# mountain/qingdai

Measured on AMD Instinct MI355X. Metric: simulated planet-days/sec at 721x1440 f64, higher is better.
Workload: dtype f64; 1 GPU; 721x1440 seed-42 planet, dt=300 s: forcing + time_step(Teq, dt, albedo) with QD_ENERGY_W=1 QD_CLOUD_COUPLE=1 + slab-ocean coupling + driver-side precipitation/cloud/albedo diagnostics (run_simulation.py:1766-1934,2063-2146) (BASELINE configs[2]; loop order of benchmark_jax.py:124-158); ocean_n_sub=13, parallelism=lat-bands x1

## Files before the change

### include/qingdai_hip.h

```cpp
#ifndef QINGDAI_HIP_H
#define QINGDAI_HIP_H

#include <stddef.h>
#include <stdint.h>

#ifdef __cplusplus
extern "C" {
#endif

#define QD_ABI_VERSION 1

typedef struct qd_ctx* qd_handle;

typedef struct qd_grid_desc {
    int32_t n_lat, n_lon;
    int32_t row0, n_rows, halo;
    int32_t device;
    int32_t rank, world;
} qd_grid_desc;

enum qd_field {
    QD_F_U = 0, QD_F_V, QD_F_H, QD_F_TS, QD_F_Q, QD_F_CLOUD, QD_F_HICE,
    QD_F_ISR, QD_F_ISR_A, QD_F_ISR_B, QD_F_TEQ, QD_F_ALBEDO,
    QD_F_OLR, QD_F_EFLUX, QD_F_PCOND, QD_F_LH, QD_F_LHREL, QD_F_CLOUD_EFF,
    QD_F_FRICTION, QD_F_CSMAP, QD_F_BASE_ALBEDO, QD_F_ELEVATION,
    QD_F_UO, QD_F_VO, QD_F_ETA, QD_F_SST, QD_F_QNET,
    QD_F_PRECIP, QD_F_CLOUD_FROM_P, QD_F_CLOUD_SRC,
    QD_F_W_LAND, QD_F_S_SNOW, QD_F_C_SNOW,
    QD_F_S_SNOW_NEXT, QD_F_MELT, QD_F_P_RAIN, QD_F_GLACIER, QD_F_RUNOFF,
    QD_F_ECO_LAI, QD_F_ECO_LAI_SNAP, QD_F_ECO_F, QD_F_ECO_EDAY, QD_F_ECO_ALPHA, QD_F_ECO_ALPHA_BANDED, QD_F_WATER_ALPHA,
    QD_F_ECO_AGE, QD_F_ECO_SEEDBANK, QD_F_ECO_GATE,
    QD_F_PHYTO_N, QD_F_KD490,
    QD_F_COUNT_F64,
    QD_F_LAND_MASK = 100, QD_F_ICE_MASK = 101,
    QD_F_ECO_DIV_LS = 110, QD_F_ECO_DIV_ALPHA = 111, QD_F_ECO_DIV_BC = 112, QD_F_ECO_DIV_SUMMARY = 113
};

typedef struct qd_params {
    double g, H, tau_rad, greenhouse_factor, a, omega;
    double t_freeze, rho_i, L_f, Cs_ocean, Cs_land, Cs_ice;
    double C_E, rho_a, h_mbl, L_v, p0, ocean_evap_scale, land_evap_scale, ice_evap_scale, tau_cond;
    double sw_a0, sw_kc, lw_eps0, lw_kc, t_floor, c_sfc;
    double energy_w, rh0, k_q, k_p, pcond_ref, hice_ref, eps_default, ch, cp_a;
    double atm_h, gh_factor_lw, eps_ocean, eps_land, eps_ice, lw_tau0, lw_ktau;
    double sigma4, k4_u, k4_v, k4_h, k4_q, k4_cloud, spec_cutoff, spec_damp, diff_factor;
    double H_ocean, rho_w, cp_w, g_ocean, CD, r_bot, rho_a_ocean, vcap, tau_scale;
    double polar_sponge_lat, polar_sponge_gain, K_h, sigma4_ocean, ocean_cfl, ocean_max_u;
    double ocean_k4_u, ocean_k4_v, ocean_k4_eta, ocean_adv_alpha, ocean_ice_qfac, eta_cap, ts_min, ts_max;
    double D_crit, k_precip, alpha_water, alpha_ice, alpha_cloud, p_betadiv, pq_min, p_blend;
    double pref, cmax, w_mem, w_p, w_src, cloud_from_p_floor, cloud_adv_alpha, cloud_smooth_sigma;
    double runoff_tau_days, wland_cap_mm, snow_thresh_K, snow_melt_rate_mm_day, snow_t_band_K;
    double snow_ddf_mm_per_k_day, snow_melt_tref_K, swe_ref_mm, swe_max_mm, snow_albedo_fresh;
    double lapse_k_kpm, land_elev_max_m, polar_ice_thick_max_m, polar_lat_thresh, rho_snow, glacier_frac, glacier_swe_mm;
    double orog_k;
    double qnet_lw_eps0, qnet_lw_kc;
    int32_t seaice_enabled, cloud_couple, lw_v2, gh_lock, polar_freeze_fix_s, polar_freeze_fix_n;
    int32_t mom_scheme;
    int32_t diff_enable, filter_type;
    int32_t diff_every, k4_nsub, diff_q, diff_cloud, shapiro_every, shapiro_n, spec_every;
    int32_t ocean_k4_nsub, ocean_diff_every, ocean_shapiro_n, ocean_shapiro_every;
    int32_t ocean_outlier;
    int32_t ocean_use_qnet, ocean_polar_fix;
    int32_t p_hybrid_fallback, cloud_advect, use_topo_albedo, has_csmap;
    int32_t snow_melt_mode;
    int32_t swe_enable, lapse_enable;
    int32_t orog_enable;
} qd_params;

int qd_abi_version(void);
int qd_device_count(void);
int qd_create(const qd_grid_desc* desc, const qd_params* params, double q_init_rh, qd_handle* out);
int qd_destroy(qd_handle h);
const char* qd_last_error(qd_handle h);

int qd_upload(qd_handle h, int field, const void* host_global, size_t bytes);
int qd_download(qd_handle h, int field, void* host_global, size_t bytes);
int qd_set_params(qd_handle h, const qd_params* params, size_t sizeof_params);
int qd_get_step_counter(qd_handle h, int64_t* atmos_counter, int64_t* ocean_counter);
int qd_set_step_counter(qd_handle h, int64_t atmos_counter, int64_t ocean_counter);

int qd_forcing(qd_handle h, const double star_a[3], const double star_b[3], double theta, int with_teq);
int qd_simple_albedo(qd_handle h, double ocean_albedo);
int qd_atmos_step(qd_handle h, double dt, int has_albedo);
int qd_ocean_step(qd_handle h, double dt, int compute_qnet, int use_ice_mask, int inject_sst);
int qd_driver_physics(qd_handle h, double dt);
int qd_hydrology_commit(qd_handle h, double dt);
int qd_step_n(qd_handle h, int n, double dt, int flags, const double* stars);
int qd_last_ocean_nsub(qd_handle h, int* n_sub);
int qd_sync(qd_handle h);

int qd_op_laplacian(qd_handle h, const double* F, int cos_kind, double* out);
int qd_op_hyperdiffuse(qd_handle h, const double* F, const double* k4_row, double k4_scalar, double dt,
                       int n_substeps, int cos_kind, double* out);
int qd_op_advect(qd_handle h, const double* field, const double* u, const double* v, double dt,
                 int cos_kind, double* out);
int qd_op_shapiro(qd_handle h, const double* F, int n, double* out);
int qd_op_zonal_filter(qd_handle h, const double* F, double cutoff, double damp, double* out);
int qd_op_divergence(qd_handle h, const double* u, const double* v, double* out);
int qd_op_vorticity(qd_handle h, const double* u, const double* v, double* out);
int qd_op_gaussian(qd_handle h, const double* F, double sigma, int mode_wrap, double* out);
int qd_op_median_positive(qd_handle h, const double* x, double dflt, double* out);
int qd_median_state(qd_handle h, double* out64);
int qd_step_scalars(qd_handle h, double* out8);
int qd_ocean_mean_next_count(qd_handle h, int64_t* out);

int qd_band_insolation(qd_handle h, int nb, const double* specA, const double* specB, const double* tray, double* out_host_or_null);

typedef struct qd_eco_params {
    double k_canopy;
    double leaf_scalar;
    double soil_ref;
    double w_lai;
    double light_update_hours;
    double recompute_lai_delta;
    int32_t substep_every_nphys;
    int32_t albedo_couple;
    int32_t bands_couple;
    int32_t water_couple;
    int32_t use_lai;
    int32_t map_f32;
} qd_eco_params;
int qd_eco_configure(qd_handle h, const qd_eco_params* p, size_t sizeof_params);
int qd_eco_set_lai_layers(qd_handle h, const double* layers, int n_planes, int init);
int qd_eco_substep(qd_handle h, double dt);
int qd_eco_banded_alpha(qd_handle h, int nb, const double* r_eff, const double* w_b);
int qd_eco_get_state(qd_handle h, double out[5]);
int qd_eco_set_state(qd_handle h, const double in[3]);

int qd_indiv_configure(qd_handle h, int n_cells, const int32_t* sample_j, const int32_t* sample_i, int n_indiv,
                       const int32_t* cell_index, const double* Ab, const double* tol, int nb, const double* specA,
                       const double* specB, const double* tray, int substeps_per_day, double day_seconds, double soil_cap,
                       int ab_f32);
int qd_indiv_substep(qd_handle h, double dt, int* fired_or_null);
int qd_indiv_download(qd_handle h, double* E_day, double* stress_days);
int qd_indiv_upload(qd_handle h, const double* E_day, const double* stress_days);

int qd_phyto_configure(qd_handle h, int n_species, double K_h, double adv_alpha);
int qd_phyto_upload(qd_handle h, int species, const double* host);
int qd_phyto_download(qd_handle h, int species, double* host);
int qd_phyto_advect_diffuse(qd_handle h, double dt_seconds);

#define QD_PHYTO_DAILY_LOG_W 4
typedef struct qd_phyto_daily_params {
    int32_t n_species, n_bands;
    int32_t idx_490;
    int32_t enable_N;
    int32_t couple;
    int32_t reserved;
    double H_mld;
    double alpha_P, Q10, T_ref, kd_exp_m;
    double sink;
    double R_remin;
    double alpha_clip_min, alpha_clip_max;
    double dt_days;
} qd_phyto_daily_params;
int qd_phyto_daily_configure(qd_handle h, const qd_phyto_daily_params* p, size_t sizeof_params, const double* band_tab,
                             const double* species_tab, const double* shape);
int qd_phyto_daily(qd_handle h, const double* star_row, int use_sst);
int qd_phyto_daily_schedule(qd_handle h, int n, const int32_t* fire);
int qd_phyto_daily_log(qd_handle h, double* out, int max, int* n);
int qd_phyto_daily_download_bands(qd_handle h, double* host, size_t n);
int qd_phyto_daily_state(qd_handle h, int64_t* n_steps);
int qd_phyto_daily_insolation(qd_handle h, const double* star_row, double* insA, double* insB);

#define QD_ECO_DAILY_LOG_W 4
#define QD_ECO_DAILY_MAX_K 8
typedef struct qd_eco_daily_params {
    int32_t n_species, n_layers;
    int32_t spread;
    int32_t moore;
    int32_t gate_soil;
    int32_t reserved;
    double lai_max, k_canopy, growth_per_j, senesce_per_day, stress_thresh, stress_strength;
    double soil_cap;
    double repro_frac;
    double spread_rate;
    double soil_exp, upfrac, dlai_max;
    double seed_energy, seed_scale;
    double seedling_lai, retain, bank_max, seed_dlai_max, germ_frac, bank_decay;
} qd_eco_daily_params;
int qd_eco_daily_configure(qd_handle h, const qd_eco_daily_params* p, size_t sizeof_params, const int32_t* species_mode,
                           const double* species_weights);
int qd_eco_daily_set_layers(qd_handle h, const double* layers, int n_planes);
int qd_eco_daily_get_layers(qd_handle h, double* layers, int n_planes);
int qd_eco_daily_step(qd_handle h, const double* soil_index);
int qd_eco_daily_schedule(qd_handle h, int n, const int32_t* fire);
int qd_eco_daily_log(qd_handle h, double* out, int max, int* n);
// ... 239 lines not shown
```

### qingdai_amd/_lib.py

```python
from __future__ import annotations

import ctypes
import os

from .params import qd_params

_HERE = os.path.dirname(os.path.abspath(__file__))
LIB_PATH = os.environ.get("QD_LIB_PATH") or os.path.join(_HERE, "libqingdai_hip.so")

FIELDS = ["U", "V", "H", "TS", "Q", "CLOUD", "HICE", "ISR", "ISR_A", "ISR_B", "TEQ", "ALBEDO",
          "OLR", "EFLUX", "PCOND", "LH", "LHREL", "CLOUD_EFF", "FRICTION", "CSMAP", "BASE_ALBEDO", "ELEVATION",
          "UO", "VO", "ETA", "SST", "QNET", "PRECIP", "CLOUD_FROM_P", "CLOUD_SRC", "W_LAND", "S_SNOW", "C_SNOW",
          "S_SNOW_NEXT", "MELT", "P_RAIN", "GLACIER", "RUNOFF",
          "ECO_LAI", "ECO_LAI_SNAP", "ECO_F", "ECO_EDAY", "ECO_ALPHA", "ECO_ALPHA_BANDED", "WATER_ALPHA",
          "ECO_AGE", "ECO_SEEDBANK", "ECO_GATE", "PHYTO_N", "KD490"]
F = {n: i for i, n in enumerate(FIELDS)}
F["LAND_MASK"] = 100
F["ICE_MASK"] = 101
F.update({"ECO_DIV_LS": 110, "ECO_DIV_ALPHA": 111, "ECO_DIV_BC": 112, "ECO_DIV_SUMMARY": 113})
R_SUM, R_COSMEAN, R_MAX, R_MIN, R_MAXABS = 0, 1, 2, 3, 4

SYMBOLS = [
    "qd_abi_version", "qd_device_count", "qd_create", "qd_destroy", "qd_last_error", "qd_upload", "qd_download", "qd_set_params",
    "qd_get_step_counter", "qd_set_step_counter", "qd_forcing", "qd_simple_albedo", "qd_atmos_step",
    "qd_ocean_step", "qd_driver_physics", "qd_hydrology_commit", "qd_step_n", "qd_last_ocean_nsub", "qd_sync",
    "qd_op_laplacian", "qd_op_hyperdiffuse", "qd_op_advect", "qd_op_shapiro", "qd_op_zonal_filter", "qd_op_divergence",
    "qd_op_vorticity", "qd_op_gaussian", "qd_op_median_positive", "qd_median_state", "qd_step_scalars", "qd_ocean_mean_next_count", "qd_reduce", "qd_energy_diagnostics", "qd_energy_diagnostics_last", "qd_band_insolation",
    "qd_comm_unique_id", "qd_comm_init", "qd_comm_init_local", "qd_comm_stats", "qd_comm_allreduce_count", "qd_comm_grouped_sum_count", "qd_comm_init_shm", "qd_comm_host_allreduce_count", "qd_hostring_open", "qd_hostring_allreduce",
    "qd_hostring_close", "qd_comm_barrier", "qd_comm_allreduce_max", "qd_peer_export", "qd_peer_connect", "qd_comm_peer_stats", "qd_comm_peer_carried", "qd_peer_selftest", "qd_peer_disable", "qd_tune_reload",
    "qd_plansim_create", "qd_plansim_destroy", "qd_plansim_plan", "qd_plansim_mark", "qd_plansim_margin", "qd_plansim_segments",
    "qd_plansim_pop_exchange", "qd_plansim_segments_rows",
    "qd_eco_configure", "qd_eco_set_lai_layers", "qd_eco_substep", "qd_eco_banded_alpha", "qd_eco_get_state", "qd_eco_set_state",
    "qd_indiv_configure", "qd_indiv_substep", "qd_indiv_download", "qd_indiv_upload",
    "qd_phyto_configure", "qd_phyto_upload", "qd_phyto_download", "qd_phyto_advect_diffuse",
    "qd_phyto_daily_configure", "qd_phyto_daily", "qd_phyto_daily_schedule", "qd_phyto_daily_log", "qd_phyto_daily_download_bands",
    "qd_phyto_daily_state", "qd_phyto_daily_insolation",
    "qd_eco_daily_configure", "qd_eco_daily_set_layers", "qd_eco_daily_get_layers", "qd_eco_daily_step", "qd_eco_daily_schedule",
    "qd_eco_daily_log", "qd_eco_daily_state", "qd_eco_daily_speciate",
    "qd_eco_state_restore",
    "qd_indiv_daily_configure", "qd_indiv_daily_step", "qd_indiv_daily_log", "qd_indiv_daily_weights", "qd_indiv_daily_state",
    "qd_eco_diversity", "qd_eco_diversity_on", "qd_eco_diversity_download",
    "qd_truecolor_configure", "qd_truecolor_render", "qd_truecolor_download",
    "qd_stateframe_configure", "qd_stateframe_scan", "qd_stateframe_render", "qd_stateframe_download",
    "qd_tiles_configure", "qd_tiles_set_plane", "qd_tiles_available", "qd_tiles_scan", "qd_tiles_order_stats", "qd_tiles_render", "qd_tiles_download",
    "qd_budget_diag_configure", "qd_budget_diag_schedule", "qd_budget_diag_log", "qd_budget_diag_reset",
    "qd_history_configure", "qd_history_schedule", "qd_history_sample", "qd_history_read", "qd_history_reset", "qd_history_restore",
    "qd_state_digest", "qd_state_scalars_get", "qd_state_scalars_set",
    "qd_route_configure", "qd_route_free", "qd_route_reset", "qd_route_accumulate", "qd_route_event", "qd_route_schedule",
    "qd_route_download", "qd_route_events", "qd_route_restore",
    "qd_hydronet_build", "qd_hydronet_sweeps",
    "qd_topogen_smooth", "qd_topogen_build", "qd_topogen_last_ms",
    "qd_copy_ceiling", "qd_timing_enable", "qd_timing_select", "qd_timing_get", "qd_timing_reset",
]


class qd_eco_params(ctypes.Structure):
    _fields_ = ([(n, ctypes.c_double) for n in ("k_canopy", "leaf_scalar", "soil_ref", "w_lai", "light_update_hours",
                                                 "recompute_lai_delta")] +
                [(n, ctypes.c_int32) for n in ("substep_every_nphys", "albedo_couple", "bands_couple", "water_couple", "use_lai", "map_f32")])


class qd_phyto_daily_params(ctypes.Structure):
    _fields_ = ([(n, ctypes.c_int32) for n in ("n_species", "n_bands", "idx_490", "enable_N", "couple", "reserved")] +
                [(n, ctypes.c_double) for n in ("H_mld", "alpha_P", "Q10", "T_ref", "kd_exp_m", "sink", "R_remin", "alpha_clip_min",
                                                 "alpha_clip_max", "dt_days")])


class qd_eco_daily_params(ctypes.Structure):
    _fields_ = ([(n, ctypes.c_int32) for n in ("n_species", "n_layers", "spread", "moore", "gate_soil", "reserved")] +
                [(n, ctypes.c_double) for n in ("lai_max", "k_canopy", "growth_per_j", "senesce_per_day", "stress_thresh", "stress_strength",
                                                 "soil_cap", "repro_frac", "spread_rate", "soil_exp", "upfrac", "dlai_max", "seed_energy",
                                                 "seed_scale", "seedling_lai", "retain", "bank_max", "seed_dlai_max", "germ_frac",
                                                 "bank_decay")])


class qd_indiv_daily_params(ctypes.Structure):
    _fields_ = ([(n, ctypes.c_int32) for n in ("n_species", "n_layers", "per_cell", "seed_couple")] +
                [(n, ctypes.c_double) for n in ("stress_penalty", "lai_grow", "lai_decay", "recruit_frac", "stress_decay", "repro_frac",
                                                 "seed_energy", "retain", "bank_max", "lai_max")])


class qd_truecolor_params(ctypes.Structure):
    _fields_ = ([(n, ctypes.c_int32) for n in ("snow_by_swe", "veg", "veg_f_one", "oceancolor", "snow_by_ts", "rivers", "lakes", "nb_eco",
                                                "nb_phyto", "reserved")] +
                [(n, ctypes.c_double) for n in ("h_ice_ref", "ice_frac_thr", "snow_cover_frac", "snow_vis_alpha", "veg_gamma", "veg_sat",
                                                 "soil_ref", "oc_gamma", "oc_blend", "snow_thresh", "cloud_alpha", "cloud_white",
                                                 "river_min", "river_alpha", "lake_alpha")])


TRUECOLOR_MAX_BANDS = 16

STATEFRAME_PANELS = 15
STATEFRAME_MAX_LEVELS = 32
STATEFRAME_GUTTER = 4
STATEFRAME_SCAN_N = 28


class qd_stateframe_params(ctypes.Structure):
    _fields_ = ([(n, ctypes.c_int32) for n in ("ps_abs", "ocean", "rivers", "lakes")] +
                [(n, ctypes.c_double) for n in ("p0", "rho_a", "H", "river_min", "river_alpha", "lake_alpha")])


class qd_stateframe_panel(ctypes.Structure):
    _fields_ = ([(n, ctypes.c_int32) for n in ("n_levels", "extend_max", "constant", "coast")] +
                [("levels", ctypes.c_double * STATEFRAME_MAX_LEVELS), ("rgb", (ctypes.c_double * 3) * STATEFRAME_MAX_LEVELS)])


class qd_stateframe_table(ctypes.Structure):
    _fields_ = [("panel", qd_stateframe_panel * STATEFRAME_PANELS), ("mark_cell", ctypes.c_int64 * 2)]

# ... 100 lines not shown
    lib.qd_op_shapiro.argtypes = [vp, vp, i32, vp]
    lib.qd_op_zonal_filter.argtypes = [vp, vp, dbl, dbl, vp]
    lib.qd_op_divergence.argtypes = [vp, vp, vp, vp]
    lib.qd_op_vorticity.argtypes = [vp, vp, vp, vp]
    lib.qd_op_gaussian.argtypes = [vp, vp, dbl, i32, vp]
    lib.qd_op_median_positive.argtypes = [vp, vp, dbl, dp]
    lib.qd_reduce.argtypes = [vp, i32, i32, dp]
    lib.qd_energy_diagnostics.argtypes = [vp, dp]
    lib.qd_energy_diagnostics_last.argtypes = [vp, dp]
    lib.qd_copy_ceiling.argtypes = [vp, sz, i32, dp]
    lib.qd_band_insolation.argtypes = [vp, i32, dp, dp, dp, vp]
    lib.qd_eco_configure.argtypes = [vp, ctypes.POINTER(qd_eco_params), sz]
    lib.qd_eco_set_lai_layers.argtypes = [vp, vp, i32, i32]
    lib.qd_eco_substep.argtypes = [vp, dbl]
    lib.qd_eco_banded_alpha.argtypes = [vp, i32, dp, dp]
    lib.qd_eco_get_state.argtypes = [vp, dp]
    lib.qd_eco_set_state.argtypes = [vp, dp]
    lib.qd_indiv_configure.argtypes = [vp, i32, ip, ip, i32, ip, vp, vp, i32, dp, dp, dp, i32, dbl, dbl, i32]
    lib.qd_indiv_substep.argtypes = [vp, dbl, ip]
    lib.qd_indiv_download.argtypes = [vp, vp, vp]
    lib.qd_indiv_upload.argtypes = [vp, vp, vp]
    lib.qd_phyto_configure.argtypes = [vp, i32, dbl, dbl]
    lib.qd_phyto_upload.argtypes = [vp, i32, vp]
    lib.qd_phyto_download.argtypes = [vp, i32, vp]
    lib.qd_phyto_advect_diffuse.argtypes = [vp, dbl]
    lib.qd_phyto_daily_configure.argtypes = [vp, ctypes.POINTER(qd_phyto_daily_params), sz, dp, dp, dp]
    lib.qd_phyto_daily.argtypes = [vp, dp, i32]
    lib.qd_phyto_daily_schedule.argtypes = [vp, i32, ip]
    lib.qd_phyto_daily_log.argtypes = [vp, dp, i32, ip]
    lib.qd_phyto_daily_download_bands.argtypes = [vp, dp, sz]
    lib.qd_phyto_daily_state.argtypes = [vp, ctypes.POINTER(i64)]
    lib.qd_phyto_daily_insolation.argtypes = [vp, dp, dp, dp]
    lib.qd_eco_daily_configure.argtypes = [vp, ctypes.POINTER(qd_eco_daily_params), sz, ip, dp]
    lib.qd_eco_daily_set_layers.argtypes = [vp, vp, i32]
    lib.qd_eco_daily_get_layers.argtypes = [vp, vp, i32]
    lib.qd_eco_state_restore.argtypes = [vp, vp, i32, dp, i32, i32, ctypes.c_double]
    lib.qd_eco_daily_step.argtypes = [vp, vp]
    lib.qd_eco_daily_schedule.argtypes = [vp, i32, ip]
    lib.qd_eco_daily_log.argtypes = [vp, dp, i32, ip]
    lib.qd_eco_daily_state.argtypes = [vp, ctypes.POINTER(i64)]
    lib.qd_eco_daily_speciate.argtypes = [vp, i32, ctypes.c_double, dp]
    lib.qd_indiv_daily_configure.argtypes = [vp, ctypes.POINTER(qd_indiv_daily_params), sz, ip, ip]
    lib.qd_indiv_daily_step.argtypes = [vp, vp]
    lib.qd_indiv_daily_log.argtypes = [vp, dp, i32, ip]
    lib.qd_indiv_daily_weights.argtypes = [vp, dp, i32]
    lib.qd_indiv_daily_state.argtypes = [vp, ctypes.POINTER(i64)]
    lib.qd_eco_diversity.argtypes = [vp, vp, i32, i32, dp, dp]
    lib.qd_eco_diversity_on.argtypes = [vp, i32, i32, u8p, vp, i32, i32, dp, dp]
    lib.qd_eco_diversity_download.argtypes = [vp, i32, dp, sz]
    lib.qd_truecolor_configure.argtypes = [vp, ctypes.POINTER(qd_truecolor_params), sz, dp, dp, dp, u8p]
    lib.qd_truecolor_render.argtypes = [vp, i32, dp, dp]
    lib.qd_truecolor_download.argtypes = [vp, i32, vp, sz]
    lib.qd_stateframe_configure.argtypes = [vp, ctypes.POINTER(qd_stateframe_params), sz, u8p]
    lib.qd_stateframe_scan.argtypes = [vp, dp, ctypes.POINTER(i64)]
    lib.qd_stateframe_render.argtypes = [vp, ctypes.POINTER(qd_stateframe_table), sz, dp, i32]
    lib.qd_stateframe_download.argtypes = [vp, i32, vp, sz]
    lib.qd_tiles_configure.argtypes = [vp, dbl, dp, i32, i32]
    lib.qd_tiles_set_plane.argtypes = [vp, dp]
    lib.qd_tiles_available.argtypes = [vp, ip]
    lib.qd_tiles_scan.argtypes = [vp, ctypes.POINTER(qd_tile_ref), i32, dp, ctypes.POINTER(i64)]
    lib.qd_tiles_order_stats.argtypes = [vp, i32, i32, ctypes.POINTER(i64), i32, dp, ctypes.POINTER(i64)]
    lib.qd_tiles_render.argtypes = [vp, ctypes.POINTER(qd_tile_desc), sz, i32, i32]
    lib.qd_tiles_download.argtypes = [vp, i32, vp, sz]
    lib.qd_budget_diag_configure.argtypes = [vp, i32, u8p]
    lib.qd_budget_diag_schedule.argtypes = [vp, i32, ip]
    lib.qd_budget_diag_log.argtypes = [vp, dp, i32, ip]
    lib.qd_budget_diag_reset.argtypes = [vp]
    lib.qd_history_configure.argtypes = [vp, i32, ip, ip, ip]
    lib.qd_history_schedule.argtypes = [vp, i32, ip]
    lib.qd_history_sample.argtypes = [vp]
    lib.qd_history_read.argtypes = [vp, dp, ctypes.POINTER(i64)]
    lib.qd_history_reset.argtypes = [vp]
    lib.qd_history_restore.argtypes = [vp, dp, i64]
    lib.qd_state_digest.argtypes = [vp, i32, ip, ctypes.POINTER(ctypes.c_uint64)]
    lib.qd_state_scalars_get.argtypes = [vp, dp, i32]
    lib.qd_state_scalars_set.argtypes = [vp, dp, i32]
    lib.qd_comm_unique_id.argtypes = [vp, sz]
    lib.qd_comm_init.argtypes = [vp, vp, sz]
    lib.qd_comm_barrier.argtypes = [vp]
    lib.qd_comm_init_local.argtypes = [ctypes.POINTER(vp), i32]
    lib.qd_median_state.argtypes = [vp, dp]
    lib.qd_step_scalars.argtypes = [vp, dp]
    lib.qd_ocean_mean_next_count.argtypes = [vp, ctypes.POINTER(i64)]
    lib.qd_comm_stats.argtypes = [vp, ctypes.POINTER(i32)]
    lib.qd_comm_allreduce_count.argtypes = [vp, ctypes.POINTER(i32)]
    lib.qd_comm_grouped_sum_count.argtypes = [vp, ctypes.POINTER(i32)]
    lib.qd_comm_init_shm.argtypes = [vp, ctypes.c_char_p]
    lib.qd_comm_host_allreduce_count.argtypes = [vp, ctypes.POINTER(i32)]
    lib.qd_hostring_open.argtypes = [ctypes.c_char_p, i32, i32, ctypes.POINTER(vp)]
    lib.qd_hostring_allreduce.argtypes = [vp, dp, i32, i32]
    lib.qd_hostring_close.argtypes = [vp]
    lib.qd_comm_allreduce_max.argtypes = [vp, dp, i32]
    lib.qd_tune_reload.argtypes = [vp]
    lib.qd_peer_export.argtypes = [vp, vp, sz]
    lib.qd_peer_connect.argtypes = [vp, vp, sz, i32]
    lib.qd_peer_selftest.argtypes = [vp, i32, ctypes.POINTER(ctypes.c_longlong)]
    lib.qd_peer_disable.argtypes = [vp]
    lib.qd_comm_peer_stats.argtypes = [vp, ctypes.POINTER(i32), ctypes.POINTER(i32)]
    lib.qd_comm_peer_carried.argtypes = [vp]
    lib.qd_plansim_create.argtypes = [ctypes.POINTER(qd_grid_desc), ctypes.POINTER(vp)]
    lib.qd_plansim_destroy.argtypes = [vp]
    lib.qd_plansim_plan.argtypes = [vp, ip, ip, i32, i32]
    lib.qd_plansim_mark.argtypes = [vp, ip, i32, i32]
    lib.qd_plansim_margin.argtypes = [vp, i32]
    lib.qd_plansim_segments.argtypes = [vp, i32, ip]
    lib.qd_plansim_pop_exchange.argtypes = [vp, ip, i32, ip]
    lib.qd_plansim_segments_rows.argtypes = [vp, i32, i32, ip]
    lib.qd_route_configure.argtypes = [vp, ctypes.POINTER(qd_route_plan), sz]
    lib.qd_route_free.argtypes = [vp]
    lib.qd_route_reset.argtypes = [vp]
    lib.qd_route_accumulate.argtypes = [vp, dbl]
    lib.qd_route_event.argtypes = [vp, dbl, i32]
    lib.qd_route_schedule.argtypes = [vp, i32, dp]
    lib.qd_route_download.argtypes = [vp, i32, dp, sz]
    lib.qd_route_events.argtypes = [vp, dp, i32, ip]
    lib.qd_route_restore.argtypes = [vp, dp, dp, dp, i64]
    lib.qd_hydronet_build.argtypes = [vp, i32, i32, u8p, dp, dbl, i32, dp, dp, dp, dbl, dp, ip, ip, u8p, ip, ip, i32,
                                      ip, ip]
    lib.qd_hydronet_sweeps.argtypes = [vp, ip]
    lib.qd_topogen_smooth.argtypes = [vp, i32, i32, dp, dp, i32, dp, i32, i32, dp]
    lib.qd_topogen_build.argtypes = [vp, i32, i32, dp, i32, dp, dp, i32, dp, dp, dp, dp, dp, ip, dp, dp, u8p, dp]
    lib.qd_topogen_last_ms.argtypes = [vp, dp]
    lib.qd_timing_enable.argtypes = [vp, i32]
    lib.qd_timing_select.argtypes = [vp, ctypes.c_char_p]
    lib.qd_timing_get.argtypes = [vp, ctypes.c_char_p, dp, ctypes.POINTER(i64)]
    lib.qd_timing_reset.argtypes = [vp]
    for s in SYMBOLS:
        getattr(lib, s).restype = i32
    lib.qd_last_error.restype = ctypes.c_char_p
    _lib = lib
    return lib
```

### qingdai_amd/csrc/qd_api.hip

```cpp
#include "qd_span.h"
#include <chrono>
#include <atomic>
#include <cstring>
#include <cstdio>
#include <cstdlib>
#include <algorithm>

thread_local std::string g_qd_create_err;

int qd_fail(qd_ctx* c, const char* what, hipError_t e) {
    std::string m = what ? what : "error";
    if (e != hipSuccess) { m += ": "; m += hipGetErrorString(e); }
    if (c) c->err = m; else g_qd_create_err = m;
    return -1;
}

static hipEvent_t qd_get_event(qd_ctx* c) {
    if (!c->ev_free.empty()) { hipEvent_t e = c->ev_free.back(); c->ev_free.pop_back(); return e; }
    hipEvent_t e = nullptr;
    hipEventCreate(&e);
    return e;
}
QdScope::QdScope(qd_ctx* c_, const char* n, bool attach_) : c(c_), name(n), attach(attach_) {
    on = c->timing == 1;
// ... 211 lines not shown
    std::atomic_thread_fence(std::memory_order_acquire);
    return 0;
}


int qd_wait_host_nonneg(qd_ctx* c, volatile double* slot, double* out, const char* what) {
    const auto t0 = std::chrono::steady_clock::now();
    unsigned spins = 0;
    double v;
    while (!((v = *slot) >= 0.0)) {
        __builtin_ia32_pause();
        if ((++spins & 0x3FFFu) == 0) {
            const hipError_t q = hipStreamQuery(c->stream);
            if (q != hipErrorNotReady && !(*slot >= 0.0)) return qd_fail(c, what, q);
            if (std::chrono::duration<double>(std::chrono::steady_clock::now() - t0).count() > 60.0) return qd_fail(c, what);
        }
    }
    *slot = -1.0;
    std::atomic_thread_fence(std::memory_order_seq_cst);
    *out = v;
    return 0;
}

__global__ void k_publish_host(const double* __restrict__ src, int n, double* dst, double* stamp, double seq) {
    if ((int)threadIdx.x < n)
        __hip_atomic_store((unsigned long long*)dst + threadIdx.x, (unsigned long long)__double_as_longlong(src[threadIdx.x]), __ATOMIC_RELAXED,
                           __HIP_MEMORY_SCOPE_SYSTEM);
    asm volatile("s_waitcnt vmcnt(0)" ::: "memory");
    if (threadIdx.x == 0)
        __hip_atomic_store((unsigned long long*)stamp, (unsigned long long)__double_as_longlong(seq), __ATOMIC_RELAXED, __HIP_MEMORY_SCOPE_SYSTEM);
}
int qd_fetch_scalars(qd_ctx* c, const double* dsrc, int n, double* hdst) {
    if (n < 1 || n > 32) return qd_fail(c, "qd_fetch_scalars: bad count");
    c->pub_seq += 1.0;
    hipLaunchKernelGGL(k_publish_host, dim3(1), dim3(64), 0, c->stream, dsrc, n, hdst, c->hpin + 61, c->pub_seq);
    if (qd_wait_host_flag(c, c->hpin + 61, c->pub_seq, "device scalars never reached the host")) return -1;
    if (c->hpin[60] != 0.0) return qd_fail(c, "peer exchange: a rank did not arrive within the deadline");
    return 0;
}

extern "C" int qd_abi_version(void) { return QD_ABI_VERSION; }
extern "C" int qd_device_count(void) { int n = 0; return hipGetDeviceCount(&n) == hipSuccess ? n : 0; }

static void qd_read_tuning(qd_ctx* c) {
    c->tune = QdTune();
    auto geti = [](const char* name, int dflt) { const char* e = std::getenv(name); return e ? std::atoi(e) : dflt; };
    QdTune& t = c->tune;
    c->stream_rows = std::max(0, geti("QD_STREAM_R", 0));
    { const int r = geti("QD_TAIL_R", 0); if (r > 0) t.tail_r = r; }
    { const int r = geti("QD_TAIL_RP", 0); if (r >= 3) t.tail_rp = r; }
    t.tail_v = geti("QD_TAIL_V", 0) == 1 ? 1 : 0;
    t.tail_general = geti("QD_TAIL_GENERAL", 0) == 1 ? 1 : 0;
    t.stream_r_dyn = std::max(0, geti("QD_STREAM_R_DYN", 0));
    t.stream_r_ocn = std::max(0, geti("QD_STREAM_R_OCN", 0));
    t.stream_vb = geti("QD_STREAM_VB", -1);
    { const int b = geti("QD_MED_BLOCKS", 0); if (b >= 16) t.med_blocks = b; }
    t.shapiro_r = std::max(0, geti("QD_SHAPIRO_R", 0));
    t.tile_tr = std::max(0, geti("QD_TILE_TR", 0));
    t.fused_r = std::max(0, geti("QD_FUSED_R", 0));
    t.fused_seq = geti("QD_FUSED_SEQ", 0) == 1 ? 1 : 0;
    t.fused_norot = geti("QD_FUSED_NOROT", 0) == 1 ? 1 : 0;
    t.stream_no_pair = geti("QD_STREAM_NO_PAIR", 0) == 1 ? 1 : 0;
}
extern "C" int qd_tune_reload(qd_handle c) { if (!c) return -1; qd_read_tuning(c); c->tile = QdTileShape{0, 0, 0, 0}; return 0; }

extern "C" int qd_create(const qd_grid_desc* d, const qd_params* params, double q_init_rh, qd_handle* out) {
    if (!d || !params || !out) return qd_fail(nullptr, "qd_create: null argument");
    if (d->n_lat < 5 || d->n_lon < 4) return qd_fail(nullptr, "qd_create: grid too small (need n_lat>=5, n_lon>=4)");
    if (d->row0 < 0 || d->n_rows < 1 || d->row0 + d->n_rows > d->n_lat || d->halo < 0)
        return qd_fail(nullptr, "qd_create: bad latitude band");
    const bool full = (d->row0 == 0 && d->n_rows == d->n_lat);
    if (full && d->halo != 0) return qd_fail(nullptr, "qd_create: a whole-globe handle takes halo = 0");
    if (!full && d->n_rows + 2 * d->halo > d->n_lat) return qd_fail(nullptr, "qd_create: band + 2 halos taller than the grid");
    if (!full && d->halo < 5) return qd_fail(nullptr, "qd_create: band handles need halo >= 5 rows");
    int ndev = 0;
    if (hipGetDeviceCount(&ndev) != hipSuccess || ndev == 0) return qd_fail(nullptr, "qd_create: no HIP device visible");
    if (d->device < 0 || d->device >= ndev) return qd_fail(nullptr, "qd_create: bad device ordinal");
    qd_ctx* c = new qd_ctx();
    c->desc = *d; c->p = *params;
    { const char* ef = std::getenv("QD_FUSED"); if (ef && ef[0] == '0') c->use_fused = 0; }
    { const char* ef = std::getenv("QD_FUSED_FAST"); if (ef) c->fused_fast = std::atoi(ef); }
    { const char* ef = std::getenv("QD_TAIL_ACC"); if (ef) c->tail_acc = std::atoi(ef); }
    { const char* ef = std::getenv("QD_MEAN_IN_MOMENTUM"); if (ef) c->mean_in_momentum = ef[0] == '0' ? 0 : 1; }
    { const char* ef = std::getenv("QD_SHAPIRO_STREAM"); if (ef) c->shapiro_stream = std::atoi(ef); }
    { const char* ef = std::getenv("QD_OCN_TAIL"); if (ef) c->ocn_tail = std::atoi(ef); }
    if (c->ocn_tail != 0) c->ocn_tail = 1;
    { const char* ef = std::getenv("QD_OCN_FUSED"); if (ef) c->ocn_fused = ef[0] == '1' ? 1 : 0; }
    { const char* ef = std::getenv("QD_BAND_TAIL"); if (ef) c->band_tail = ef[0] == '0' ? 0 : 1; }
    qd_read_tuning(c);
    { const char* ef = std::getenv("QD_GROUP_SUMS"); if (ef) c->group_sums = ef[0] == '0' ? 0 : 1; }
    c->geo = QdGeom{d->n_lat, d->n_lon, d->row0, d->n_rows, d->halo, full ? 1 : 0, d->row0 - d->halo, d->n_rows + 2 * d->halo};
    c->own_row0 = d->row0; c->own_nrows = d->n_rows;
    auto bail = [&](const char* w, hipError_t e) { qd_fail(nullptr, w, e); qd_destroy(c); return -1; };
    hipError_t e;
    if ((e = hipSetDevice(d->device)) != hipSuccess) return bail("hipSetDevice", e);
    if ((e = hipStreamCreate(&c->stream)) != hipSuccess) return bail("hipStreamCreate", e);
    { int ncu = 0; c->n_cu = (hipDeviceGetAttribute(&ncu, hipDeviceAttributeMultiprocessorCount, d->device) == hipSuccess && ncu > 0) ? ncu : 256; }
    const size_t cells = c->geo.cells() + (size_t)QD_PAD_ROWS * c->geo.nlon;
    for (int f = 0; f < QD_F_COUNT_F64; ++f) {
        if ((e = hipMalloc(&c->f[f], cells * sizeof(double))) != hipSuccess) return bail("hipMalloc field", e);
        hipMemsetAsync(c->f[f], 0, cells * sizeof(double), c->stream);
    }
    for (int s = 0; s < QD_NSCRATCH; ++s) {
        if ((e = hipMalloc(&c->scratch[s], cells * sizeof(double))) != hipSuccess) return bail("hipMalloc scratch", e);
        hipMemsetAsync(c->scratch[s], 0, cells * sizeof(double), c->stream);
    }
    if ((e = hipMalloc(&c->land, cells)) != hipSuccess) return bail("hipMalloc mask", e);
    if ((e = hipMalloc(&c->icemask, cells)) != hipSuccess) return bail("hipMalloc mask", e);
    hipMemsetAsync(c->land, 0, cells, c->stream); hipMemsetAsync(c->icemask, 0, cells, c->stream);
    if (build_tables(c)) return bail("table allocation", hipErrorOutOfMemory);
    if ((e = hipMalloc(&c->k4_atm, (size_t)5 * d->n_lat * sizeof(double))) != hipSuccess) return bail("hipMalloc", e);
    if ((e = hipMalloc(&c->k4_ocn, (size_t)3 * d->n_lat * sizeof(double))) != hipSuccess) return bail("hipMalloc", e);
    c->red_blocks = (12 + (d->n_lon + QD_BLOCK - 1) / QD_BLOCK) * c->geo.lrows() + 64;
    if ((e = hipMalloc(&c->red_partial, (size_t)c->red_blocks * sizeof(double))) != hipSuccess) return bail("hipMalloc", e);
    if ((e = hipMalloc(&c->dscal, QD_S_COUNT * sizeof(double))) != hipSuccess) return bail("hipMalloc", e);
    if ((e = hipMalloc(&c->dcount, 32 * sizeof(unsigned long long))) != hipSuccess) return bail("hipMalloc", e);
    if ((e = hipMalloc(&c->eta_acc, 1024 * sizeof(unsigned long long))) != hipSuccess) return bail("hipMalloc", e);
    hipMemsetAsync(c->eta_acc, 0, 1024 * sizeof(unsigned long long), c->stream);
    if ((e = hipMalloc(&c->hist, 2 * QD_HIST_BINS * sizeof(unsigned int))) != hipSuccess) return bail("hipMalloc", e);
    if ((e = hipMalloc(&c->sel_state, 8 * sizeof(unsigned long long))) != hipSuccess) return bail("hipMalloc", e);
    hipMemsetAsync(c->dscal, 0, QD_S_COUNT * sizeof(double), c->stream);
    hipMemsetAsync(c->dcount, 0, 32 * sizeof(unsigned long long), c->stream);
    hipMemsetAsync(c->hist, 0, 2 * QD_HIST_BINS * sizeof(unsigned int), c->stream);
    hipMemsetAsync(c->sel_state, 0, 8 * sizeof(unsigned long long), c->stream);
    { const char* ef = std::getenv("QD_TAIL_FIX"); if (ef) c->tail_fix = ef[0] == '0' ? 0 : 1; }
    c->fix_dense = 256.0 * (double)c->geo.cells() / (721.0 * 1440.0);
    { const char* ef = std::getenv("QD_TAIL_FIX_DENSE"); if (ef) c->fix_dense = std::atof(ef); }
    { const char* ef = std::getenv("QD_LAZY_DIAG"); if (ef) c->lazy_diag = ef[0] == '0' ? 0 : 1; }
    if (c->tail_fix) {
        if ((e = hipMalloc(&c->fix_count, 64)) != hipSuccess) return bail("hipMalloc", e);
        hipMemsetAsync(c->fix_count, 0, 64, c->stream);
        if ((e = hipMalloc(&c->fix_list, c->geo.cells() * 3 * sizeof(unsigned long long))) != hipSuccess) return bail("hipMalloc", e);
    }
    if (!full) {
        if ((e = hipMalloc(&c->med_pred, 64 * sizeof(double))) != hipSuccess) return bail("hipMalloc", e);
        hipMemsetAsync(c->med_pred, 0, 64 * sizeof(double), c->stream);
        if ((e = hipMalloc(&c->med_gather, (size_t)std::max(1, d->world) * 4096 * sizeof(double))) != hipSuccess) return bail("hipMalloc", e);
        if ((e = hipMalloc(&c->sel_ccount, 2 * sizeof(unsigned int))) != hipSuccess) return bail("hipMalloc", e);
        hipMemsetAsync(c->sel_ccount, 0, 2 * sizeof(unsigned int), c->stream);
        { const char* ef = std::getenv("QD_MEDIAN_PREDICT"); if (ef && ef[0] == '0') c->med_predict = 0; }
    }
    if (full) {
        if ((e = hipMalloc(&c->sel_cand, 2 * cells * sizeof(double))) != hipSuccess) return bail("hipMalloc", e);
        if ((e = hipMalloc(&c->sel_ccount, 2 * sizeof(unsigned int))) != hipSuccess) return bail("hipMalloc", e);
        hipMemsetAsync(c->sel_ccount, 0, 2 * sizeof(unsigned int), c->stream);
        if ((e = hipMalloc(&c->med_pred, 64 * sizeof(double))) != hipSuccess) return bail("hipMalloc", e);
        hipMemsetAsync(c->med_pred, 0, 64 * sizeof(double), c->stream);
        { const char* ef = std::getenv("QD_MEDIAN_PREDICT"); if (ef && ef[0] == '0') c->med_predict = 0; }
        { const char* ef = std::getenv("QD_MERGE_POINTWISE"); if (ef) c->merge_pointwise = ef[0] == '0' ? 0 : 1; }
        { const char* ef = std::getenv("QD_HOIST_PRECIP"); if (ef) c->hoist_precip = ef[0] == '0' ? 0 : 1; }
        { const char* ef = std::getenv("QD_SIDE_STREAM"); if (ef) c->side_stream_on = ef[0] == '0' ? 0 : 1; }
        { const char* ef = std::getenv("QD_MERGE_FINAL"); if (ef) c->merge_final = ef[0] == '0' ? 0 : 1; }
        { const char* ef = std::getenv("QD_MERGE_PCOND"); if (ef) c->merge_pcond = ef[0] == '0' ? 0 : 1; }


        c->n_wgmax = (int)(qd_grid2d(c->geo).x * (unsigned)c->geo.nrows);
        if ((e = hipMalloc(&c->wgmax, (size_t)2 * c->n_wgmax * sizeof(double))) != hipSuccess) return bail("hipMalloc", e);
        { const char* ef = std::getenv("QD_MED_SIDE"); if (ef) c->med_side = ef[0] == '0' ? 0 : 1; }
        { const char* ef = std::getenv("QD_MED_PAIR"); if (ef) c->med_pair = ef[0] == '0' ? 0 : 1; }
        { const char* ef = std::getenv("QD_MED_FOLD"); if (ef) c->med_fold = ef[0] == '0' ? 0 : 1; }
        { const char* ef = std::getenv("QD_MERGE_SAF"); if (ef) c->merge_saf = ef[0] == '0' ? 0 : 1; }
        if (c->med_side) {
            if ((e = hipEventCreateWithFlags(&c->med_fork, hipEventDisableTiming)) != hipSuccess) return bail("hipEventCreate", e);
            if ((e = hipEventCreateWithFlags(&c->med_done, hipEventDisableTiming)) != hipSuccess) return bail("hipEventCreate", e);
        }
        if (c->med_side || c->med_pair) {
            if ((e = hipMalloc(&c->hist_b, 2 * QD_HIST_BINS * sizeof(unsigned int))) != hipSuccess) return bail("hipMalloc", e);
            if ((e = hipMalloc(&c->sel_state_b, 8 * sizeof(unsigned long long))) != hipSuccess) return bail("hipMalloc", e);
            if ((e = hipMalloc(&c->sel_cand_b, 2 * cells * sizeof(double))) != hipSuccess) return bail("hipMalloc", e);
            if ((e = hipMalloc(&c->sel_ccount_b, 2 * sizeof(unsigned int))) != hipSuccess) return bail("hipMalloc", e);
            hipMemsetAsync(c->hist_b, 0, 2 * QD_HIST_BINS * sizeof(unsigned int), c->stream);
            hipMemsetAsync(c->sel_state_b, 0, 8 * sizeof(unsigned long long), c->stream);
            hipMemsetAsync(c->sel_ccount_b, 0, 2 * sizeof(unsigned int), c->stream);
        }
        if ((c->side_stream_on || c->med_side) && (e = hipStreamCreateWithFlags(&c->side_stream, hipStreamNonBlocking)) != hipSuccess) return bail("hipStreamCreate", e);
        if (c->side_stream_on) {
            if ((e = hipEventCreateWithFlags(&c->side_fork, hipEventDisableTiming)) != hipSuccess) return bail("hipEventCreate", e);
            if ((e = hipEventCreateWithFlags(&c->side_done, hipEventDisableTiming)) != hipSuccess) return bail("hipEventCreate", e);
            if ((e = hipMalloc(&c->red_partial_b, (size_t)c->red_blocks * sizeof(double))) != hipSuccess) return bail("hipMalloc", e);
        }
    }
    if ((e = hipHostMalloc((void**)&c->hpin, 64 * sizeof(double), hipHostMallocMapped | hipHostMallocCoherent)) != hipSuccess) return bail("hipHostMalloc", e);
    if ((e = hipHostMalloc((void**)&c->hpin_rows, (size_t)3 * c->geo.lrows() * sizeof(double), hipHostMallocMapped | hipHostMallocCoherent)) != hipSuccess) return bail("hipHostMalloc", e);
    std::memset(c->hpin, 0, 64 * sizeof(double));
    c->hpin[57] = -1.0; c->hpin[58] = -1.0; c->hpin[59] = -1.0;
    std::memset(c->hpin_rows, 0, (size_t)3 * c->geo.lrows() * sizeof(double));
    const double q0 = std::min(std::max(q_init_rh, 0.0), 1.0) * host_qsat(288.0, params->p0);
    hipLaunchKernelGGL(k_init_state, dim3((d->n_lon + QD_BLOCK - 1) / QD_BLOCK, c->geo.lrows()), dim3(QD_BLOCK), 0,
                       c->stream, c->geo, c->tabs, params->H, q0, c->f[QD_F_H], c->f[QD_F_TS], c->f[QD_F_Q], c->f[QD_F_SST]);
    if ((e = hipStreamSynchronize(c->stream)) != hipSuccess) return bail("init", e);
    if (!full) {
        for (int f = 0; f < QD_F_COUNT_F64; ++f) c->vm[c->f[f]] = d->halo;
        c->vm[c->land] = d->halo; c->vm[c->icemask] = d->halo;
    }
    *out = c;
    return 0;
}

extern "C" int qd_destroy(qd_handle c) {
    if (!c) return 0;
    hipSetDevice(c->desc.device);
    if (c->stream) hipStreamSynchronize(c->stream);
    if (c->med_pred && std::getenv("QD_MEDIAN_DEBUG")) {
        double h[64];
        if (hipMemcpy(h, c->med_pred, sizeof(h), hipMemcpyDeviceToHost) == hipSuccess)
            for (int s = 0; s < 4; ++s)
                fprintf(stderr, "[median site %d] last median %.6g bracket [%.6g, %.6g] hits %.0f misses %.0f last list %.0f of %.0f; "
                        "last miss at call %.0f: centre %.6g -> median %.6g\n", s, h[16 * s], h[16 * s + 8], h[16 * s + 9], h[16 * s + 4],
                        h[16 * s + 5], h[16 * s + 6], h[16 * s + 7], h[16 * s + 13], h[16 * s + 14], h[16 * s + 15]);
    }
    qd_phyto_release(c);
    qd_route_release(c);
    qd_phyto_daily_release(c);
    qd_indiv_daily_release(c);
    qd_eco_daily_release(c);
    qd_eco_div_release(c);
    qd_truecolor_release(c);
    qd_stateframe_release(c);
    qd_tiles_release(c);
    qd_budget_release(c);
    qd_history_release(c);
    for (int f = 0; f < QD_F_COUNT_F64; ++f) if (c->f[f]) hipFree(c->f[f]);
    for (int s = 0; s < QD_NSCRATCH; ++s) if (c->scratch[s]) hipFree(c->scratch[s]);
    for (double* t : c->tab_alloc) hipFree(t);
    if (c->land) hipFree(c->land); if (c->icemask) hipFree(c->icemask);
    if (c->k4_atm) hipFree(c->k4_atm); if (c->k4_ocn) hipFree(c->k4_ocn); for (int k = 0; k < 2; ++k) if (c->qs_tab[k]) hipFree(c->qs_tab[k]);
    if (c->red_partial) hipFree(c->red_partial); if (c->dscal) hipFree(c->dscal);
    if (c->red_partial_b) hipFree(c->red_partial_b);
    if (c->wgmax) hipFree(c->wgmax);
    qd_saf_drop(c);
    if (c->fix_count && std::getenv("QD_TAIL_FIX_DEBUG")) {
        unsigned int h[8] = {0};
        if (hipMemcpy(h, c->fix_count, sizeof(h), hipMemcpyDeviceToHost) == hipSuccess)
            fprintf(stderr, "[tail fix list] %u entries in %u launches (%.1f per launch), longest list %u of %zu cells\n", h[4], h[5],
                    h[5] ? (double)h[4] / h[5] : 0.0, h[6], c->geo.cells());
    }
    if (c->fix_count) hipFree(c->fix_count); if (c->fix_list) hipFree(c->fix_list);
    if (c->side_stream) { hipStreamSynchronize(c->side_stream); hipStreamDestroy(c->side_stream); }
    if (c->side_fork) hipEventDestroy(c->side_fork); if (c->side_done) hipEventDestroy(c->side_done);
    if (c->med_fork) hipEventDestroy(c->med_fork); if (c->med_done) hipEventDestroy(c->med_done);
    if (c->hist_b) hipFree(c->hist_b); if (c->sel_state_b) hipFree(c->sel_state_b); if (c->sel_cand_b) hipFree(c->sel_cand_b); if (c->sel_ccount_b) hipFree(c->sel_ccount_b);
    if (c->eta_acc) hipFree(c->eta_acc);
    if (c->dcount) hipFree(c->dcount); if (c->hist) hipFree(c->hist); if (c->sel_state) hipFree(c->sel_state);
    if (c->zonal_tw) hipFree(c->zonal_tw);
    if (c->bands) hipFree(c->bands);
    if (c->digest_out) hipFree(c->digest_out);
    qd_eco_free(c);
    if (c->sel_cand) hipFree(c->sel_cand); if (c->sel_ccount) hipFree(c->sel_ccount);
    if (c->med_pred) hipFree(c->med_pred);
    if (c->med_gather) hipFree(c->med_gather);
    qd_comm_release(c);
    if (c->hpin) hipHostFree(c->hpin);
    if (c->hpin_rows) hipHostFree(c->hpin_rows);
    if (c->stage) hipHostFree(c->stage);
    qd_resolve_timers(c);
    for (hipEvent_t e : c->ev_free) hipEventDestroy(e);
    if (c->stream) hipStreamDestroy(c->stream);
    delete c;
    return 0;
}

extern "C" const char* qd_last_error(qd_handle c) { return c ? c->err.c_str() : g_qd_create_err.c_str(); }

int qd_band_copy_in(qd_ctx* c, void* dst, const void* host, size_t esz) {
    const QdGeom& G = c->geo;
    const size_t rowb = (size_t)G.nlon * esz;
    if (G.full) return hipMemcpyAsync(dst, host, rowb * G.nlat, hipMemcpyHostToDevice, c->stream) == hipSuccess ? 0 : -1;
    for (int l = 0; l < G.lrows(); ++l) {
        int g = l + G.row0 - G.halo;
        if (g < 0) g += G.nlat; if (g >= G.nlat) g -= G.nlat;
        if (hipMemcpyAsync((char*)dst + (size_t)l * rowb, (const char*)host + (size_t)g * rowb, rowb,
                           hipMemcpyHostToDevice, c->stream) != hipSuccess) return -1;
    }
    return 0;
}

extern "C" int qd_upload(qd_handle c, int field, const void* host, size_t bytes) {
    if (!c || !host) return -1;
    hipSetDevice(c->desc.device);
    const size_t n = (size_t)c->geo.nlat * c->geo.nlon;
    if (field == QD_F_LAND_MASK || field == QD_F_ICE_MASK) {
        if (bytes != n) return qd_fail(c, "qd_upload: mask size mismatch");
        uint8_t* dst = field == QD_F_LAND_MASK ? c->land : c->icemask;
        if (qd_band_copy_in(c, dst, host, 1)) return qd_fail(c, "qd_upload: copy failed");
        qd_mark(c, {dst}, c->geo.halo);
    } else {
        if (field < 0 || field >= QD_F_COUNT_F64) return qd_fail(c, "qd_upload: unknown field");
        if (bytes != n * sizeof(double)) return qd_fail(c, "qd_upload: size mismatch (expect n_lat*n_lon float64)");
        if (qd_eco_is_f32(c, field)) {
            if (qd_band_copy_in(c, c->scratch[10], host, sizeof(double))) return qd_fail(c, "qd_upload: copy failed");
            qd_eco_convert_slab(c, c->scratch[10], 0, c->f[field], 1);
        } else if (qd_band_copy_in(c, c->f[field], host, sizeof(double))) return qd_fail(c, "qd_upload: copy failed");
        qd_mark(c, {c->f[field]}, c->geo.halo);
        if (field == QD_F_CLOUD_EFF) c->cloud_eff_valid = 1;
        if (field == QD_F_ELEVATION) c->has_elevation = 1;
        if (field == QD_F_ECO_ALPHA) c->eco.alpha_valid = 1;
        if (field == QD_F_ECO_ALPHA_BANDED) c->eco.banded_valid = 1;
        if (field == QD_F_WATER_ALPHA) c->eco.water_valid = 1;
    }
    QD_HIP(c, hipStreamSynchronize(c->stream));
    if (field == QD_F_LAND_MASK) {
        const uint8_t* m = (const uint8_t*)host;
        const int nlat = c->geo.nlat, nlon = c->geo.nlon;
        double ws = 0.0;
        for (int i = 0; i < nlat; ++i) {
            const double w = std::max(std::cos((-90.0 + 180.0 * i / (double)(nlat - 1)) * (M_PI / 180.0)), 0.0);
            int cnt = 0;
            for (int j = 0; j < nlon; ++j) cnt += (m[(size_t)i * nlon + j] == 0);
            ws += w * cnt;
        }
        c->wsum_ocean = ws;
    }
    return 0;
}

extern "C" int qd_download(qd_handle c, int field, void* host, size_t bytes) {
    if (!c || !host) return -1;
    hipSetDevice(c->desc.device);
    const QdGeom& G = c->geo;
    const size_t n = (size_t)G.nlat * G.nlon;
    const void* src; size_t esz;
    if (field == QD_F_LAND_MASK || field == QD_F_ICE_MASK) { src = field == QD_F_LAND_MASK ? c->land : c->icemask; esz = 1; }
    else {
        if (field < 0 || field >= QD_F_COUNT_F64) return qd_fail(c, "qd_download: unknown field");
        src = c->f[field]; esz = sizeof(double);
        if (qd_eco_is_f32(c, field)) { qd_eco_convert_slab(c, c->f[field], 1, c->scratch[10], 0); src = c->scratch[10]; }
    }
    if (bytes != n * esz) return qd_fail(c, "qd_download: size mismatch");
    const size_t rowb = (size_t)G.nlon * esz;
    QD_HIP(c, hipMemcpyAsync((char*)host + (size_t)G.row0 * rowb, (const char*)src + (size_t)G.halo * rowb,
                             rowb * G.nrows, hipMemcpyDeviceToHost, c->stream));
    QD_HIP(c, hipStreamSynchronize(c->stream));
    return 0;
}

extern "C" int qd_set_params(qd_handle c, const qd_params* p, size_t sz) {
    if (!c || !p) return -1;
    if (sz != sizeof(qd_params)) return qd_fail(c, "qd_set_params: struct size mismatch (ABI drift)");
    const bool tabs_stale = (p->omega != c->p.omega) || (p->g != c->p.g) || (p->a != c->p.a) || (p->polar_sponge_lat != c->p.polar_sponge_lat) ||
                            (p->polar_sponge_gain != c->p.polar_sponge_gain);
    c->p = *p;
    c->k4_atm_dt = -1; c->k4_ocn_dt = -1;
    if (tabs_stale) {
        hipSetDevice(c->desc.device);
        hipStreamSynchronize(c->stream);
        for (double* t : c->tab_alloc) hipFree(t);
        c->tab_alloc.clear();
        if (build_tables(c)) return qd_fail(c, "qd_set_params: table rebuild failed");
    }
    return 0;
}

extern "C" int qd_get_step_counter(qd_handle c, int64_t* a, int64_t* o) {
    if (!c) return -1; if (a) *a = c->atm_counter; if (o) *o = c->ocn_counter; return 0;
}
extern "C" int qd_set_step_counter(qd_handle c, int64_t a, int64_t o) {
    if (!c) return -1; c->atm_counter = a; c->ocn_counter = o; return 0;
}
extern "C" int qd_sync(qd_handle c) {
    if (!c) return -1;
    hipSetDevice(c->desc.device);
    QD_HIP(c, hipStreamSynchronize(c->stream));
    return 0;
}
extern "C" int qd_last_ocean_nsub(qd_handle c, int* n) { if (!c || !n) return -1; *n = c->last_nsub; return 0; }

extern "C" int qd_forcing(qd_handle c, const double sa[3], const double sb[3], double theta, int with_teq) {
    if (!c || !sa || !sb) return -1;
    hipSetDevice(c->desc.device);
    return qd_forcing_impl(c, sa, sb, theta, with_teq);
}
extern "C" int qd_simple_albedo(qd_handle c, double ocean_albedo) {
    if (!c) return -1;
    hipSetDevice(c->desc.device);
    return qd_simple_albedo_impl(c, ocean_albedo);
}
extern "C" int qd_atmos_step(qd_handle c, double dt, int has_albedo) {
    if (!c) return -1;
    hipSetDevice(c->desc.device);
    if (int rc = qd_atmos_step_impl(c, dt, has_albedo)) return rc;
    return qd_launch_check(c, "qd_atmos_step");
}
extern "C" int qd_ocean_step(qd_handle c, double dt, int compute_qnet, int use_ice_mask, int inject_sst) {
    if (!c) return -1;
    hipSetDevice(c->desc.device);
    if (int rc = qd_ocean_step_impl(c, dt, compute_qnet, use_ice_mask, inject_sst)) return rc;
    return qd_launch_check(c, "qd_ocean_step");
}
extern "C" int qd_driver_physics(qd_handle c, double dt) {
    if (!c) return -1;
    hipSetDevice(c->desc.device);
    if (int rc = qd_driver_physics_impl(c, dt)) return rc;
    return qd_launch_check(c, "qd_driver_physics");
}
// ... 148 lines not shown
    qd_hyperdiffuse_fields(c, fl, 1, tab, &skip, &ov, dt, n_substeps, cos_kind ? c->tabs.cos05 : c->tabs.cos02, 0);
    int rc = seam_out(c, fl[0], out);
    if (fl[0] != save10) { for (int s = 0; s < QD_NSCRATCH; ++s) if (c->scratch[s] == save10 && s != 10) { c->scratch[s] = fl[0]; break; } c->scratch[10] = save10; }
    return rc;
}

extern "C" int qd_op_advect(qd_handle c, const double* field, const double* u, const double* v, double dt,
                            int cos_kind, double* out) {
    if (!c || !field || !u || !v || !out) return -1;
    hipSetDevice(c->desc.device);
    if (seam_in(c, c->scratch[10], field) || seam_in(c, c->scratch[11], u) || seam_in(c, c->scratch[12], v)) return -1;
    qd_launch_advect(c, c->scratch[11], c->scratch[12], cos_kind ? c->tabs.cos05 : c->tabs.cos6, dt,
                     c->scratch[10], c->scratch[13], nullptr, nullptr, 1.0, 0, 0);
    return seam_out(c, c->scratch[13], out);
}

extern "C" int qd_op_shapiro(qd_handle c, const double* F, int n, double* out) {
    if (!c || !F || !out) return -1;
    hipSetDevice(c->desc.device);
    if (seam_in(c, c->scratch[10], F)) return -1;
    double* fl[1] = {c->scratch[10]};
    double* save10 = c->scratch[10];
    qd_shapiro_fields(c, fl, 1, n, 0);
    int rc = seam_out(c, fl[0], out);
    if (fl[0] != save10) { for (int s = 0; s < QD_NSCRATCH; ++s) if (c->scratch[s] == save10 && s != 10) { c->scratch[s] = fl[0]; break; } c->scratch[10] = save10; }
    return rc;
}

static int seam_divvort(qd_ctx* c, const double* u, const double* v, double* out, int vort) {
    if (!c || !u || !v || !out) return -1;
    hipSetDevice(c->desc.device);
    if (seam_in(c, c->scratch[10], u) || seam_in(c, c->scratch[11], v)) return -1;
    qd_launch_divvort(c, c->scratch[10], c->scratch[11], c->scratch[12], vort, 0);
    return seam_out(c, c->scratch[12], out);
}
extern "C" int qd_op_zonal_filter(qd_handle c, const double* F, double cutoff, double damp, double* out) {
    if (!c || !F || !out) return -1;
    hipSetDevice(c->desc.device);
    if (seam_in(c, c->scratch[10], F)) return -1;
    double* fl[1] = {c->scratch[10]};
    if (qd_zonal_filter_fields(c, fl, 1, cutoff, damp, 0)) return -1;
    return seam_out(c, c->scratch[10], out);
}
extern "C" int qd_op_divergence(qd_handle c, const double* u, const double* v, double* out) { return seam_divvort(c, u, v, out, 0); }
extern "C" int qd_op_vorticity(qd_handle c, const double* u, const double* v, double* out) { return seam_divvort(c, u, v, out, 1); }

extern "C" int qd_op_gaussian(qd_handle c, const double* F, double sigma, int mode_wrap, double* out) {
    if (!c || !F || !out) return -1;
    hipSetDevice(c->desc.device);
    if (seam_in(c, c->scratch[10], F)) return -1;
    if (qd_gaussian(c, c->scratch[10], c->scratch[11], c->scratch[12], sigma, mode_wrap, 0)) return -1;
    return seam_out(c, c->scratch[11], out);
}

extern "C" int qd_op_median_positive(qd_handle c, const double* x, double dflt, double* out) {
    if (!c || !x || !out) return -1;
    hipSetDevice(c->desc.device);
    if (seam_in(c, c->scratch[10], x)) return -1;
    qd_median_positive_dev(c, c->scratch[10], dflt, QD_S_MED_OUT, 0, 0.0, 0);
    QD_HIP(c, hipMemcpyAsync(c->hpin, c->dscal + QD_S_MED_OUT, sizeof(double), hipMemcpyDeviceToHost, c->stream));
    QD_HIP(c, hipStreamSynchronize(c->stream));
    *out = c->hpin[0];
    return 0;
}

extern "C" int qd_median_state(qd_handle c, double* out64) {
    if (!c || !out64) return -1;
    hipSetDevice(c->desc.device);
    for (int k = 0; k < 16 * 4; ++k) out64[k] = 0.0;
    if (!c->med_pred) return 0;
    QD_HIP(c, hipStreamSynchronize(c->stream));
    QD_HIP(c, hipMemcpy(out64, c->med_pred, sizeof(double) * 16 * 4, hipMemcpyDeviceToHost));
    return 0;
}

extern "C" int qd_step_scalars(qd_handle c, double* out8) {
    if (!c || !out8) return -1;
    hipSetDevice(c->desc.device);
    QD_HIP(c, hipStreamSynchronize(c->stream));
    QD_HIP(c, hipMemcpy(out8, c->dscal, sizeof(double) * 8, hipMemcpyDeviceToHost));
    return 0;
}

extern "C" int qd_ocean_mean_next_count(qd_handle c, int64_t* out) {
    if (!c || !out) return -1;
    *out = c->mean_next_count;
    return 0;
}

extern "C" int qd_reduce(qd_handle c, int field, int op, double* out) {
    if (!c || !out) return -1;
    if (field < 0 || field >= QD_F_COUNT_F64) return qd_fail(c, "qd_reduce: unknown field");
    hipSetDevice(c->desc.device);
    double v = 0;
    const int op1 = (op == QD_R_COSWEIGHTED_MEAN) ? 1 : (op == QD_R_SUM ? 0 : (op == QD_R_MAX ? 2 : (op == QD_R_MIN ? 3 : 4)));
    if (qd_reduce_field(c, c->f[field], op1, &v)) return -1;
    if (op == QD_R_COSWEIGHTED_MEAN) v = v / (c->wsum_all + 1e-15);
    *out = v;
    return 0;
}

extern "C" int qd_band_insolation(qd_handle c, int nb, const double* specA, const double* specB, const double* tray, double* out_host) {
    if (!c || !specA || !specB || !tray) return -1;
    hipSetDevice(c->desc.device);
    return qd_band_insolation_impl(c, nb, specA, specB, tray, out_host);
}
extern "C" int qd_energy_diagnostics_last(qd_handle c, double* out) {
    if (!c || !out) return -1;
    for (int k = 0; k < 10; ++k) out[k] = c->last_diag[k];
    return 0;
}
extern "C" int qd_energy_diagnostics(qd_handle c, double* out) {
    if (!c || !out) return -1;
    hipSetDevice(c->desc.device);
    return qd_energy_diag_impl(c, out);
}

extern "C" int qd_copy_ceiling(qd_handle c, size_t bytes, int reps, double* gbs) {
    if (!c || !gbs || bytes == 0 || reps < 1) return -1;
    hipSetDevice(c->desc.device);
    void *a = nullptr, *b = nullptr;
    if (hipMalloc(&a, bytes) != hipSuccess || hipMalloc(&b, bytes) != hipSuccess) { if (a) hipFree(a); return qd_fail(c, "qd_copy_ceiling: hipMalloc"); }
    hipMemsetAsync(a, 1, bytes, c->stream); hipMemsetAsync(b, 2, bytes, c->stream);
    hipEvent_t e0, e1;
    hipEventCreate(&e0); hipEventCreate(&e1);
    hipMemcpyAsync(b, a, bytes, hipMemcpyDeviceToDevice, c->stream);
    hipEventRecord(e0, c->stream);
    for (int r = 0; r < reps; ++r) hipMemcpyAsync((r & 1) ? a : b, (r & 1) ? b : a, bytes, hipMemcpyDeviceToDevice, c->stream);
    hipEventRecord(e1, c->stream);
    hipStreamSynchronize(c->stream);
    float ms = 0.f;
    hipEventElapsedTime(&ms, e0, e1);
    hipEventDestroy(e0); hipEventDestroy(e1);
    hipFree(a); hipFree(b);
    *gbs = ms > 0.f ? (2.0 * (double)bytes * reps / 1e9) / ((double)ms / 1e3) : 0.0;
    return 0;
}

extern "C" int qd_timing_enable(qd_handle c, int on) { if (!c) return -1; c->timing = on ? 1 : 0; return 0; }
extern "C" int qd_timing_select(qd_handle c, const char* name) {
    if (!c || !name) return -1; c->timing = 2; c->timing_sel = name; return 0;
}
extern "C" int qd_timing_reset(qd_handle c) { if (!c) return -1; qd_resolve_timers(c); c->timers.clear(); c->timing_seen.clear(); return 0; }
extern "C" int qd_timing_get(qd_handle c, const char* name, double* mean_ms, int64_t* launches) {
    if (!c || !name) return -1;
    hipSetDevice(c->desc.device);
    qd_resolve_timers(c);
    auto it = c->timers.find(name);
    if (it == c->timers.end() || it->second.n == 0) { if (mean_ms) *mean_ms = 0; if (launches) *launches = 0; return 0; }
    if (mean_ms) *mean_ms = it->second.total_ms / (double)it->second.n;
    if (launches) *launches = it->second.n;
    return 0;
}
```

### qingdai_amd/csrc/qd_fused.h

```cpp
#pragma once
#include "qd_internal.h"

struct QdDynArgs {
    const double *u, *v, *h, *fric, *q, *cloud;
    double *uo, *vo, *ho, *qo, *co;
    const double* k4row[5];
    double k4s[5];
    int skip[5];
    double g, a, dt, dlat, dlon, f_min;
    double inv_dlon, inv_2dlon, inv_dlat, inv_2dlat, pgf_y;
    int primitive;
    int fast;
    QdTileShape ts;
};


struct QdOcnArgs {
    const double *uo, *vo, *eta, *taux, *tauy;
    const uint8_t* land;
    double *uo_out, *vo_out, *eta_out;
    const double* k4row[3];
    double k4s[3];
    int skip[3];
    double a, g, dlat, dlon, sub_dt, rhoH, r_bot;
    double inv_2dlon, inv_2dlat, inv_a, inv_rhoH;
    const double* eta_mean;
    double eta_cap;
    int fast;
    QdTileShape ts;
    const unsigned long long* acc_read = nullptr;
    const double* acc_partial = nullptr;
    int acc_n = 0;
    double acc_wsum = 0.0;
};


QdTileShape qd_pick_tile(const QdGeom& G);
int qd_launch_dyn_hyper(qd_ctx* c, QdDynArgs& P, int margin);
int qd_launch_ocn_hyper(qd_ctx* c, QdOcnArgs& P, int margin);

bool qd_stream_ok(const qd_ctx* c, int margin);
bool qd_ocn_stream_ok(const qd_ctx* c, int margin);
int qd_launch_dyn_stream(qd_ctx* c, const QdDynArgs& P, int margin);
int qd_launch_ocn_stream(qd_ctx* c, const QdOcnArgs& P, int margin);
bool qd_ocn_stream_ok_list(const qd_ctx* c, const QdSegList& S);
int qd_launch_ocn_stream_list(qd_ctx* c, const QdOcnArgs& P, const QdSegList& S);
```

### qingdai_amd/csrc/qd_internal.h

```cpp
#pragma once

#include <hip/hip_runtime.h>
#include <hip/hip_ext.h>
#include <stdint.h>
#include <string>
#include <vector>
#include <functional>
#include <map>
#include <unordered_map>
#include <initializer_list>
#include <climits>
#include <cfloat>
#include <cmath>

#include "../../include/qingdai_hip.h"

#define QD_NSCRATCH 16
#define QD_MAX_DEVICES 64
#define QD_PAD_ROWS 8
#define QD_BLOCK 256
#define QD_MAXF 5
#define QD_HIST_BINS 2048

struct QdGeom {
// ... 138 lines not shown
    double k4_atm_dt = -1, k4_ocn_dt = -1;
    int k4_atm_skip[5] = {0}, k4_ocn_skip[3] = {0};
    double* red_partial = nullptr;
    int red_blocks = 0;
    double* dscal = nullptr;
    unsigned long long* dcount = nullptr;
    unsigned int* hist = nullptr;
    unsigned long long* sel_state = nullptr;
    double* bands = nullptr;
    int bands_nb = 0;
    double last_diag[10] = {0};
    int has_elevation = 0;
    QdPhyto phyto;
    QdEco eco;
    struct QdRoute* route = nullptr;
    struct QdPhytoDaily* pdaily = nullptr;
    struct QdEcoDaily* edaily = nullptr;
    struct QdIndivDaily* idaily = nullptr;
    struct QdEcoDiv* ediv = nullptr;
    struct QdTrueColor* tcol = nullptr;
    struct QdTiles* tiles = nullptr;
    struct QdStateFrame* sframe = nullptr;
    struct QdBudget* budget = nullptr;
    struct QdHistory* history = nullptr;
    unsigned long long* digest_out = nullptr;
    double budget_fire = 0.0;
    int hydronet_sweeps = -1;
    double topogen_ms = -1.0;
    double* zonal_tw = nullptr;
    double* sel_cand = nullptr;
    unsigned int* sel_ccount = nullptr;
    double* med_pred = nullptr;
    int med_predict = 1;
    int med_seen[4] = {0, 0, 0, 0};
    double* pending_sum = nullptr;
    int group_sums = 1;
    long grouped_sums = 0;
    int band_tail = 1;
    double* qt_tab = nullptr;
    double qt_tab_a = 0.0;
    int hoist_precip = 1;
    int precip_done = 0;
    int lazy_diag = 1, diag_write = 1;
    int merge_pcond = 1;
    int med_pair = 1;
    int med_fold = 0;
    int med_side = 0;
    bool med_side_active = false;
    hipEvent_t med_fork = nullptr, med_done = nullptr;
    unsigned int* hist_b = nullptr; unsigned long long* sel_state_b = nullptr; double* sel_cand_b = nullptr; unsigned int* sel_ccount_b = nullptr;
    int want_pcond_ahead = 0;
    int pcond_ahead = 0;
    int tail_fix = 1;
    unsigned int* fix_count = nullptr;
    unsigned long long* fix_list = nullptr;
    double fix_avg = 0.0;
    double fix_dense = 256.0;
    int64_t fix_probe_at = 0;
    int fix_probe_every = 32;
    int merge_saf = 1;
    void* saf_pending = nullptr;
    int defer_final = 0;
    int merge_final = 1;
    struct { int on = 0; double dt = 0, decay = 0, dfac = 0; } final_pending;
    double* wgmax = nullptr;
    int n_wgmax = 0;
    int side_stream_on = 0;
    hipStream_t side_stream = nullptr;
    hipEvent_t side_fork = nullptr, side_done = nullptr;
    bool side_pending = false;
    double* red_partial_b = nullptr;
    std::function<int()> before_cfl_wait;
    int merge_pointwise = 1;
    double* med_gather = nullptr;
    double* hpin = nullptr;
    double* hpin_rows = nullptr;
    double wsum_ocean = 0, wsum_all = 0;
    int64_t atm_counter = 0, ocn_counter = 0;
    QdTileShape tile{0, 0, 0, 0};
    int use_fused = 1;
    int fused_fast = 1;
    long long mean_next_count = 0;
    int mean_in_momentum = 1;
    int tail_acc = 1;
    unsigned long long* eta_acc = nullptr;
    int shapiro_stream = 1;
    int ocn_fused = 0;
    int ocn_tail = 1;
    int stream_rows = 0;
    double* qs_tab[2] = {nullptr, nullptr};
    double qs_key[2][8] = {{NAN, 0, 0, 0, 0, 0, 0, 0}, {NAN, 0, 0, 0, 0, 0, 0, 0}};
    std::vector<double> h_lapK[2];
    std::vector<double> h_k4[2];
    QdTune tune;
    int n_cu = 0;
    int qs_wgs_per_cu[3] = {0, 0, 0};
    int cloud_eff_valid = 0;
    int last_nsub = 0;
    void* stage = nullptr; size_t stage_bytes = 0;
    std::unordered_map<const void*, int> vm;
    int own_row0 = 0, own_nrows = 0;
    void* comm = nullptr;
    struct QdLocalGroup* lgroup = nullptr;
    struct QdPeer* peer = nullptr;
    std::vector<struct QdUse> split_pending;
    std::vector<struct QdUse> corefresh;
    int exchanges = 0;
    int allreduces = 0;
    double pub_seq = 0.0;
    double eta_seq = 0.0;
    void* hring = nullptr;
    void* plansim = nullptr;
    int host_allreduces = 0;
    const char* lap_tag = "k_laplacian";
    const char* hyp_tag = "k_hyper_apply";
    int timing = 0;
    std::string timing_sel;
    std::map<std::string, long> timing_seen;
    std::map<std::string, QdTimer> timers;
    struct Pending { hipEvent_t e0, e1; std::string name; };
    std::vector<Pending> pending;
    std::vector<hipEvent_t> ev_free;
    std::string err;
};

enum { QD_S_PREF = 0, QD_S_ETA_MEAN, QD_S_MED_OUT, QD_S_PSCALE, QD_S_RENORM, QD_S_PQMEAN, QD_S_TMP0, QD_S_TMP1,
       QD_S_DIAG0 = 16,
       QD_S_COUNT = 32 };

extern thread_local std::string g_qd_create_err;

int qd_fail(qd_ctx* c, const char* what, hipError_t e = hipSuccess);
#define QD_HIP(c, call) do { hipError_t _e = (call); if (_e != hipSuccess) return qd_fail((c), #call, _e); } while (0)
inline int qd_launch_check(qd_ctx* c, const char* who) {
    const hipError_t e = hipGetLastError();
    return e == hipSuccess ? 0 : qd_fail(c, (std::string(who) + ": launch").c_str(), e);
}
inline bool qd_whole_globe(const qd_ctx* c) { return c->geo.full && c->desc.world <= 1; }
struct QdPartials {
    double* p = nullptr; int nblk = 0, planes = 0; size_t cap = 0;
    int ensure(qd_ctx* c, int planes_, int nblk_) {
        const size_t n = (size_t)planes_ * (size_t)nblk_;
        if (!p || cap < n) {
            free();
            QD_HIP(c, hipMalloc(&p, n * sizeof(double)));
            cap = n;
        }
        planes = planes_; nblk = nblk_;
        return 0;
    }
    void free() { if (p) hipFree(p); p = nullptr; cap = 0; }
};

struct QdScope {
    qd_ctx* c; const char* name; hipEvent_t e0 = nullptr, e1 = nullptr; bool on = false, attach = false;
    bool used = false;
    QdScope(qd_ctx* c_, const char* n, bool attach_ = false);
    ~QdScope();
};
#define QD_LAUNCH_TIMED(sc, kernel, grid, block, stream, ...) do { \
    if ((sc).on && (sc).attach) { (sc).used = true; hipExtLaunchKernelGGL(kernel, grid, block, 0, stream, (sc).e0, (sc).e1, 0, __VA_ARGS__); } \
    else hipLaunchKernelGGL(kernel, grid, block, 0, stream, __VA_ARGS__); } while (0)

#define QD_IN(ptr, r) QdUse{(void**)&(ptr), (r), 0}
#define QD_IN8(ptr, r) QdUse{(void**)&(ptr), (r), 1}
int qd_allreduce_sum_deferred(qd_ctx* c, double* dptr);
// ... 152 lines not shown
```

### qingdai_amd/csrc/qd_ocean.hip

```cpp
#include <cstdlib>
#include <atomic>
#include <chrono>
#include "qd_internal.h"
#include "qd_device.h"
#include "qd_wave.h"

#include "qd_fluxes.h"
#include "qd_fused.h"
#include "qd_ocntail.h"
#include "qd_band.h"
#include "qd_blockred.h"

QdColP qd_make_colp(const qd_ctx* c, double dt);

__global__ void __launch_bounds__(QD_BLOCK)
k_qnet(QdGeom G, QdColP P, const double* __restrict__ isr, const double* __restrict__ albedo,
       const double* __restrict__ cloud, const double* __restrict__ Ts, const double* __restrict__ h,
       const double* __restrict__ u, const double* __restrict__ v, const uint8_t* __restrict__ land,
       const double* __restrict__ hice, const double* __restrict__ LH, double* __restrict__ qnet,
       uint8_t* __restrict__ icemask) {
    const QdTile tl = qd_tile();
    const int j = tl.seg * QD_BLOCK + threadIdx.x;
    if (j >= G.nlon) return;
    const size_t o = (size_t)qd_lrow(G, G.row0 + tl.row) * G.nlon + j;
// ... 716 lines not shown
            } else {
            for (int k = 0; k < G.nrows; ++k)
                if (qd_wait_host_flag(c, c->hpin_rows + (size_t)2 * G0.lrows() + k, c->eta_seq, "ocean step: the CFL maxima never arrived")) return -1;
            for (int k = 0; k < G.nrows; ++k) { maxVa = std::max(maxVa, c->hpin_rows[k]); maxUo = std::max(maxUo, c->hpin_rows[G.nrows + k]); }
            }
        } else {
        const bool hooked = qd_peer_hooks(c) && !qd_has_host_ring(c) && S.n <= 3;
        for (int k = 0; k < S.n; ++k) {
            const QdGeom& G = S.g[k];
            hipLaunchKernelGGL(k_stress_max, dim3(1, G.nrows), blk, 0, c->stream, G, F[QD_F_U], F[QD_F_V], F[QD_F_UO],
                               F[QD_F_VO], p.vcap, p.rho_a_ocean * p.CD, p.tau_scale, taux, tauy,
                               c->red_partial + (size_t)k * 2 * G0.lrows(), (double*)nullptr, 0.0);
            if (!hooked)
            hipLaunchKernelGGL(k_max2_finish, dim3(1), blk, 0, c->stream, c->red_partial + (size_t)k * 2 * G0.lrows(), G.nrows,
                               c->dscal + QD_S_TMP0 + 2 * k, k == S.n - 1 ? 2 * (3 - S.n) : 0);
        }
        qd_mark(c, {taux, tauy}, m);
        if (hooked) {
            QdPeerHook H; H.pre = 3; H.partial = c->red_partial; H.pstride = (size_t)2 * G0.lrows(); H.nseg = S.n;
            for (int k = 0; k < S.n; ++k) H.nsegrows[k] = S.g[k].nrows;
            c->allreduces++;
            c->pub_seq += 1.0;
            H.fixstat = (c->tail_fix && c->fix_count) ? c->fix_count : nullptr;
            if (qd_peer_allreduce_hooked(c, c->dscal + QD_S_TMP0, H.fixstat ? 7 : 6, 1, H, c->hpin, c->pub_seq)) return -1;
            if (qd_wait_host_flag(c, c->hpin + 61, c->pub_seq, "reduced scalars never reached the host")) return -1;
            if (c->hpin[60] != 0.0) return qd_fail(c, "peer exchange: a rank did not arrive within the deadline");
            if (H.fixstat && c->hpin[6] >= 0.0) c->fix_avg = c->hpin[6];
            band_fix_stats = H.fixstat != nullptr;
        } else if (qd_has_host_ring(c)) {
            QD_HIP(c, hipMemcpyAsync(c->hpin, c->dscal + QD_S_TMP0, 6 * sizeof(double), hipMemcpyDeviceToHost, c->stream));
            QD_HIP(c, hipStreamSynchronize(c->stream));
            if (qd_host_allreduce(c, c->hpin, 6, 1)) return -1;
        } else {
        if (qd_allreduce_fetch(c, c->dscal + QD_S_TMP0, 6, 1, c->hpin)) return -1;
        }
        for (int k = 0; k < 3; ++k) { maxVa = std::max(maxVa, c->hpin[2 * k]); maxUo = std::max(maxUo, c->hpin[2 * k + 1]); }
        }
        const double dx_lat = p.a * c->dlat;
        const double min_cos = 0.5;
        const double dx_lon_min = p.a * c->dlon * std::max(1e-3, min_cos);
        const double dx_min = std::min(dx_lat, dx_lon_min);
        const double cg = std::sqrt(p.g_ocean * H);
        double uadv = std::max(maxUo, maxVa);
        const double target = std::max(1e-3, p.ocean_cfl);
        const double v = std::ceil(std::max(cg, uadv) * (dt / std::max(1e-12, dx_min)) / target);
        n_sub = (v != v) ? 1 : (v > 500.0 ? 500 : (v < 1.0 ? 1 : (int)v));
        c->last_nsub = n_sub;
    }
    bool fix_now = c->tail_fix && c->fix_count && (!band || band_fix_stats);
    if (fix_now) {
        if (c->fix_avg <= c->fix_dense) c->fix_probe_every = 32;
        else if (step >= c->fix_probe_at) {
            c->fix_probe_at = step + c->fix_probe_every;
            c->fix_probe_every = std::min(256, c->fix_probe_every * 2);
        } else fix_now = false;
    }
    const double sub_dt = dt / n_sub;
    QdOcnP OP{p.a, p.g_ocean, c->dlat, c->dlon, sub_dt, p.rho_w * H, p.r_bot};
    QdHeatP HP{sub_dt, p.K_h, p.rho_w * p.cp_w * H, p.ocean_ice_qfac, p.ocean_use_qnet ? 1 : 0, use_ice_mask ? 1 : 0};
    const bool do_diff = (p.ocean_diff_every > 0) && (step % p.ocean_diff_every == 0);
    const bool do_shap = (p.ocean_shapiro_n > 0) && (p.ocean_shapiro_every > 0) && (step % p.ocean_shapiro_every == 0);
    if (do_diff) { int rc = qd_build_k4_tables(c, dt, true, sub_dt); if (rc) return rc; }
    const double ov[3] = {p.ocean_k4_u, p.ocean_k4_v, p.ocean_k4_eta};
    const int Ro = qd_adv_reach(c, sub_dt, 4.0);

    const bool can_defer = do_diff && c->use_fused && p.ocean_k4_nsub == 1 && !do_shap && c->wsum_ocean > 0.0;
    const bool band_defer = band && can_defer && qd_has_host_ring(c);
    const bool band_tail = band && can_defer && !band_defer && c->ocn_tail == 1 && c->tail_acc && c->band_tail && G0.nlon >= 64 &&
                           G0.halo >= std::max(7, Ro + 2);
    const bool defer_eta = (!band && can_defer) || band_defer || band_tail;
    double* const mean_ptr = band_defer ? c->hpin + 42 : c->dscal + QD_S_ETA_MEAN;
    struct CoRefresh { qd_ctx* c; ~CoRefresh() { c->corefresh.clear(); } } corefresh_guard{c};
    if (band) c->corefresh = {QD_IN(F[QD_F_UO], 0), QD_IN(F[QD_F_VO], 0), QD_IN(F[QD_F_ETA], 0), QD_IN(F[QD_F_SST], 0), QD_IN(taux, 0),
                              QD_IN(tauy, 0), QD_IN(F[QD_F_QNET], 0), QD_IN8(c->icemask, 0)};
    const bool use_tail = c->use_fused && (!band || band_tail) && defer_eta && G0.nlon >= 64 && c->ocn_tail;
    const bool tail_acc = use_tail && c->tail_acc;
    const bool use_fused1 = use_tail && !band && c->ocn_fused && c->ocn_tail == 1 && tail_acc && c->fused_fast == 1 && do_diff &&
                            p.ocean_k4_nsub == 1 && !do_shap && HP.use_q && HP.K_h > 0.0 && qd_ocn_fused_ok(c) &&
                            !c->k4_ocn_skip[0] && !c->k4_ocn_skip[1] && !c->k4_ocn_skip[2];
    const bool mean_form_ok = c->mean_in_momentum && !band && G0.full && tail_acc && !use_fused1 && do_diff && c->use_fused && n_sub > 1 &&
                              p.ocean_k4_nsub == 1 && !do_shap && qd_ocn_tail_is_fast(c) && qd_ocn_stream_ok(c, 0);
    if (mean_form_ok) fix_now = false;
    const bool mean_next_ok = mean_form_ok;
    unsigned long long* acc_pending = nullptr;
    for (int s = 0; s < n_sub; ++s) {
        if (use_fused1) {
            QdOcnArgs O;
            O.uo = F[QD_F_UO]; O.vo = F[QD_F_VO]; O.eta = F[QD_F_ETA]; O.taux = taux; O.tauy = tauy; O.land = c->land;
            O.uo_out = qd_scratch(c, 0); O.vo_out = qd_scratch(c, 1); O.eta_out = qd_scratch(c, 6);
            for (int f = 0; f < 3; ++f) {
                const bool sc1 = !(ov[f] != ov[f]);
                O.k4row[f] = sc1 ? nullptr : c->k4_ocn + (size_t)f * G0.nlat;
                O.k4s[f] = sc1 ? ov[f] : 0.0;
                O.skip[f] = c->k4_ocn_skip[f];
            }
            O.a = p.a; O.g = p.g_ocean; O.dlat = c->dlat; O.dlon = c->dlon; O.sub_dt = sub_dt; O.rhoH = p.rho_w * H; O.r_bot = p.r_bot;
            O.inv_2dlon = 1.0 / (2.0 * c->dlon); O.inv_2dlat = 1.0 / (2.0 * c->dlat); O.inv_a = 1.0 / p.a; O.inv_rhoH = 1.0 / (p.rho_w * H);
            O.eta_mean = s > 0 ? mean_ptr : nullptr;
            O.eta_cap = p.eta_cap;
            QdTailArgs A;
            A.uo = O.uo_out; A.vo = O.vo_out; A.eta_in = O.eta_out; A.Ts = F[QD_F_SST]; A.qnet = F[QD_F_QNET]; A.land = c->land; A.ice = c->icemask;
            A.eta = qd_scratch(c, 2); A.Ts_out = qd_scratch(c, 3); A.uo_out = qd_scratch(c, 12); A.vo_out = qd_scratch(c, 13); A.partial = c->red_partial;
            A.a = p.a; A.dlat = c->dlat; A.dlon = c->dlon; A.sub_dt = sub_dt; A.msdtH = -sub_dt * H; A.alpha = p.ocean_adv_alpha;
            A.K_h = HP.K_h; A.rcH = HP.rcH; A.ice_qfac = HP.ice_qfac; A.cap = p.ocean_max_u;
            A.use_q = HP.use_q; A.has_ice = HP.has_ice; A.mean4 = p.ocean_outlier == 0 ? 1 : 0;
            A.r_a = 1.0 / p.a; A.r_dlon = 1.0 / c->dlon; A.r_dlat = 1.0 / c->dlat; A.r_2dlon = 1.0 / (2 * c->dlon); A.r_2dlat = 1.0 / (2 * c->dlat);
            A.r_rcH = 1.0 / HP.rcH;
            A.acc = c->eta_acc; A.mean_out = c->dscal + QD_S_ETA_MEAN; A.wsum = c->wsum_ocean;
            if (qd_launch_ocn_fused(c, O, A)) return -1;
            qd_swap(c, QD_F_UO, 12); qd_swap(c, QD_F_VO, 13); qd_swap(c, QD_F_ETA, 2); qd_swap(c, QD_F_SST, 3);
            continue;
        }
        if (do_diff && c->use_fused && p.ocean_k4_nsub == 1) {
            const QdUse narrow[5] = {QD_IN(F[QD_F_ETA], 5), QD_IN(F[QD_F_UO], 4), QD_IN(F[QD_F_VO], 4), QD_IN(taux, 4), QD_IN(tauy, 4)};
            bool pending = false;
            int m_old = 0;
            if (band_tail) {
                const QdUse wide[8] = {QD_IN(F[QD_F_ETA], 7), QD_IN(F[QD_F_UO], 6), QD_IN(F[QD_F_VO], 6), QD_IN(taux, 6), QD_IN(tauy, 6),
                                       QD_IN(F[QD_F_SST], Ro + 2), QD_IN(F[QD_F_QNET], 0), QD_IN8(c->icemask, 0)};
                if (qd_plan_begin(c, wide, 8, &pending) < 0) return -1;
                if (pending) m_old = qd_plan_peek(c, narrow, 5);
            }
            QdOcnArgs O;
            O.uo = F[QD_F_UO]; O.vo = F[QD_F_VO]; O.eta = F[QD_F_ETA]; O.taux = taux; O.tauy = tauy; O.land = c->land;
            O.uo_out = qd_scratch(c, 0); O.vo_out = qd_scratch(c, 1); O.eta_out = qd_scratch(c, 2);
            for (int f = 0; f < 3; ++f) {
                const bool sc1 = !(ov[f] != ov[f]);
                O.k4row[f] = sc1 ? nullptr : c->k4_ocn + (size_t)f * G0.nlat;
                O.k4s[f] = sc1 ? ov[f] : 0.0;
                O.skip[f] = c->k4_ocn_skip[f];
            }
            O.a = p.a; O.g = p.g_ocean; O.dlat = c->dlat; O.dlon = c->dlon; O.sub_dt = sub_dt; O.rhoH = p.rho_w * H; O.r_bot = p.r_bot;
            O.inv_2dlon = 1.0 / (2.0 * c->dlon); O.inv_2dlat = 1.0 / (2.0 * c->dlat); O.inv_a = 1.0 / p.a; O.inv_rhoH = 1.0 / (p.rho_w * H);
            O.eta_mean = (defer_eta && s > 0) ? mean_ptr : nullptr;
            O.eta_cap = p.eta_cap;
            if (acc_pending) { O.acc_read = acc_pending; O.acc_partial = c->red_partial; O.acc_n = qd_ocn_tail_tiles(c, Gown); O.acc_wsum = c->wsum_ocean; }
            int m_int = 0;
            bool split = false;
            if (pending) {
                m_int = m_old >= 0 ? m_old : -12;
                const QdSegList Si = qd_segments_rows(c, c->own_row0 - m_int, c->own_nrows + 2 * m_int);
                if (c->own_nrows + 2 * m_int >= 12 && qd_ocn_stream_ok_list(c, Si)) {
                    if (qd_launch_ocn_stream_list(c, O, Si)) return -1;
                    split = true;
                }
                if (qd_plan_end(c)) return -1;
            }
            const int m = qd_plan(c, narrow, 5);
            if (m < 0) return -1;
            if (qd_allreduce_flush(c)) return -1;
            if (split && m > m_int) {
                QdSegList Sb = qd_segments_rows(c, c->own_row0 - m, m - m_int);
                Sb = qd_segments_rows(c, c->own_row0 + c->own_nrows + m_int, m - m_int, Sb);
                if (!qd_ocn_stream_ok_list(c, Sb)) {
                    if (qd_launch_ocn_hyper(c, O, m)) return -1;
                } else if (qd_launch_ocn_stream_list(c, O, Sb)) return -1;
            } else if (!split) {
                if (qd_launch_ocn_hyper(c, O, m)) return -1;
            }
            qd_mark(c, {O.uo_out, O.vo_out, O.eta_out}, m);
            qd_swap(c, QD_F_UO, 0); qd_swap(c, QD_F_VO, 1); qd_swap(c, QD_F_ETA, 2);
        } else {
            {
                QdScope sc(c, "ocean_momentum");
                const int m = qd_plan(c, {QD_IN(F[QD_F_ETA], 1), QD_IN(F[QD_F_UO], 0), QD_IN(F[QD_F_VO], 0), QD_IN(taux, 0),
                                          QD_IN(tauy, 0)});
                if (m < 0) return -1;
                QD_ROWS(c, m, G, hipLaunchKernelGGL(k_ocean_momentum, qd_grid2d(G), blk, 0, c->stream, G, c->tabs, OP,
                                                    F[QD_F_ETA], taux, tauy, c->land, F[QD_F_UO], F[QD_F_VO]));
                qd_mark(c, {F[QD_F_UO], F[QD_F_VO]}, m);
            }
            if (do_diff) {
                QdScope sc(c, "ocean_hyperdiffusion");
                const int ns = std::max(1, p.ocean_k4_nsub);
                const int m = qd_plan(c, {QD_IN(F[QD_F_UO], 4 * ns), QD_IN(F[QD_F_VO], 4 * ns), QD_IN(F[QD_F_ETA], 4 * ns)});
                if (m < 0) return -1;
                double* fl[3] = {F[QD_F_UO], F[QD_F_VO], F[QD_F_ETA]};
                c->lap_tag = "ocean_k_laplacian"; c->hyp_tag = "ocean_k_hyper_apply";
                qd_hyperdiffuse_fields(c, fl, 3, c->k4_ocn, c->k4_ocn_skip, ov, sub_dt, ns, c->tabs.cos05, m);
                c->lap_tag = "k_laplacian"; c->hyp_tag = "k_hyper_apply";
                F[QD_F_UO] = fl[0]; F[QD_F_VO] = fl[1]; F[QD_F_ETA] = fl[2];
            }
        }
        if (do_shap) {
            const int np_ = p.ocean_shapiro_n;
            const int m = qd_plan(c, {QD_IN(F[QD_F_UO], np_), QD_IN(F[QD_F_VO], np_), QD_IN(F[QD_F_ETA], np_)});
            if (m < 0) return -1;
            double* fl[3] = {F[QD_F_UO], F[QD_F_VO], F[QD_F_ETA]};
            qd_shapiro_fields(c, fl, 3, np_, m);
            F[QD_F_UO] = fl[0]; F[QD_F_VO] = fl[1]; F[QD_F_ETA] = fl[2];
        }
        if (use_tail) {
            QdTailArgs A;
            A.uo = F[QD_F_UO]; A.vo = F[QD_F_VO]; A.Ts = F[QD_F_SST]; A.qnet = F[QD_F_QNET]; A.land = c->land; A.ice = c->icemask;
            A.eta = F[QD_F_ETA]; A.Ts_out = qd_scratch(c, 1); A.uo_out = qd_scratch(c, 2); A.vo_out = qd_scratch(c, 3); A.partial = c->red_partial;
            A.a = p.a; A.dlat = c->dlat; A.dlon = c->dlon; A.sub_dt = sub_dt; A.msdtH = -sub_dt * H; A.alpha = p.ocean_adv_alpha;
            A.K_h = HP.K_h; A.rcH = HP.rcH; A.ice_qfac = HP.ice_qfac; A.cap = p.ocean_max_u;
            A.use_q = HP.use_q; A.has_ice = HP.has_ice; A.mean4 = p.ocean_outlier == 0 ? 1 : 0;
            A.r_a = 1.0 / p.a; A.r_dlon = 1.0 / c->dlon; A.r_dlat = 1.0 / c->dlat; A.r_2dlon = 1.0 / (2 * c->dlon); A.r_2dlat = 1.0 / (2 * c->dlat);
            A.r_rcH = 1.0 / HP.rcH;
            A.acc = tail_acc ? c->eta_acc : nullptr; A.mean_out = c->dscal + QD_S_ETA_MEAN; A.wsum = c->wsum_ocean;
            if (band) {
                const int m = qd_plan(c, {QD_IN(F[QD_F_UO], 2), QD_IN(F[QD_F_VO], 2), QD_IN(F[QD_F_ETA], 0), QD_IN(F[QD_F_SST], Ro + 2),
                                          QD_IN(F[QD_F_QNET], 0), QD_IN8(c->icemask, 0)});
                if (m < 0) return -1;
                A.own0 = c->own_row0; A.own1 = c->own_row0 + c->own_nrows;
                QdSegs S = qd_segments(c, m);
                size_t off = 0;
                QdPeerFold pf;
                const bool folded = qd_peer_fold_begin(c, &pf);
                if (fix_now && S.n == 1) { A.fix_count = c->fix_count; A.fix_list = c->fix_list; }
                for (int k = 0; k < S.n; ++k) {
                    const QdGeom& Gs = S.g[k];
                    const bool owned = Gs.row0 <= c->own_row0 && c->own_row0 < Gs.row0 + Gs.nrows;
                    A.acc = owned ? c->eta_acc : nullptr;
                    A.pf = owned ? pf : QdPeerFold();
                    A.partial = c->red_partial + off;
                    if (qd_launch_ocn_tail(c, Gs, A)) return -1;
                    off += (size_t)qd_ocn_tail_tiles(c, Gs);
                }
                if (!folded && qd_allreduce_sum_deferred(c, c->dscal + QD_S_ETA_MEAN)) return -1;
                if (A.fix_count) qd_mark(c, {F[QD_F_ETA], A.Ts_out, F[QD_F_UO], F[QD_F_VO]}, m);
                else qd_mark(c, {F[QD_F_ETA], A.Ts_out, A.uo_out, A.vo_out}, m);
            } else {
            if (fix_now) { A.fix_count = c->fix_count; A.fix_list = c->fix_list; }
            A.acc_clear = acc_pending;
            acc_pending = (mean_next_ok && s + 1 < n_sub) ? QD_ACC_NEXT_SET(c->eta_acc, s & 1) : nullptr;
            A.acc_next = acc_pending;
            if (acc_pending) c->mean_next_count++;
            if (qd_launch_ocn_tail(c, Gown, A)) return -1;
            if (!tail_acc)
                hipLaunchKernelGGL(k_eta_mean_tail, dim3(1), dim3(256), 0, c->stream, c->red_partial, qd_ocn_tail_tiles(c, Gown), c->wsum_ocean,
                                   c->dscal + QD_S_ETA_MEAN);
            }
            qd_swap(c, QD_F_SST, 1);
            if (!A.fix_count) { qd_swap(c, QD_F_UO, 2); qd_swap(c, QD_F_VO, 3); }
        } else if (c->use_fused) {
            QdScope sc(c, "ocean_cont_sst");
            bool band_raw_mean = false;
            const int m = qd_plan(c, {QD_IN(F[QD_F_UO], 1), QD_IN(F[QD_F_VO], 1), QD_IN(F[QD_F_ETA], 0), QD_IN(F[QD_F_SST], Ro)});
            if (m < 0) return -1;
            double* T1 = qd_scratch(c, 0);
            const int own0 = c->own_row0, own1 = c->own_row0 + c->own_nrows;
            const int has_ocean = c->wsum_ocean > 0.0 ? 1 : 0;
            if (!band) {
                const dim3 g2 = qd_grid2d(Gown);
                hipLaunchKernelGGL(k_cont_sstadv, g2, blk, 0, c->stream, Gown, c->tabs, p.a, c->dlat, c->dlon, -sub_dt * H, sub_dt,
                                   p.ocean_adv_alpha, F[QD_F_UO], F[QD_F_VO], c->land, F[QD_F_ETA], F[QD_F_SST], T1, own0, own1,
                                   c->red_partial, (unsigned long long*)nullptr, 0.0, (double*)nullptr);
                if (!defer_eta)
                    hipLaunchKernelGGL(k_eta_mean, dim3(1), blk, 0, c->stream, c->red_partial, (int)(g2.x * g2.y), c->wsum_ocean,
                                       c->dscal + QD_S_ETA_MEAN);
            } else {
                QdSegs S = qd_segments(c, m);
                size_t off = 0;
                for (int k = 0; k < S.n; ++k) {
                    hipLaunchKernelGGL(k_cont_sstadv, qd_grid2d(S.g[k]), blk, 0, c->stream, S.g[k], c->tabs, p.a, c->dlat, c->dlon,
                                       -sub_dt * H, sub_dt, p.ocean_adv_alpha, F[QD_F_UO], F[QD_F_VO], c->land, F[QD_F_ETA],
                                       F[QD_F_SST], T1, own0, own1, c->red_partial + off, (unsigned long long*)nullptr, 0.0,
                                       (double*)nullptr);
                    off += (size_t)S.g[k].nrows * qd_grid2d(S.g[k]).x;
                }
                if (band_defer) {
                    c->eta_seq += 1.0;
                    hipLaunchKernelGGL(k_eta_mean, dim3(1), blk, 0, c->stream, c->red_partial, (int)off, -1.0, c->hpin + 40, c->eta_seq);
                } else {
                hipLaunchKernelGGL(k_eta_mean, dim3(1), blk, 0, c->stream, c->red_partial, (int)off, -1.0, c->dscal + QD_S_ETA_MEAN);
                if (qd_allreduce_f64(c, c->dscal + QD_S_ETA_MEAN, 1, 0)) return -1;
                band_raw_mean = !defer_eta;
                if (!band_raw_mean)
                    hipLaunchKernelGGL(k_eta_mean_post, dim3(1), dim3(64), 0, c->stream, c->dscal + QD_S_ETA_MEAN, c->wsum_ocean);
                }
            }
            qd_mark(c, {T1, F[QD_F_ETA]}, m);
            double*& T1s = c->scratch[0];
            double* T2 = qd_scratch(c, 1);
            const int m2 = qd_plan(c, {QD_IN(T1s, 2), QD_IN(F[QD_F_QNET], 0), QD_IN8(c->icemask, 0), QD_IN(F[QD_F_UO], 1),
                                       QD_IN(F[QD_F_VO], 1), QD_IN(F[QD_F_ETA], 0)});
            if (m2 < 0) return -1;
            double* u2 = qd_scratch(c, 2); double* v2 = qd_scratch(c, 3);
            QD_ROWS(c, m2, G, hipLaunchKernelGGL(k_sst_outlier_fused, qd_grid2d(G), blk, 0, c->stream, G, c->tabs, c->dlat,
                                                 c->dlon, p.a, HP, c->scratch[0], T2, F[QD_F_QNET], c->land, c->icemask,
                                                 F[QD_F_UO], F[QD_F_VO], u2, v2, F[QD_F_ETA], p.ocean_max_u, p.eta_cap,
                                                 p.ocean_outlier == 0 ? 1 : 0,
                                                 has_ocean ? c->dscal + QD_S_ETA_MEAN : (const double*)nullptr,
                                                 c->red_partial, band_defer ? 0 : (band_raw_mean ? -1 : (int)(qd_grid2d(Gown).x * qd_grid2d(Gown).y)), c->wsum_ocean,
                                                 band_defer ? c->dscal + QD_S_TMP1 : (defer_eta ? c->dscal + QD_S_ETA_MEAN : (double*)nullptr)));
            qd_mark(c, {T2, u2, v2, F[QD_F_ETA]}, m2);
            if (band_defer) {
                if (qd_wait_host_flag(c, c->hpin + 41, c->eta_seq, "ocean sub-step: the eta sum never arrived")) return -1;
                double sum = c->hpin[40];
                if (qd_host_allreduce(c, &sum, 1, 0)) return -1;
                c->hpin[42] = sum / (c->wsum_ocean + 1e-15);
            }
            qd_swap(c, QD_F_SST, 1); qd_swap(c, QD_F_UO, 2); qd_swap(c, QD_F_VO, 3);
        } else {
        {
            QdScope sc(c, "ocean_continuity");
            const int m = qd_plan(c, {QD_IN(F[QD_F_UO], 1), QD_IN(F[QD_F_VO], 1), QD_IN(F[QD_F_ETA], 0)});
            if (m < 0) return -1;
            if (band && m > 0) {
                QdSegs S = qd_segments(c, m);
                for (int k = 0; k < S.n; ++k) {
                    QdGeom G = S.g[k];
                    const int own0 = c->own_row0, own1 = c->own_row0 + c->own_nrows;
                    int a0 = G.row0, a1 = G.row0 + G.nrows;
                    auto run = [&](int r0, int r1) {
                        if (r1 <= r0) return;
                        QdGeom g2 = G; g2.row0 = r0; g2.nrows = r1 - r0;
                        hipLaunchKernelGGL(k_continuity, dim3(1, g2.nrows), blk, 0, c->stream, g2, c->tabs, p.a, c->dlat, c->dlon,
                                           -sub_dt * H, F[QD_F_UO], F[QD_F_VO], c->land, F[QD_F_ETA],
                                           c->red_partial + (size_t)G0.lrows());
// ... 76 lines not shown
```

### qingdai_amd/csrc/qd_ocntail.h

```cpp
#pragma once
#include "qd_internal.h"
#include "qd_peer_dev.h"

struct QdTailArgs {
    const double *uo, *vo, *Ts, *qnet;
    const uint8_t *land, *ice;
    double *eta, *Ts_out, *uo_out, *vo_out, *partial;
    const double* tab;
    unsigned long long* acc;
    double* mean_out;
    double wsum;
    double a, dlat, dlon, sub_dt, msdtH, alpha, K_h, rcH, ice_qfac, cap;
    double r_a, r_dlon, r_dlat, r_2dlon, r_2dlat, r_rcH;
    int use_q, has_ice, mean4, ntc, R, Rp;
    int nmid, flags;
    int own0, own1;
    const double* eta_in = nullptr;
    unsigned int* fix_count = nullptr;
    unsigned long long* fix_list = nullptr;
    unsigned long long* acc_next = nullptr;
    unsigned long long* acc_clear = nullptr;
    QdPeerFold pf;
};

int qd_ocn_tail_tiles(const qd_ctx* c, const QdGeom& G);
int qd_launch_ocn_tail(qd_ctx* c, const QdGeom& G, QdTailArgs& P);
bool qd_ocn_tail_is_fast(const qd_ctx* c);

struct QdOcnArgs;
bool qd_ocn_fused_ok(const qd_ctx* c);
int qd_ocn_fused_tiles(const qd_ctx* c);
int qd_launch_ocn_fused(qd_ctx* c, const QdOcnArgs& O, QdTailArgs& P);
```

### qingdai_amd/csrc/qd_ocntail.hip

```cpp
#include "qd_internal.h"
#include "qd_device.h"
#include "qd_wave.h"
#include "qd_ocntail.h"
#include "qd_stream.h"
#include "qd_blockred.h"
#include <cstdlib>
#include <cstdio>
#include <vector>
#include <cstring>
#include <algorithm>


__device__ __forceinline__ double qt_div(double x, double c, double rc) {
    const double q0 = x * rc;
    const double e = __builtin_fma(-c, q0, x);
    const double q1 = __builtin_fma(e, rc, q0);
    return (q0 - q0 == 0.0) ? q1 : q0;
}

__device__ __forceinline__ double qt_div_fin(double x, double c, double rc) {
    const double q0 = x * rc;
    const double e = __builtin_fma(-c, q0, x);
    return __builtin_fma(e, rc, q0);
}
// ... 342 lines not shown
}
__device__ __forceinline__ double qfu_ring_ld(const double* plane, int row, int lane) { return plane[(row & (QFU_NR - 1)) * 64 + lane]; }

struct QtCurSlot { double u, v, e; int l; qt_f64x2 k0, k1; };
struct QtCurK { double dlon2, r_2dlon, dlat2, r_2dlat, msdtH, cap, cap81; int mean4; QtFixW fx = QtFixW{nullptr, nullptr, nullptr, nullptr}; };

template <bool RING = false, bool FIX = false>
__device__ __forceinline__ void qt_cur_fast_step(const QtCurK& P, const QtW& W, qt_rsrc U, qt_rsrc V, qt_rsrc E, qt_rsrc L,
                                                 qt_rsrc UO, qt_rsrc VO, qt_rsrc KT, double& us, double& uc, double& vs, double& vc, double& acc,
                                                 QtCurSlot& sl, int g, unsigned ro, const QfuRing* R = nullptr) {
    double un, vn, e0;
    if (RING) {
        qfu_wait_gt(R->prog + 0, g + 1); qfu_wait_gt(R->prog + 1, g + 1); qfu_wait_gt(R->prog + 2, g);
        un = qfu_ring_ld(R->u, g + 1, W.lane); vn = qfu_ring_ld(R->v, g + 1, W.lane); e0 = qfu_ring_ld(R->e, g, W.lane);
    } else { un = qs_own(sl.u); vn = qs_own(sl.v); e0 = sl.e; }
    const bool island = sl.l == 1;
    const double ue = qd_east(uc), uw = qd_west(uc), ve = qd_east(vc), vw = qd_west(vc);
    const double dp = qt_div(ue - uw, P.dlon2, P.r_2dlon);
    const double qn = vn * sl.k0.x;
    const double qs = vs * sl.k0.y;
    const double dq = qt_div(qn - qs, P.dlat2, P.r_2dlat);
    const double div = sl.k1.x * (dp + dq);
    double e = e0 + P.msdtH * div;
    if (island) e = 0.0;
    qt_st(E, ro, W.vs, e);
    acc += (W.own && g >= W.own0 && g < W.own1) ? e * (island ? 0.0 : sl.k1.y) : 0.0;
    double u = qd_nn(uc), v = qd_nn(vc);
    const double cap = P.cap, s2 = u * u + v * v;
    if (!(s2 < P.cap81)) {
        const double speed = sqrt(s2);
        if (P.mean4) {
            if (speed > cap) {
                u = 0.25 * (qd_nn(un) + qd_nn(us) + qd_nn(ue) + qd_nn(uw));
                v = 0.25 * (qd_nn(vn) + qd_nn(vs) + qd_nn(ve) + qd_nn(vw));
            }
            const double sp2 = sqrt(u * u + v * v);
            const double sc2 = (sp2 > cap) ? cap / (sp2 + 1e-12) : 1.0;
            u = u * sc2; v = v * sc2;
        } else {
            const double sc = (speed > cap) ? cap / (speed + 1e-12) : 1.0;
            u = u * sc; v = v * sc;
        }
    }
    qt_put_uv<FIX>(P.fx, UO, VO, ro, W.vs, u, v, uc, vc);
    us = uc; uc = un; vs = vc; vc = vn;
    if (RING) { if (W.lane == 0) __hip_atomic_store(R->prog + 3, g + 1, __ATOMIC_RELAXED, __HIP_MEMORY_SCOPE_WORKGROUP); }
    __builtin_amdgcn_sched_barrier(0);
    const unsigned r2 = ro + 2u * (unsigned)W.m;
    if (!RING) { sl.u = qt_ld(U, r2 + (unsigned)W.m, W.vo); sl.v = qt_ld(V, r2 + (unsigned)W.m, W.vo); sl.e = qt_ld(E, r2, W.vo); }
    sl.l = qt_ld8(L, r2, W.vo8);
    sl.k0 = qt_ldk(KT, 16u * (unsigned)(g + 2), 4u); sl.k1 = qt_ldk(KT, 16u * (unsigned)(g + 2), 5u);
    __builtin_amdgcn_sched_barrier(0);
}

template <bool FIX = false>
__device__ __forceinline__ double qt_currents_fast(const QdTailArgs& P, const QtW& W, const QtFixW& FX = QtFixW{nullptr, nullptr, nullptr, nullptr}) {
    const unsigned sb = W.slab, m = (unsigned)W.m;
    const qt_rsrc U = qt_make_rsrc(P.uo, sb), V = qt_make_rsrc(P.vo, sb), E = qt_make_rsrc(P.eta, sb), L = qt_make_rsrc(P.land, sb / 8u);
    const qt_rsrc UO = qt_make_rsrc(P.uo_out, sb), VO = qt_make_rsrc(P.vo_out, sb), KT = qt_make_rsrc(P.tab, (unsigned)W.n * 128u);
    unsigned ro = (unsigned)(W.o0 - W.lbase) * m;
    double us = qt_ld(U, ro - m, W.vo), vs = qt_ld(V, ro - m, W.vo);
    double uc = qt_ld(U, ro, W.vo), vc = qt_ld(V, ro, W.vo);
    double acc = 0.0;
    QtCurK K;
    K.dlon2 = qt_vreg(2 * P.dlon); K.r_2dlon = qt_vreg(P.r_2dlon); K.dlat2 = qt_vreg(2 * P.dlat); K.r_2dlat = qt_vreg(P.r_2dlat);
    K.msdtH = qt_vreg(P.msdtH); K.cap = qt_vreg(P.cap); K.cap81 = qt_vreg(0.81 * (P.cap * P.cap)); K.mean4 = P.mean4;
    if (FIX) K.fx = FX;
    QtCurSlot a, b;
    a.u = qt_ld(U, ro + m, W.vo); a.v = qt_ld(V, ro + m, W.vo); a.e = qt_ld(E, ro, W.vo); a.l = qt_ld8(L, ro, W.vo8);
    a.k0 = qt_ldk(KT, 16u * (unsigned)W.o0, 4u); a.k1 = qt_ldk(KT, 16u * (unsigned)W.o0, 5u);
    b.u = qt_ld(U, ro + 2u * m, W.vo); b.v = qt_ld(V, ro + 2u * m, W.vo); b.e = qt_ld(E, ro + m, W.vo); b.l = qt_ld8(L, ro + m, W.vo8);
    b.k0 = qt_ldk(KT, 16u * (unsigned)(W.o0 + 1), 4u); b.k1 = qt_ldk(KT, 16u * (unsigned)(W.o0 + 1), 5u);
    __builtin_amdgcn_s_waitcnt(0x0F70);
    int g = W.o0;
    for (; g + 1 < W.o1; g += 2) {
        qt_cur_fast_step<false, FIX>(K, W, U, V, E, L, UO, VO, KT, us, uc, vs, vc, acc, a, g, ro);
        qt_cur_fast_step<false, FIX>(K, W, U, V, E, L, UO, VO, KT, us, uc, vs, vc, acc, b, g + 1, ro + m);
        ro += 2u * m;
    }
    if (g < W.o1) qt_cur_fast_step<false, FIX>(K, W, U, V, E, L, UO, VO, KT, us, uc, vs, vc, acc, a, g, ro);
    return acc;
}

struct QtSstSlot { double u, v, s, q; int l, ic; qt_f64x2 k0, k1, k2; };
struct QtSstK { double a, r_a, dt, dlon, r_dlon, dlat, r_dlat, alpha, om_alpha, dtK, rcH, r_rcH, dtq; int has_ice, qfac_on; };

__device__ __forceinline__ double qt_shfl(double x, int src_lane) {
    const int lo = __builtin_amdgcn_ds_bpermute(src_lane << 2, __double2loint(x));
    const int hi = __builtin_amdgcn_ds_bpermute(src_lane << 2, __double2hiint(x));
    return __hiloint2double(hi, lo);
}

template <bool EDGE, bool OUT, bool RING = false>
__device__ __forceinline__ void qt_sst_fast_step(const QtSstK& K, const QtW& W, qt_rsrc U, qt_rsrc V, qt_rsrc S, qt_rsrc Q,
                                                 qt_rsrc L, qt_rsrc I, qt_rsrc SO, qt_rsrc KT, double& Tm, double& T0, double& Wm, double& W0, double& Em,
                                                 double& E0, double& w0, double& w1, double& w2, double& w3, double& w4, bool& bad,
                                                 QtSstSlot& sl, int g, unsigned ro, const QfuRing* R = nullptr) {
    const double Tp = qs_own(sl.s);
    double Wp = 0.0, Ep = 0.0;
    if (!EDGE) { Wp = qd_west(Tp); Ep = qd_east(Tp); }
    double u, v;
    if (RING) {
        qfu_wait_gt(R->prog + 0, g); qfu_wait_gt(R->prog + 1, g);
        u = qfu_ring_ld(R->u, g, W.lane); v = qfu_ring_ld(R->v, g, W.lane);
        if (W.lane == 0) __hip_atomic_store(R->prog + 4, g + 1, __ATOMIC_RELAXED, __HIP_MEMORY_SCOPE_WORKGROUP);
    } else { u = sl.u; v = sl.v; }
    const double acos = sl.k0.x, r_acos = sl.k0.y;
    const double dl = qt_div_fin(u * K.dt, acos, r_acos);
    const double dph = qt_div_fin(v * K.dt, K.a, K.r_a);
    const double dx = qt_div_fin(dl, K.dlon, K.r_dlon);
    const double dy = qt_div_fin(dph, K.dlat, K.r_dlat);
    const bool near = fabs(dx) < 1.0 && fabs(dy) < 1.0;
    bad = bad || (W.lane >= 1 && W.lane <= 62 && !near);
    const double r = (double)g - dy;
    double cc = (double)W.j - dx;
    if (EDGE) {
        const double sz = (double)(W.m - 1);
        cc = cc < 0.0 ? cc + sz * 1.0 : (cc > sz ? cc - sz * 1.0 : cc);
    }
    const double r0f = floor(r), c0f = floor(cc);
    const double tr = r - r0f, tc = cc - c0f;
    const bool pr = r0f < (double)g;
    double X_m, X_0, X_p, Y_m, Y_0, Y_p;
    if (EDGE) {
        const int c0 = (int)c0f;
        const int c1 = c0 + 1 < W.m ? c0 + 1 : W.m - 1;
        int l0 = c0 - W.jbase, l1 = c1 - W.jbase;
        l0 = l0 < 0 ? l0 + W.m : (l0 >= W.m ? l0 - W.m : l0);
        l1 = l1 < 0 ? l1 + W.m : (l1 >= W.m ? l1 - W.m : l1);
        l0 &= 63; l1 &= 63;
        X_m = qt_shfl(Tm, l0); X_0 = qt_shfl(T0, l0); X_p = qt_shfl(Tp, l0);
        Y_m = qt_shfl(Tm, l1); Y_0 = qt_shfl(T0, l1); Y_p = qt_shfl(Tp, l1);
    } else {
        const bool pc = c0f < (double)W.j;
        X_m = pc ? Wm : Tm; X_0 = pc ? W0 : T0; X_p = pc ? Wp : Tp;
        Y_m = pc ? Tm : Em; Y_0 = pc ? T0 : E0; Y_p = pc ? Tp : Ep;
    }
    QtGather q;
    q.f00 = pr ? X_m : X_0; q.f10 = pr ? X_0 : X_p; q.f01 = pr ? Y_m : Y_0; q.f11 = pr ? Y_0 : Y_p;
    q.wr0 = 1.0 - tr; q.wr1 = tr; q.wc0 = 1.0 - tc; q.wc1 = tc; q.nan_coord = false;
    const double t1v = qd_nn(K.om_alpha * T0 + K.alpha * qt_gather_use(q));
    Tm = T0; T0 = Tp;
    if (!EDGE) { Wm = W0; W0 = Wp; Em = E0; E0 = Ep; }
    w0 = w1; w1 = w2; w2 = w3; w3 = w4; w4 = t1v;
    if (OUT) {
        const double e = qd_east(w2), wst = qd_west(w2);
        const double Gb = sl.k1.x * (w4 - w2);
        const double Ga = sl.k1.y * (w2 - w0);
        const double d2 = (e - 2.0 * w2) + wst;
        const double lap = sl.k2.x * (Gb - Ga) + sl.k2.y * d2;
        double Tv = w2 + K.dtK * lap;
        const double heat = qt_div(sl.q, K.rcH, K.r_rcH);
        const bool ocean = sl.l == 0;
        const bool ic = K.has_ice && sl.ic != 0;
        if (ocean && !ic) Tv = Tv + K.dt * heat;
        if (K.qfac_on && ocean && ic) Tv = Tv + K.dtq * heat;
        qt_st(SO, ro - 2u * (unsigned)W.m, W.vs, qd_nn(Tv));
    }
    __builtin_amdgcn_sched_barrier(0);
    const unsigned r2 = ro + 2u * (unsigned)W.m;
    if (!RING) { sl.u = qt_ld(U, r2, W.vo); sl.v = qt_ld(V, r2, W.vo); }
    sl.s = qt_ld(S, r2 + (unsigned)W.m, W.vo);
    sl.q = qt_ld(Q, ro, W.vo); sl.l = qt_ld8(L, ro, W.vo8); sl.ic = qt_ld8(I, ro, W.vo8);
    sl.k0 = qt_ldk(KT, 16u * (unsigned)(g + 2), 0u); sl.k1 = qt_ldk(KT, 16u * (unsigned)(g + 2), 1u); sl.k2 = qt_ldk(KT, 16u * (unsigned)(g + 2), 2u);
    __builtin_amdgcn_sched_barrier(0);
}

template <bool EDGE>
__device__ __forceinline__ bool qt_sst_fast(const QdTailArgs& P, const QtW& W) {
    const unsigned sb = W.slab, m = (unsigned)W.m;
    const qt_rsrc U = qt_make_rsrc(P.uo, sb), V = qt_make_rsrc(P.vo, sb), S = qt_make_rsrc(P.Ts, sb), Q = qt_make_rsrc(P.qnet, sb);
    const qt_rsrc L = qt_make_rsrc(P.land, sb / 8u), I = qt_make_rsrc(P.ice, sb / 8u), SO = qt_make_rsrc(P.Ts_out, sb);
    const qt_rsrc KT = qt_make_rsrc(P.tab, (unsigned)W.n * 128u);
    QtSstK K;
    K.a = qt_vreg(P.a); K.r_a = qt_vreg(P.r_a); K.dt = qt_vreg(P.sub_dt); K.dlon = qt_vreg(P.dlon); K.r_dlon = qt_vreg(P.r_dlon);
    K.dlat = qt_vreg(P.dlat); K.r_dlat = qt_vreg(P.r_dlat); K.alpha = qt_vreg(P.alpha); K.om_alpha = qt_vreg(1.0 - P.alpha);
    K.dtK = qt_vreg(P.sub_dt * P.K_h); K.rcH = qt_vreg(P.rcH); K.r_rcH = qt_vreg(P.r_rcH); K.dtq = qt_vreg(P.sub_dt * P.ice_qfac);
    K.has_ice = P.has_ice; K.qfac_on = P.ice_qfac > 0.0 ? 1 : 0;
    const int t0 = W.o0 - 2;
    unsigned ro = (unsigned)(t0 - W.lbase) * m;
    double Tm = qt_ld(S, ro - m, W.vo), T0 = qt_ld(S, ro, W.vo);
    QtSstSlot a, b;
    a.u = qt_ld(U, ro, W.vo); a.v = qt_ld(V, ro, W.vo); a.s = qt_ld(S, ro + m, W.vo);
    a.k0 = qt_ldk(KT, 16u * (unsigned)t0, 0u); a.k1 = qt_ldk(KT, 16u * (unsigned)t0, 1u); a.k2 = qt_ldk(KT, 16u * (unsigned)t0, 2u);
    b.u = qt_ld(U, ro + m, W.vo); b.v = qt_ld(V, ro + m, W.vo); b.s = qt_ld(S, ro + 2u * m, W.vo);
    b.k0 = qt_ldk(KT, 16u * (unsigned)(t0 + 1), 0u); b.k1 = qt_ldk(KT, 16u * (unsigned)(t0 + 1), 1u); b.k2 = qt_ldk(KT, 16u * (unsigned)(t0 + 1), 2u);
    a.q = b.q = 0.0; a.l = b.l = 0; a.ic = b.ic = 0;
    __builtin_amdgcn_s_waitcnt(0x0F70);
    double Wm = 0.0, W0 = 0.0, Em = 0.0, E0 = 0.0;
    if (!EDGE) { Wm = qd_west(Tm); W0 = qd_west(T0); Em = qd_east(Tm); E0 = qd_east(T0); }
    double w0 = 0.0, w1 = 0.0, w2 = 0.0, w3 = 0.0, w4 = 0.0;
    bool bad = false;
#define QT_FS(OUTF, SL, GG, RO) qt_sst_fast_step<EDGE, OUTF>(K, W, U, V, S, Q, L, I, SO, KT, Tm, T0, Wm, W0, Em, E0, w0, w1, w2, w3, w4, bad, SL, GG, RO)
    int g = t0;
    QT_FS(false, a, g, ro); QT_FS(false, b, g + 1, ro + m); QT_FS(false, a, g + 2, ro + 2u * m); QT_FS(false, b, g + 3, ro + 3u * m);
    g += 4; ro += 4u * m;
    const int gend = W.o1 + 2;
    for (; g + 1 < gend; g += 2) { QT_FS(true, a, g, ro); QT_FS(true, b, g + 1, ro + m); ro += 2u * m; }
    if (g < gend) QT_FS(true, a, g, ro);
#undef QT_FS
    return __builtin_amdgcn_ballot_w64(bad) != 0ull;
}

template <bool FIX>
__global__ void __launch_bounds__(128)
k_ocn_tail_fast(QdGeom G, QdTabs T, QdTailArgs P) {
    const unsigned w = qd_xcd_chunk(blockIdx.x, gridDim.x);
    const int rs = (int)(w / (unsigned)P.ntc), cs = (int)(w % (unsigned)P.ntc);
    QtW W;
    W.n = G.nlat; W.m = G.nlon; W.lane = threadIdx.x & 63;
    W.jbase = cs * QS_TCF - 2;
    const int jraw = W.jbase + W.lane;
    W.j = jraw < 0 ? jraw + W.m : (jraw >= W.m ? jraw - W.m : jraw);
    W.own = W.lane >= 2 && W.lane <= QS_TCF + 1 && jraw < W.m;
    W.vo = (unsigned)W.j * 8u; W.vo8 = (unsigned)W.j; W.vs = W.own ? (unsigned)jraw * 8u : 0x80000000u;
    W.slab = (unsigned)(G.lrows_ + QD_PAD_ROWS) * (unsigned)G.nlon * 8u;
    W.lbase = G.lbase; W.lrows = G.lrows_; W.own0 = P.own0; W.own1 = P.own1;
    const int lo = G.row0, hi = G.row0 + G.nrows;
    const QtPart q = qt_partition(lo, hi, G.nlat, P.R, P.Rp);
    const int k = rs - (q.ps > 0 ? 1 : 0);
    if (q.ps > 0 && rs == 0) { W.o0 = lo; W.o1 = lo + q.ps; }
    else if (k < q.nmid) {
        const int M = q.mid1 - q.mid0;
        W.o0 = q.mid0 + (int)(((long long)k * M) / q.nmid);
        W.o1 = q.mid0 + (int)(((long long)(k + 1) * M) / q.nmid);
    } else { W.o0 = q.mid1; W.o1 = hi; }
    const int wv = __builtin_amdgcn_readfirstlane(threadIdx.x >> 6);
    const bool plain = (P.flags & 1) == 0 && W.o0 - 3 - W.lbase >= 0 && W.o1 + 2 - W.lbase <= W.lrows - 1;
    QT_STAMP(0);
    if (wv >= 1) {
        __builtin_amdgcn_s_setprio(2);
        bool general = !(plain && W.o0 >= 3 && W.o1 <= W.n - 3 && P.use_q && P.K_h > 0.0);
        if (!general) {
            const bool edge_lane = W.lane >= 1 && W.lane <= 62 && (W.j == 0 || W.j == W.m - 1);
            general = __builtin_amdgcn_ballot_w64(edge_lane) != 0ull ? qt_sst_fast<true>(P, W) : qt_sst_fast<false>(P, W);
        }
        if (general) qt_sst_wave(G, T, P, W);
        QT_STAMP(2);
        if (!FIX) return;
        __syncthreads();
        return;
    }
    __shared__ unsigned long long s_fix[FIX ? 3 * QT_FIX_STAGE : 1];
    __shared__ unsigned int s_nfix;
    const QtFixW FX{P.fix_count, P.fix_list, s_fix, &s_nfix};
    if (FIX && W.lane == 0) __hip_atomic_store(&s_nfix, 0u, __ATOMIC_RELAXED, __HIP_MEMORY_SCOPE_WAVEFRONT);
    double acc = (plain && W.o0 >= 1 && W.o1 <= W.n - 1) ? qt_currents_fast<FIX>(P, W, FX) : qt_currents_wave<FIX>(T, P, W, FX);
    if (FIX) qt_fix_flush(FX);
    QT_STAMP(2);
    if (FIX) __syncthreads();
    acc = qd_wave_sum(acc);
    if (W.lane == 0) __hip_atomic_store(P.partial + w, acc, __ATOMIC_RELAXED, __HIP_MEMORY_SCOPE_AGENT);
    if (!FIX && P.acc_clear && w == 0u) qd_acc_clear_set(P.acc_clear);
    if (!FIX && P.acc_next) {
        if (W.lane == 0) qd_acc_add(P.acc_next, w, acc);
        return;
    }
    if (P.acc) {
        const bool last = W.lane == 0 && qd_acc_arrive(P.acc, w, gridDim.x, acc);
        if (__builtin_amdgcn_ballot_w64(last) != 0ull) {
            double mm = qd_acc_finish(P.acc, P.partial, (int)gridDim.x, P.wsum);
            if (P.pf.pbox) mm = qp_fold_sum(P.pf, mm);
            if (W.lane == 0) *P.mean_out = mm;
            if (FIX) {
                const unsigned nfix = __hip_atomic_load(P.fix_count, __ATOMIC_RELAXED, __HIP_MEMORY_SCOPE_AGENT);
                for (unsigned k0 = 0; k0 < nfix; k0 += 512u) {
                    unsigned long long off[8], ub[8], vb[8];
#pragma unroll
                    for (int q = 0; q < 8; ++q) {
                        const unsigned k = k0 + (unsigned)q * 64u + (unsigned)W.lane;
                        const unsigned long long* e = P.fix_list + (size_t)3 * (k < nfix ? k : nfix - 1u);
                        off[q] = __hip_atomic_load(e, __ATOMIC_RELAXED, __HIP_MEMORY_SCOPE_AGENT);
                        ub[q] = __hip_atomic_load(e + 1, __ATOMIC_RELAXED, __HIP_MEMORY_SCOPE_AGENT);
                        vb[q] = __hip_atomic_load(e + 2, __ATOMIC_RELAXED, __HIP_MEMORY_SCOPE_AGENT);
                    }
#pragma unroll
                    for (int q = 0; q < 8; ++q) {
                        if (k0 + (unsigned)q * 64u + (unsigned)W.lane >= nfix) continue;
                        *(unsigned long long*)((char*)const_cast<double*>(P.uo) + off[q]) = ub[q];
                        *(unsigned long long*)((char*)const_cast<double*>(P.vo) + off[q]) = vb[q];
                    }
                }
                if (W.lane == 0) {
                    __hip_atomic_store(P.fix_count, 0u, __ATOMIC_RELAXED, __HIP_MEMORY_SCOPE_AGENT);
                    P.fix_count[4] += nfix; P.fix_count[5] += 1u; if (nfix > P.fix_count[6]) P.fix_count[6] = nfix;
                }
            }
        }
    }
}

#define QFU_TC 56
#define QFU_PH 7
typedef double __attribute__((address_space(3)))* qfu_ldp;
typedef int __attribute__((address_space(3)))* qfu_lip;
struct QfuArgs { int ntc, nmid, R, mode; };

struct QsOutRing {
    double* plane; int* prod; const int* c3; const int* c4; int row, chk, lane;
    __device__ __forceinline__ void put(double v) {
        if (row >= chk) {
            for (;;) {
                const int a = __hip_atomic_load(c3, __ATOMIC_RELAXED, __HIP_MEMORY_SCOPE_WORKGROUP);
                const int b = __hip_atomic_load(c4, __ATOMIC_RELAXED, __HIP_MEMORY_SCOPE_WORKGROUP);
                if (row + 3 - (a < b ? a : b) < QFU_NR) break;
                __builtin_amdgcn_s_sleep(1);
            }
            chk = row + 4;
        }
        plane[(row & (QFU_NR - 1)) * 64 + lane] = v;
        asm volatile("s_waitcnt lgkmcnt(0)" ::: "memory");
        if (lane == 0) __hip_atomic_store(prod, row + 1, __ATOMIC_RELAXED, __HIP_MEMORY_SCOPE_WORKGROUP);
        ++row;
    }
};

__device__ __forceinline__ void qfu_k1w(const QdGeom& G, int cs, int k0, int k1, QsW& W) {
    W.n = G.nlat; W.nlon = G.nlon; W.lane = threadIdx.x & 63;
    const int jraw = cs * QFU_TC - 4 + W.lane;
    W.j = jraw < 0 ? jraw + G.nlon : (jraw >= G.nlon ? jraw - G.nlon : jraw);
    W.vo = (unsigned)W.j * 8u; W.vo8 = (unsigned)W.j;
    W.vs = (W.lane >= 3 && W.lane <= 60) ? (unsigned)W.j * 8u : QS_OOB;
    W.slab_bytes = (unsigned)(G.lrows_ + QD_PAD_ROWS) * (unsigned)G.nlon * 8u;
    W.west_edge = W.j == 0; W.east_edge = W.j == G.nlon - 1;
    W.o0 = k0; W.o1 = k1;
}
__device__ __forceinline__ void qfu_tailw(const QdGeom& G, const QdTailArgs& P, int cs, int o0, int o1, QtW& W) {
    W.n = G.nlat; W.m = G.nlon; W.lane = threadIdx.x & 63;
    W.jbase = cs * QFU_TC - 4;
    const int jraw = W.jbase + W.lane;
// ... 185 lines not shown
    QsOcnArgs A;
    if (!qd_stream_ocn_args(c, O, A)) return qd_fail(c, "k_ocn_fused: coefficient row tables");
    A.G = c->geo;
    if (F.ntc * (1 + F.nmid) > c->red_blocks) return qd_fail(c, "k_ocn_fused: partial buffer too small");
    if (!c->qt_tab || c->qt_tab_a != P.a) {
        if (!c->qt_tab) {
            if (hipMalloc(&c->qt_tab, (size_t)c->geo.nlat * 16 * sizeof(double)) != hipSuccess) return qd_fail(c, "k_ocn_fused: row table");
            c->tab_alloc.push_back(c->qt_tab);
        }
        hipLaunchKernelGGL(k_tail_tab, dim3((c->geo.nlat + 255) / 256), dim3(256), 0, c->stream, c->tabs, c->geo.nlat, P.a, c->qt_tab);
        c->qt_tab_a = P.a;
    }
    P.tab = c->qt_tab; P.own0 = 0; P.own1 = c->geo.nlat; P.flags = 0; P.R = F.R; P.Rp = QFU_PH; P.ntc = F.ntc; P.nmid = F.nmid;
    QdScope sc(c, "ocean_step", true);
#ifdef QT_STAMPS
    static unsigned long long* stamps = nullptr;
    const size_t stamp_words = (size_t)8 * 5 * 8192;
    if (!stamps) { hipMalloc(&stamps, stamp_words * 8); hipMemcpyToSymbol(HIP_SYMBOL(qt_stamp_buf), &stamps, sizeof(stamps)); }
    hipMemsetAsync(stamps, 0, stamp_words * 8, c->stream);
#endif
    QD_LAUNCH_TIMED(sc, k_ocn_fused, dim3(F.ntc * (1 + F.nmid)), dim3(320), c->stream, A, c->tabs, P, F);
#ifdef QT_STAMPS
    if (const char* f = std::getenv("QD_STAMPS_FILE")) {
        std::vector<unsigned long long> h(stamp_words);
        hipStreamSynchronize(c->stream);
        hipMemcpy(h.data(), stamps, stamp_words * 8, hipMemcpyDeviceToHost);
        if (FILE* fp = std::fopen(f, "wb")) { std::fwrite(h.data(), 8, stamp_words, fp); std::fclose(fp); }
    }
#endif
    return 0;
}

static int qt_rows(const qd_ctx* c) { return c->tune.tail_r > 0 ? c->tune.tail_r : 7; }

static bool qt_use_fast(const qd_ctx* c) { return !c->tune.tail_v && c->ocn_tail == 1; }
bool qd_ocn_tail_is_fast(const qd_ctx* c) { return qt_use_fast(c); }
static int qt_fast_rows(const qd_ctx* c, const QdGeom& G) {
    if (c->tune.tail_r > 0) return c->tune.tail_r;
    const int ntc = (G.nlon + QS_TCF - 1) / QS_TCF;
    const double target = 13.7 * 256;
    const int r = (int)std::lround((double)G.nrows * ntc * 2.0 / target);
    return r < 7 ? 7 : r;
}
static int qt_fast_pole_rows(const qd_ctx* c) { return c->tune.tail_rp; }

int qd_ocn_tail_tiles(const qd_ctx* c, const QdGeom& G) {
    if (qt_use_fast(c))
        return qt_part_strips(qt_partition(G.row0, G.row0 + G.nrows, G.nlat, qt_fast_rows(c, G), qt_fast_pole_rows(c))) * ((G.nlon + QS_TCF - 1) / QS_TCF);
    const int R = qt_rows(c);
    return ((G.nrows + R - 1) / R) * ((G.nlon + QS_TC2 - 1) / QS_TC2);
}

int qd_launch_ocn_tail(qd_ctx* c, const QdGeom& G, QdTailArgs& P) {
    if (G.nlon < 64) return qd_fail(c, "k_ocn_tail: >= 64 columns");
    if (G.full) { P.own0 = 0; P.own1 = G.nlat; }
    QdScope sc(c, "ocean_tail", true);
    const bool fast = qt_use_fast(c);
    if (fast && (!c->qt_tab || c->qt_tab_a != P.a)) {
        if (!c->qt_tab) {
            if (hipMalloc(&c->qt_tab, (size_t)G.nlat * 16 * sizeof(double)) != hipSuccess) return qd_fail(c, "k_ocn_tail_fast: row table");
            c->tab_alloc.push_back(c->qt_tab);
        }
        hipLaunchKernelGGL(k_tail_tab, dim3((G.nlat + 255) / 256), dim3(256), 0, c->stream, c->tabs, G.nlat, P.a, c->qt_tab);
        c->qt_tab_a = P.a;
    }
    P.tab = c->qt_tab;
    P.flags = c->tune.tail_general ? 1 : 0;
    P.R = fast ? qt_fast_rows(c, G) : qt_rows(c);
    P.Rp = qt_fast_pole_rows(c);
    P.ntc = fast ? (G.nlon + QS_TCF - 1) / QS_TCF : (G.nlon + QS_TC2 - 1) / QS_TC2;
    const QtPart part = qt_partition(G.row0, G.row0 + G.nrows, G.nlat, P.R, P.Rp);
    P.nmid = part.nmid;
    const int nrs = fast ? qt_part_strips(part) : (G.nrows + P.R - 1) / P.R;
    if (nrs * P.ntc > c->red_blocks) return qd_fail(c, "k_ocn_tail_stream: partial buffer too small");
#ifdef QT_STAMPS
    static unsigned long long* stamps = nullptr;
    const size_t stamp_words = (size_t)8 * 2 * 8192;
    if (!stamps) { hipMalloc(&stamps, stamp_words * 8); hipMemcpyToSymbol(HIP_SYMBOL(qt_stamp_buf), &stamps, sizeof(stamps)); }
    hipMemsetAsync(stamps, 0, stamp_words * 8, c->stream);
#endif
    if ((P.acc_next || P.acc_clear) && (!fast || P.fix_count || !G.full))
        return qd_fail(c, "k_ocn_tail: the mean of a sub-step can only be left to the next launch by the storing fast form");
    if (!fast || !P.acc) { P.fix_count = nullptr; P.fix_list = nullptr; }
    if (fast && P.fix_count) QD_LAUNCH_TIMED(sc, k_ocn_tail_fast<true>, dim3(nrs * P.ntc), dim3(128), c->stream, G, c->tabs, P);
    else if (fast) QD_LAUNCH_TIMED(sc, k_ocn_tail_fast<false>, dim3(nrs * P.ntc), dim3(128), c->stream, G, c->tabs, P);
    else QD_LAUNCH_TIMED(sc, k_ocn_tail_stream<1>, dim3(nrs * P.ntc), dim3(128), c->stream, G, c->tabs, P);
#ifdef QT_STAMPS
    if (const char* f = std::getenv("QD_STAMPS_FILE")) {
        std::vector<unsigned long long> h(stamp_words);
        hipStreamSynchronize(c->stream);
        hipMemcpy(h.data(), stamps, stamp_words * 8, hipMemcpyDeviceToHost);
        if (FILE* fp = std::fopen(f, "wb")) { std::fwrite(h.data(), 8, stamp_words, fp); std::fclose(fp); }
    }
#endif
    return 0;
}
```

### qingdai_amd/csrc/qd_stream.h

```cpp
#pragma once
#include "qd_internal.h"
#include "qd_device.h"
#include "qd_fused.h"
#include "qd_wave.h"

#ifndef QS_STAMP
#define QS_STAMP(k) ((void)0)
#endif

#define QS_TC 58

struct QsRec { const double* in; const double* aux; double* out; const double* tab; int skip; int pad_; };

struct QsDynArgs {
    QdGeom G;
    const double *poleA, *c8, *c9;
    const double *h, *fric;
    double dt, inv_dlon, inv_2dlon, inv_dlat, inv_2dlat, pgf_y;
    int vb, ntc, nrs, exact;
    QsRec rec[5];
};

struct QsOcnArgs {
    QdGeom G;
    const double *poleA, *fcor, *igx, *rx;
    const double *uo, *vo, *eta;
    const uint8_t* land;
    const double* eta_mean;
    double eta_cap, sub_dt, g, r_bot, inv_2dlon, inv_2dlat, inv_a, inv_rhoH;
    int vb, ntc, nrs, exact;
    QsRec rec[3];
    const unsigned long long* acc_read = nullptr;
    const double* acc_partial = nullptr;
    int acc_n = 0;
    double acc_wsum = 0.0;
};

typedef unsigned int qs_u32x2 __attribute__((ext_vector_type(2)));
typedef __amdgpu_buffer_rsrc_t qs_rsrc;
#define QS_RSRC_FLAGS 0x00020000
#define QS_OOB 0x80000000u

__device__ __forceinline__ qs_rsrc qs_make_rsrc(const void* p, unsigned bytes) {
    return __builtin_amdgcn_make_buffer_rsrc(const_cast<void*>(p), 0, (int)bytes, QS_RSRC_FLAGS);
}
__device__ __forceinline__ double qs_ld(qs_rsrc r, unsigned row, unsigned vo) {
    return __builtin_bit_cast(double, __builtin_amdgcn_raw_buffer_load_b64(r, vo, row * 8u, 0));
}
__device__ __forceinline__ void qs_st(qs_rsrc r, unsigned row, unsigned vo, double v) {
    __builtin_amdgcn_raw_buffer_store_b64(__builtin_bit_cast(qs_u32x2, v), r, vo, row * 8u, 0);
}
__device__ __forceinline__ int qs_ld8(qs_rsrc r, unsigned row, unsigned vo8) {
    return (int)__builtin_amdgcn_raw_buffer_load_b8(r, vo8, row, 0);
}

__device__ __forceinline__ unsigned qs_off(const QdGeom& G, int g) {
    g = qd_clampi(g, 0, G.nlat - 1);
    int l = qd_lrow(G, g);
    l = l < G.lrows_ ? l : G.lrows_ - 1;
    return (unsigned)l * (unsigned)G.nlon;
}
__device__ __forceinline__ unsigned qs_off_roll(const QdGeom& G, int g) {
    if (g < 0) g += G.nlat; else if (g >= G.nlat) g -= G.nlat;
    return qs_off(G, g);
}

#ifndef QS_PD_DYN
#define QS_PD_DYN 4
#endif
#ifndef QS_PD_OCN
#define QS_PD_OCN 2
#endif

struct QsW {
    int n, nlon, lane, j, o0, o1;
    unsigned vo, vs, vo8;
    unsigned slab_bytes;
    bool west_edge, east_edge;
};

enum { QS_FAST = 0, QS_EXACT = 2 };

template <int V> __device__ __forceinline__ double qs_clip200(double x, bool& bad) {
    if (V == QS_EXACT) return qd_clip(x, -200.0, 200.0);
    bad |= qd_nonfinite(x);
    return fmin(fmax(x, -200.0), 200.0);
}


__device__ __forceinline__ double qs_own(double x) {
#if QS_OWN_ASM
    double y;
    asm("v_mov_b64 %0, %1" : "=v"(y) : "v"(x));
    return y;
#else
    const int lo = __builtin_amdgcn_update_dpp(0, __double2loint(x), 0xE4, 0xf, 0xf, true);
    const int hi = __builtin_amdgcn_update_dpp(0, __double2hiint(x), 0xE4, 0xf, 0xf, true);
    return __hiloint2double(hi, lo);
#endif
}

template <int V, int PD> struct QsSrcPlain {
    qs_rsrc p; const QdGeom& G; const QsW& W; double q[PD]; unsigned ro;
    __device__ __forceinline__ void start(int g0, bool&) {
        ro = qs_off(G, g0);
#pragma unroll
        for (int k = 0; k < PD; ++k) { q[k] = qs_ld(p, ro, W.vo); ro += W.nlon; }
    }
    __device__ __forceinline__ void settle(bool&) {}
    template <int K> __device__ __forceinline__ double get(int, bool&) { return qs_own(q[K % PD]); }
    template <int K> __device__ __forceinline__ double get_edge(int g, bool& bad) { return get<K>(g, bad); }
    template <int K> __device__ __forceinline__ void refill() { q[K % PD] = qs_ld(p, ro, W.vo); ro += W.nlon; }
};

template <bool PRIM, int V, int PD> struct QsSrcLat {
    const QsDynArgs& A; const QsW& W;
    qs_rsrc H, FR, X, Y;
    double hm, hc, hq[PD], x[PD], y[PD], fr[PD];
    unsigned ro;
// ... 339 lines not shown
        }
    }
    return bad;
}

__host__ __device__ __forceinline__ int qs_cut(int nrows, int nrs, int vb, int rs) {
    return rs >= nrs ? nrows : (int)(((long long)rs * (nrows + vb)) / nrs);
}
__device__ __forceinline__ void qs_strip(const QdGeom& G, int vb, int ntc, int nrs, QsW& W, unsigned bid, unsigned nb) {
    const unsigned w = qd_xcd_chunk(bid, nb);
    const int rs = (int)(w / (unsigned)ntc), cs = (int)(w % (unsigned)ntc);
    W.n = G.nlat; W.nlon = G.nlon;
    W.lane = threadIdx.x & 63;
    const int jraw = cs * QS_TC - 3 + W.lane;
    W.j = jraw < 0 ? jraw + G.nlon : (jraw >= G.nlon ? jraw - G.nlon : jraw);
    const bool col_ok = W.lane >= 3 && W.lane <= 60 && jraw < G.nlon;
    W.vo = (unsigned)W.j * 8u; W.vo8 = (unsigned)W.j; W.vs = col_ok ? (unsigned)jraw * 8u : QS_OOB;
#ifdef QS_NOSTORE
    W.vs = QS_OOB;
#endif
    W.slab_bytes = (unsigned)(G.lrows_ + QD_PAD_ROWS) * (unsigned)G.nlon * 8u;
    W.west_edge = W.j == 0; W.east_edge = W.j == G.nlon - 1;
    W.o0 = G.row0 + qs_cut(G.nrows, nrs, vb, rs);
    W.o1 = G.row0 + qs_cut(G.nrows, nrs, vb, rs + 1);
}
__device__ __forceinline__ void qs_strip(const QdGeom& G, int vb, int ntc, int nrs, QsW& W) { qs_strip(G, vb, ntc, nrs, W, blockIdx.x, gridDim.x); }

template <bool PRIM, int V>
__device__ __forceinline__ bool qs_dyn_wave(const QsDynArgs& A, const QsW& W, int wv) {
    const QsDynArgs QD_CONST* Ak = (const QsDynArgs QD_CONST*)__builtin_amdgcn_kernarg_segment_ptr();
    const QsRec QD_CONST* fp = &Ak->rec[wv];
    const unsigned sb = W.slab_bytes;
    QsOutGlobal out{qs_make_rsrc(fp->out, sb), qs_off(A.G, W.o0), W.vs, (unsigned)W.nlon};
    if (wv <= 1) {
        const qs_rsrc H = qs_make_rsrc(A.h, sb), FR = qs_make_rsrc(A.fric, sb), X = qs_make_rsrc(fp->in, sb), Y = qs_make_rsrc(fp->aux, sb);
        if ((wv == 0) == PRIM) {
            if (__builtin_amdgcn_ballot_w64(W.west_edge || W.east_edge) != 0ull) {
                QsSrcLon<PRIM, V, QS_PD_DYN, true> S{A, W, H, FR, X, Y};
                return qs_del4_stream<V>(S, A.G, W, A.poleA, fp, A.dt, out);
            }
            QsSrcLon<PRIM, V, QS_PD_DYN, false> S{A, W, H, FR, X, Y};
            return qs_del4_stream<V>(S, A.G, W, A.poleA, fp, A.dt, out);
        }
        QsSrcLat<PRIM, V, QS_PD_DYN> S{A, W, H, FR, X, Y};
        return qs_del4_stream<V>(S, A.G, W, A.poleA, fp, A.dt, out);
    }
    QsSrcPlain<V, QS_PD_DYN> S{qs_make_rsrc(fp->in, sb), A.G, W};
    return qs_del4_stream<V>(S, A.G, W, A.poleA, fp, A.dt, out);
}

template <int V, class OUT>
__device__ __forceinline__ bool qs_ocn_wave(const QsOcnArgs& A, const QsW& W, int wv, const QsRec QD_CONST* fp, OUT& out,
                                            double* sy = nullptr, double* em_io = nullptr) {
    const bool handover = em_io != nullptr && A.acc_read != nullptr;
    const bool defer = handover || A.eta_mean != nullptr;
    const double em = handover ? *em_io : (defer ? *A.eta_mean : 0.0);
    if (!handover) sy = nullptr;
    const double cap = (V == QS_EXACT || defer) ? A.eta_cap : __builtin_inf();
    const unsigned sb = W.slab_bytes;
    const qs_rsrc E = qs_make_rsrc(A.eta, sb);
    bool bad;
    if (wv <= 1) {
        const qs_rsrc U = qs_make_rsrc(A.uo, sb), Vv = qs_make_rsrc(A.vo, sb), T = qs_make_rsrc(fp->aux, sb), L = qs_make_rsrc(A.land, sb / 8u);
        if (wv == 0) {
            QsSrcOcnU<V, QS_PD_OCN> S{A, W, E, U, Vv, T, L, defer, em, cap};
            S.sy = sy;
            bad = qs_del4_stream<V>(S, A.G, W, A.poleA, fp, A.sub_dt, out);
            if (handover) *em_io = S.em;
            return bad;
        }
        QsSrcOcnV<V, QS_PD_OCN> S{A, W, E, U, Vv, T, L, defer, em, cap};
        S.sy = sy;
        bad = qs_del4_stream<V>(S, A.G, W, A.poleA, fp, A.sub_dt, out);
        if (handover) *em_io = S.em;
        return bad;
    }
    QsSrcEta<V, QS_PD_OCN> S{A, W, E, defer, em, cap};
    S.sy = sy;
    bad = qs_del4_stream<V>(S, A.G, W, A.poleA, fp, A.sub_dt, out);
    if (handover) *em_io = S.em;
    return bad;
}


const double* qd_stream_tables(qd_ctx* c, int kind, int nf, const double* const* k4row, const double* k4s, const int* skip);
bool qd_stream_ocn_args(qd_ctx* c, const QdOcnArgs& P, QsOcnArgs& A);
```

### qingdai_amd/csrc/qd_stream.hip

```cpp
#include "qd_internal.h"
#include <cstdlib>
#include <cstdio>
#include <vector>
#include <algorithm>

#ifdef QS_STAMPS
__device__ unsigned long long* qs_stamp_buf;
__device__ __forceinline__ void qs_stamp(int slot) {
    if ((threadIdx.x & 63) == 0) {
        const unsigned wid = blockIdx.x * (blockDim.x >> 6) + (threadIdx.x >> 6);
        qs_stamp_buf[(size_t)wid * 8 + slot] = __builtin_amdgcn_s_memrealtime();
        if (slot == 0) {
            unsigned hw, xcc;
            asm volatile("s_getreg_b32 %0, hwreg(HW_REG_HW_ID)" : "=s"(hw));
            asm volatile("s_getreg_b32 %0, hwreg(HW_REG_XCC_ID)" : "=s"(xcc));
            qs_stamp_buf[(size_t)wid * 8 + 4] = hw; qs_stamp_buf[(size_t)wid * 8 + 5] = xcc;
        }
    }
}
#define QS_STAMP(k) qs_stamp(k)
#endif

#include "qd_stream.h"
#include "qd_band.h"

template <bool PRIM>
__global__ void __launch_bounds__(320)
k_dyn_stream(QsDynArgs A) {
    QsW W;
    qs_strip(A.G, A.vb, A.ntc, A.nrs, W);
    const int wv = __builtin_amdgcn_readfirstlane(threadIdx.x >> 6);
    if (wv <= 1) __builtin_amdgcn_s_setprio(2);
    QS_STAMP(0);
    if (!A.exact) {
        const bool bad = qs_dyn_wave<PRIM, QS_FAST>(A, W, wv);
        QS_STAMP(2);
        if (__builtin_amdgcn_ballot_w64(bad) == 0ull) return;
    }
    qs_dyn_wave<PRIM, QS_EXACT>(A, W, wv);
}

__global__ void __launch_bounds__(192)
k_ocn_stream(QsOcnArgs A) {
    QsW W;
    qs_strip(A.G, A.vb, A.ntc, A.nrs, W);
    const int wv = __builtin_amdgcn_readfirstlane(threadIdx.x >> 6);
    if (wv <= 1) __builtin_amdgcn_s_setprio(2);
    const QsOcnArgs QD_CONST* Ak = (const QsOcnArgs QD_CONST*)__builtin_amdgcn_kernarg_segment_ptr();
    const QsRec QD_CONST* fp = &Ak->rec[wv];
    __shared__ double s_em;
    double em = 0.0;
    if (!A.exact) {
        QsOutGlobal out{qs_make_rsrc(fp->out, W.slab_bytes), qs_off(A.G, W.o0), W.vs, (unsigned)W.nlon};
        const bool bad = qs_ocn_wave<QS_FAST>(A, W, wv, fp, out, &s_em, &em);
        if (__builtin_amdgcn_ballot_w64(bad) == 0ull) return;
    }
    QsOutGlobal out{qs_make_rsrc(fp->out, W.slab_bytes), qs_off(A.G, W.o0), W.vs, (unsigned)W.nlon};
    qs_ocn_wave<QS_EXACT>(A, W, wv, fp, out, A.exact ? &s_em : (double*)nullptr, &em);
}

static int qs_wgs_per_cu(qd_ctx* c, int which) {
    if (c->qs_wgs_per_cu[which] > 0) return c->qs_wgs_per_cu[which];
    int nb = 0;
    hipError_t e = hipSuccess;
    if (which == 0) e = hipOccupancyMaxActiveBlocksPerMultiprocessor(&nb, k_dyn_stream<false>, 320, 0);
    else if (which == 1) e = hipOccupancyMaxActiveBlocksPerMultiprocessor(&nb, k_dyn_stream<true>, 320, 0);
    else e = hipOccupancyMaxActiveBlocksPerMultiprocessor(&nb, k_ocn_stream, 192, 0);
    if (e != hipSuccess || nb < 1) nb = which == 2 ? 6 : 4;
    c->qs_wgs_per_cu[which] = nb;
    return nb;
}

struct QsShape { int R, nrs, vb; };
static QsShape qs_shape(qd_ctx* c, int nrows, int nlon, int which, bool north_pole) {
    const int ntc = (nlon + QS_TC - 1) / QS_TC;
    int R = 0;
    R = which == 2 ? c->tune.stream_r_ocn : c->tune.stream_r_dyn;
    if (R <= 0) R = c->stream_rows;
    int nrs;
    if (R > 0) nrs = std::max(1, nrows / std::max(R, 5));
    else {
        const long target = which == 2 ? 1000 : 760;
        nrs = (int)std::max(1L, (target + ntc / 2) / ntc);
    }
    nrs = std::max(1, std::min(nrs, nrows / 12));
    int vb = 0;
    if (north_pole && nrs > 1) {
        vb = 6;
        if (c->tune.stream_vb >= 0) vb = c->tune.stream_vb;
        while (vb > 0 && nrows - qs_cut(nrows, nrs, vb, nrs - 1) < 12) --vb;
    }
    return QsShape{(nrows + nrs - 1) / nrs, nrs, vb};
}

static int host_lrow(const QdGeom& G, int g) {
    int l = g - G.lbase;
    if (l < 0) l += G.nlat; else if (l >= G.nlat) l -= G.nlat;
    return l;
}

static bool qs_segments_ok(const qd_ctx* c, int margin) {
    QdSegs S = qd_segments(const_cast<qd_ctx*>(c), margin);
    for (int k = 0; k < S.n; ++k) {
        const QdGeom& G = S.g[k];
        const int s0 = G.row0, s1 = G.row0 + G.nrows;
        if ((s0 > 0 && s0 < 5) || (s1 < G.nlat && s1 > G.nlat - 5) || G.nrows < 10) return false;
    }
    return true;
}

bool qd_stream_ok(const qd_ctx* c, int margin) {
    return c->fused_fast >= 1 && c->fused_fast <= 2 && c->geo.nlon >= 64 && c->geo.nlat >= 12 &&
           (size_t)(c->geo.lrows_ + QD_PAD_ROWS) * (size_t)c->geo.nlon * 8u < 0x7fffffffull &&
           qs_segments_ok(c, margin);
}

const double* qd_stream_tables(qd_ctx* c, int kind, int nf, const double* const* k4row, const double* k4s, const int* skip) {
    const int nlat = c->geo.nlat;
    double key[8] = {1.0, 0, 0, 0, 0, 0, 0, 0};
    for (int f = 0; f < nf; ++f) key[1 + f] = (k4row[f] || skip[f]) ? 0.0 : k4s[f];
    bool same = c->qs_tab[kind] != nullptr && c->qs_key[kind][0] == 1.0;
    for (int f = 0; same && f < nf; ++f) same = c->qs_key[kind][1 + f] == key[1 + f] || (key[1 + f] != key[1 + f] && c->qs_key[kind][1 + f] != c->qs_key[kind][1 + f]);
    if (same) return c->qs_tab[kind];
    if (c->h_lapK[kind].size() != (size_t)nlat * 4) return nullptr;
    std::vector<double> t((size_t)nf * nlat * 4);
    for (int f = 0; f < nf; ++f)
        for (int r = 0; r < nlat; ++r) {
            double* o = &t[((size_t)f * nlat + r) * 4];
            o[0] = c->h_lapK[kind][4 * r + 1]; o[1] = c->h_lapK[kind][4 * r + 2]; o[2] = c->h_lapK[kind][4 * r + 3];
            o[3] = k4row[f] ? (c->h_k4[kind].size() == (size_t)nf * nlat ? c->h_k4[kind][(size_t)f * nlat + r] : 0.0) : k4s[f];
        }
    if (!c->qs_tab[kind] && hipMalloc(&c->qs_tab[kind], (size_t)5 * nlat * 4 * sizeof(double)) != hipSuccess) return nullptr;
    if (hipMemcpyAsync(c->qs_tab[kind], t.data(), t.size() * sizeof(double), hipMemcpyHostToDevice, c->stream) != hipSuccess) return nullptr;
    hipStreamSynchronize(c->stream);
    for (int k = 0; k < 8; ++k) c->qs_key[kind][k] = key[k];
    return c->qs_tab[kind];
}

int qd_launch_dyn_stream(qd_ctx* c, const QdDynArgs& P, int margin) {
    QsDynArgs A;
    A.poleA = c->tabs.lapPoleA[0];
    A.c8 = P.primitive ? c->tabs.mom_px : c->tabs.mom_cu;
    A.c9 = P.primitive ? c->tabs.fcor : c->tabs.mom_cv;
    A.h = P.h; A.fric = P.fric;
    const double* tab = qd_stream_tables(c, 0, 5, P.k4row, P.k4s, P.skip);
    if (!tab) return qd_fail(c, "fused kernel: coefficient row tables");
    const double* in[5] = {P.u, P.v, P.h, P.q, P.cloud};
    const double* aux[5] = {P.v, P.u, nullptr, nullptr, nullptr};
    double* out[5] = {P.uo, P.vo, P.ho, P.qo, P.co};
    for (int f = 0; f < 5; ++f) A.rec[f] = QsRec{in[f], aux[f], out[f], tab + (size_t)f * c->geo.nlat * 4, P.skip[f], 0};
    A.dt = P.dt; A.inv_dlon = P.inv_dlon; A.inv_2dlon = P.inv_2dlon; A.inv_dlat = P.inv_dlat; A.inv_2dlat = P.inv_2dlat; A.pgf_y = P.pgf_y;
    A.exact = c->fused_fast == 2;
    QdScope sc(c, "k_dyn_hyper", c->geo.full != 0);
#ifdef QS_STAMPS
    static unsigned long long* stamps = nullptr;
    const size_t stamp_words = (size_t)8 * 5 * 4096;
    if (!stamps) { hipMalloc(&stamps, stamp_words * 8); hipMemcpyToSymbol(HIP_SYMBOL(qs_stamp_buf), &stamps, sizeof(stamps)); }
    hipMemsetAsync(stamps, 0, stamp_words * 8, c->stream);
#endif
    QD_ROWS(c, margin, G,
            const QsShape sh = qs_shape(c, G.nrows, G.nlon, P.primitive ? 1 : 0, G.row0 + G.nrows == G.nlat);
            A.G = G; A.vb = sh.vb; A.nrs = sh.nrs; A.ntc = (G.nlon + QS_TC - 1) / QS_TC;
            if (P.primitive) QD_LAUNCH_TIMED(sc, k_dyn_stream<true>, dim3(A.nrs * A.ntc), dim3(320), c->stream, A);
            else QD_LAUNCH_TIMED(sc, k_dyn_stream<false>, dim3(A.nrs * A.ntc), dim3(320), c->stream, A));
#ifdef QS_STAMPS
    if (const char* f = std::getenv("QD_STAMPS_FILE")) {
        std::vector<unsigned long long> h(stamp_words);
        hipStreamSynchronize(c->stream);
        hipMemcpy(h.data(), stamps, stamp_words * 8, hipMemcpyDeviceToHost);
        if (FILE* fp = std::fopen(f, "wb")) { std::fwrite(h.data(), 8, stamp_words, fp); std::fclose(fp); }
    }
#endif
    return 0;
}

bool qd_ocn_stream_ok(const qd_ctx* c, int margin) {
    if (!qd_stream_ok(c, margin)) return false;
    if (c->geo.full) return true;
    QdSegs S = qd_segments(const_cast<qd_ctx*>(c), margin);
    for (int k = 0; k < S.n; ++k) {
        const QdGeom& G = S.g[k];
        const bool pole = G.row0 == 0 || G.row0 + G.nrows == G.nlat;
        if (pole && !(host_lrow(G, 0) < G.lrows_ && host_lrow(G, G.nlat - 1) < G.lrows_)) return false;
    }
    return true;
}

bool qd_stream_ocn_args(qd_ctx* c, const QdOcnArgs& P, QsOcnArgs& A) {
    A.poleA = c->tabs.lapPoleA[1];
    A.fcor = c->tabs.fcor; A.igx = c->tabs.ocn_igx; A.rx = c->tabs.r_extra;
    A.uo = P.uo; A.vo = P.vo; A.eta = P.eta; A.land = P.land;
    const double* tab = qd_stream_tables(c, 1, 3, P.k4row, P.k4s, P.skip);
    if (!tab) return false;
    const double* in[3] = {P.uo, P.vo, P.eta};
    const double* aux[3] = {P.taux, P.tauy, nullptr};
    double* out[3] = {P.uo_out, P.vo_out, P.eta_out};
    for (int f = 0; f < 3; ++f) A.rec[f] = QsRec{in[f], aux[f], out[f], tab + (size_t)f * c->geo.nlat * 4, P.skip[f], 0};
    A.eta_mean = P.eta_mean; A.eta_cap = P.eta_cap; A.sub_dt = P.sub_dt; A.g = P.g; A.r_bot = P.r_bot;
    A.inv_2dlon = P.inv_2dlon; A.inv_2dlat = P.inv_2dlat; A.inv_a = P.inv_a; A.inv_rhoH = P.inv_rhoH;
    A.exact = c->fused_fast == 2;
    A.vb = 0; A.ntc = 0; A.nrs = 0;
    return true;
}

static bool qs_seg_ok(const QdGeom& G) {
    const int s0 = G.row0, s1 = G.row0 + G.nrows;
    return !((s0 > 0 && s0 < 5) || (s1 < G.nlat && s1 > G.nlat - 5) || G.nrows < 10);
}
bool qd_ocn_stream_ok_list(const qd_ctx* c, const QdSegList& S) {
    if (!(c->fused_fast >= 1 && c->fused_fast <= 2 && c->geo.nlon >= 64 && c->geo.nlat >= 12 &&
          (size_t)(c->geo.lrows_ + QD_PAD_ROWS) * (size_t)c->geo.nlon * 8u < 0x7fffffffull)) return false;
    for (int k = 0; k < S.n; ++k) {
        const QdGeom& G = S.g[k];
        if (!qs_seg_ok(G)) return false;
        const bool pole = G.row0 == 0 || G.row0 + G.nrows == G.nlat;
        if (!c->geo.full && pole && !(host_lrow(G, 0) < G.lrows_ && host_lrow(G, G.nlat - 1) < G.lrows_)) return false;
    }
    return S.n > 0;
}

int qd_launch_ocn_stream_list(qd_ctx* c, const QdOcnArgs& P, const QdSegList& S) {
    QsOcnArgs A;
    if (!qd_stream_ocn_args(c, P, A)) return qd_fail(c, "fused kernel: coefficient row tables");
    if (S.n == 2 && !c->tune.stream_no_pair && !qd_peer_job_waiting(c)) {
        const QsShape s0 = qs_shape(c, S.g[0].nrows, S.g[0].nlon, 2, S.g[0].row0 + S.g[0].nrows == S.g[0].nlat);
        const QsShape s1 = qs_shape(c, S.g[1].nrows, S.g[1].nlon, 2, S.g[1].row0 + S.g[1].nrows == S.g[1].nlat);
        A.G = S.g[0]; A.vb = s0.vb; A.nrs = s0.nrs; A.ntc = (S.g[0].nlon + QS_TC - 1) / QS_TC;
        qd_launch_ocn_stream_pair(c, A, S.g[1], s1.vb, s1.nrs, (S.g[1].nlon + QS_TC - 1) / QS_TC);
        return 0;
    }
    for (int k = 0; k < S.n; ++k) {
        const QdGeom& G = S.g[k];
        const QsShape sh = qs_shape(c, G.nrows, G.nlon, 2, G.row0 + G.nrows == G.nlat);
        A.G = G; A.vb = sh.vb; A.nrs = sh.nrs; A.ntc = (G.nlon + QS_TC - 1) / QS_TC;
        if (!qd_launch_ocn_stream_push(c, A)) hipLaunchKernelGGL(k_ocn_stream, dim3(A.nrs * A.ntc), dim3(192), 0, c->stream, A);
    }
    return 0;
}

int qd_launch_ocn_stream(qd_ctx* c, const QdOcnArgs& P, int margin) {
    QsOcnArgs A;
    A.poleA = c->tabs.lapPoleA[1];
    A.fcor = c->tabs.fcor; A.igx = c->tabs.ocn_igx; A.rx = c->tabs.r_extra;
    A.uo = P.uo; A.vo = P.vo; A.eta = P.eta; A.land = P.land;
    const double* tab = qd_stream_tables(c, 1, 3, P.k4row, P.k4s, P.skip);
    if (!tab) return qd_fail(c, "fused kernel: coefficient row tables");
    const double* in[3] = {P.uo, P.vo, P.eta};
    const double* aux[3] = {P.taux, P.tauy, nullptr};
    double* out[3] = {P.uo_out, P.vo_out, P.eta_out};
    for (int f = 0; f < 3; ++f) A.rec[f] = QsRec{in[f], aux[f], out[f], tab + (size_t)f * c->geo.nlat * 4, P.skip[f], 0};
    A.eta_mean = P.eta_mean; A.eta_cap = P.eta_cap; A.sub_dt = P.sub_dt; A.g = P.g; A.r_bot = P.r_bot;
    A.acc_read = P.acc_read; A.acc_partial = P.acc_partial; A.acc_n = P.acc_n; A.acc_wsum = P.acc_wsum;
    A.inv_2dlon = P.inv_2dlon; A.inv_2dlat = P.inv_2dlat; A.inv_a = P.inv_a; A.inv_rhoH = P.inv_rhoH;
    A.exact = c->fused_fast == 2;
    QdScope sc(c, "k_ocn_hyper", c->geo.full != 0);
    QD_ROWS(c, margin, G,
            const QsShape sh = qs_shape(c, G.nrows, G.nlon, 2, G.row0 + G.nrows == G.nlat);
            A.G = G; A.vb = sh.vb; A.nrs = sh.nrs; A.ntc = (G.nlon + QS_TC - 1) / QS_TC;
            QD_LAUNCH_TIMED(sc, k_ocn_stream, dim3(A.nrs * A.ntc), dim3(192), c->stream, A));
    return 0;
}
```

### qingdai_amd/device.py

```python
from __future__ import annotations

import ctypes

import numpy as np

from . import _lib
from ._lib import F, QdError
from .params import QdParams


def _c(a, dtype=np.float64):
    return np.ascontiguousarray(a, dtype=dtype)


class Device:
    _history_n = 0
    _tiles_n = 1
    _div_shape = None

    def __init__(self, grid, params: QdParams | None = None, device=0, row0=0, n_rows=None, halo=0, rank=0, world=1):
        self.lib = _lib.load()
        self.grid = grid
        self.params = params or QdParams.from_env()
        self.shape = (grid.n_lat, grid.n_lon)
# ... 460 lines not shown
    def _tile_refs(refs):
        arr = (_lib.qd_tile_ref * max(1, len(refs)))()
        for k, (src, idx) in enumerate(refs):
            arr[k].source, arr[k].index = (_lib.TILE[src] if isinstance(src, str) else int(src)), int(idx)
        return arr

    def tiles_scan(self, refs):
        self.flush()
        n = len(refs)
        out = np.empty((max(1, n), 4), dtype=np.float64)
        cells = (ctypes.c_int64 * max(1, n))()
        self._chk(self.lib.qd_tiles_scan(self.h, self._tile_refs(refs), n, out.ctypes.data_as(ctypes.POINTER(ctypes.c_double)), cells), "qd_tiles_scan")
        return [{"min": float(out[k, 0]), "max": float(out[k, 1]), "nan": bool(out[k, 2] > 0.0), "argmax": int(cells[k]),
                 "argmax_value": float(out[k, 3])} for k in range(n)]

    def tiles_order_stats(self, source, index, ranks):
        self.flush()
        r = (ctypes.c_int64 * max(1, len(ranks)))(*[int(x) for x in ranks])
        vals = np.full(max(1, len(ranks)), np.nan, dtype=np.float64)
        count = ctypes.c_int64(-1)
        self._chk(self.lib.qd_tiles_order_stats(self.h, _lib.TILE[source] if isinstance(source, str) else int(source), int(index), r, len(ranks),
                                                vals.ctypes.data_as(ctypes.POINTER(ctypes.c_double)), ctypes.byref(count)), "qd_tiles_order_stats")
        return int(count.value), vals[:len(ranks)]

    def tiles_render(self, tiles, want_stacks=False):
        self.flush()
        n = len(tiles)
        arr = (_lib.qd_tile_desc * max(1, n))(*tiles)
        self._chk(self.lib.qd_tiles_render(self.h, arr, ctypes.sizeof(_lib.qd_tile_desc), n, 1 if want_stacks else 0), "qd_tiles_render")
        self._tiles_n = n

    def tiles_image(self):
        g, n = _lib.STATEFRAME_GUTTER, self._tiles_n
        out = np.empty((self.shape[0] + 2 * g, n * self.shape[1] + (n + 1) * g, 3), dtype=np.uint8)
        self._chk(self.lib.qd_tiles_download(self.h, 0, out.ctypes.data, out.size), "qd_tiles_download")
        return out

    def tiles_bands(self):
        out = np.empty((self._tiles_n,) + self.shape, dtype=np.int8)
        self._chk(self.lib.qd_tiles_download(self.h, 1, out.ctypes.data, out.size), "qd_tiles_download")
        return out

    def tiles_planes(self):
        out = np.empty((self._tiles_n,) + self.shape, dtype=np.float64)
        self._chk(self.lib.qd_tiles_download(self.h, 2, out.ctypes.data, out.size), "qd_tiles_download")
        return out

    def phyto_configure(self, n_species, K_h, adv_alpha):
        self._chk(self.lib.qd_phyto_configure(self.h, int(n_species), float(K_h), float(adv_alpha)), "qd_phyto_configure")
        self._phyto_S = int(n_species)

    def phyto_upload(self, C_s):
        C_s = np.ascontiguousarray(C_s, dtype=np.float64)
        assert C_s.ndim == 3 and C_s.shape[0] == getattr(self, "_phyto_S", -1) and C_s.shape[1:] == self.shape
        for s in range(C_s.shape[0]):
            self._chk(self.lib.qd_phyto_upload(self.h, s, C_s[s].ctypes.data), "qd_phyto_upload")

    def phyto_download(self):
        self.flush()
        out = np.zeros((self._phyto_S,) + self.shape, dtype=np.float64)
        for s in range(self._phyto_S):
            self._chk(self.lib.qd_phyto_download(self.h, s, out[s].ctypes.data), "qd_phyto_download")
        return out

    def phyto_advect_diffuse(self, dt_seconds):
        self.flush()
        self._chk(self.lib.qd_phyto_advect_diffuse(self.h, float(dt_seconds)), "qd_phyto_advect_diffuse")

    def last_ocean_nsub(self):
        n = ctypes.c_int(0)
        self.lib.qd_last_ocean_nsub(self.h, ctypes.byref(n))
        return n.value

    def step_scalars(self):
        out = np.zeros(8)
        self._chk(self.lib.qd_step_scalars(self.h, out.ctypes.data_as(ctypes.POINTER(ctypes.c_double))), "qd_step_scalars")
        return dict(zip(("PREF", "ETA_MEAN", "MED_OUT", "PSCALE", "RENORM", "BLEND_W", "TMP0", "TMP1"), out))

    def ocean_mean_next_count(self):
        n = ctypes.c_int64(0)
        self._chk(self.lib.qd_ocean_mean_next_count(self.h, ctypes.byref(n)), "qd_ocean_mean_next_count")
        return n.value

    def counters(self):
        a, o = ctypes.c_int64(0), ctypes.c_int64(0)
        self.lib.qd_get_step_counter(self.h, ctypes.byref(a), ctypes.byref(o))
        return a.value, o.value

    def set_counters(self, a, o):
        self.lib.qd_set_step_counter(self.h, int(a), int(o))

    def digest(self, names):
        self.flush()
        refs = _c([_lib.state_ref(n) for n in names], np.int32)
        out = np.zeros(refs.size, dtype=np.uint64)
        for k in range(0, int(refs.size), _lib.STATE_DIGEST_MAX):
            r, o = refs[k:k + _lib.STATE_DIGEST_MAX], out[k:k + _lib.STATE_DIGEST_MAX]
            self._chk(self.lib.qd_state_digest(self.h, int(r.size), r.ctypes.data_as(ctypes.POINTER(ctypes.c_int32)),
                                               o.ctypes.data_as(ctypes.POINTER(ctypes.c_uint64))), "qd_state_digest")
        return out

    def state_scalars(self):
        out = np.zeros(_lib.STATE_SCALARS_N, dtype=np.float64)
        self._chk(self.lib.qd_state_scalars_get(self.h, out.ctypes.data_as(ctypes.POINTER(ctypes.c_double)), int(out.size)), "qd_state_scalars_get")
        return out

    def set_state_scalars(self, values):
        v = _c(values)
        self._chk(self.lib.qd_state_scalars_set(self.h, v.ctypes.data_as(ctypes.POINTER(ctypes.c_double)), int(v.size)), "qd_state_scalars_set")

    def route_restore(self, buffer, flow, lakes, steps):
        dp = ctypes.POINTER(ctypes.c_double)
        b, f = _c(buffer).ravel(), _c(flow).ravel()
        lk = None if lakes is None or np.size(lakes) == 0 else _c(lakes).ravel()
        if b.size != self._route_n[0] or f.size != self._route_n[0] or (0 if lk is None else lk.size) != self._route_n[1]:
            raise ValueError("route_restore: the arrays do not have the configured network's cell and lake counts")
        self._chk(self.lib.qd_route_restore(self.h, b.ctypes.data_as(dp), f.ctypes.data_as(dp), None if lk is None else lk.ctypes.data_as(dp),
                                            int(steps)), "qd_route_restore")

    def history_restore(self, sums, count):
        a = _c(sums)
        if a.shape != (self._history_n,) + self.shape:
            raise ValueError(f"history_restore: expected sums of shape {(self._history_n,) + self.shape}, got {a.shape}")
        self._chk(self.lib.qd_history_restore(self.h, a.ctypes.data_as(ctypes.POINTER(ctypes.c_double)), int(count)), "qd_history_restore")

    def reduce(self, name, op):
        self.flush()
        out = ctypes.c_double(0.0)
        self._chk(self.lib.qd_reduce(self.h, F[name], int(op), ctypes.byref(out)), "qd_reduce")
        return out.value

    def timing(self, on=True, select=None):
        if select:
            self.lib.qd_timing_select(self.h, select.encode())
        else:
            self.lib.qd_timing_enable(self.h, 1 if on else 0)
        self.lib.qd_timing_reset(self.h)

    def timing_get(self, name):
        ms, n = ctypes.c_double(0), ctypes.c_int64(0)
        self.lib.qd_timing_get(self.h, name.encode(), ctypes.byref(ms), ctypes.byref(n))
        return ms.value, n.value

    def _out(self):
        return np.empty(self.shape, dtype=np.float64)

    def op_laplacian(self, Fh, ocean=False):
        a, out = _c(Fh), self._out()
        self._chk(self.lib.qd_op_laplacian(self.h, a.ctypes.data, 1 if ocean else 0, out.ctypes.data), "qd_op_laplacian")
        return out

    def op_hyperdiffuse(self, Fh, k4, dt, n_substeps=1, ocean=False):
        a, out = _c(Fh), self._out()
        if np.isscalar(k4):
            rc = self.lib.qd_op_hyperdiffuse(self.h, a.ctypes.data, None, float(k4), float(dt), int(n_substeps),
                                             1 if ocean else 0, out.ctypes.data)
        else:
            k = np.asarray(k4, dtype=np.float64)
            if k.ndim == 2:
                if not np.all(k == k[:, :1]):
                    raise ValueError("k4 map must be a function of latitude only")
                k = k[:, 0]
            k = _c(k)
            rc = self.lib.qd_op_hyperdiffuse(self.h, a.ctypes.data, k.ctypes.data, 0.0, float(dt), int(n_substeps),
                                             1 if ocean else 0, out.ctypes.data)
        self._chk(rc, "qd_op_hyperdiffuse")
# ... 56 lines not shown
```

Before: 5.085 planet-days/s.

## Skip ocean stencil work on tiles that are entirely deep land

```diff
diff --git a/include/qingdai_hip.h b/include/qingdai_hip.h
--- a/include/qingdai_hip.h
+++ b/include/qingdai_hip.h
@@ -103,6 +103,8 @@
 int qd_median_state(qd_handle h, double* out64);
 int qd_step_scalars(qd_handle h, double* out8);
 int qd_ocean_mean_next_count(qd_handle h, int64_t* out);
+int qd_ocean_land_skip_counts(qd_handle h, int64_t* out2);
+int qd_ocean_land_skip_tally(qd_handle h, int64_t* out3);
 
 int qd_band_insolation(qd_handle h, int nb, const double* specA, const double* specB, const double* tray, double* out_host_or_null);
 
diff --git a/qingdai_amd/_lib.py b/qingdai_amd/_lib.py
--- a/qingdai_amd/_lib.py
+++ b/qingdai_amd/_lib.py
@@ -25,7 +25,7 @@
     "qd_get_step_counter", "qd_set_step_counter", "qd_forcing", "qd_simple_albedo", "qd_atmos_step",
     "qd_ocean_step", "qd_driver_physics", "qd_hydrology_commit", "qd_step_n", "qd_last_ocean_nsub", "qd_sync",
     "qd_op_laplacian", "qd_op_hyperdiffuse", "qd_op_advect", "qd_op_shapiro", "qd_op_zonal_filter", "qd_op_divergence",
-    "qd_op_vorticity", "qd_op_gaussian", "qd_op_median_positive", "qd_median_state", "qd_step_scalars", "qd_ocean_mean_next_count", "qd_reduce", "qd_energy_diagnostics", "qd_energy_diagnostics_last", "qd_band_insolation",
+    "qd_op_vorticity", "qd_op_gaussian", "qd_op_median_positive", "qd_median_state", "qd_step_scalars", "qd_ocean_mean_next_count", "qd_ocean_land_skip_counts", "qd_ocean_land_skip_tally", "qd_reduce", "qd_energy_diagnostics", "qd_energy_diagnostics_last", "qd_band_insolation",
     "qd_comm_unique_id", "qd_comm_init", "qd_comm_init_local", "qd_comm_stats", "qd_comm_allreduce_count", "qd_comm_grouped_sum_count", "qd_comm_init_shm", "qd_comm_host_allreduce_count", "qd_hostring_open", "qd_hostring_allreduce",
     "qd_hostring_close", "qd_comm_barrier", "qd_comm_allreduce_max", "qd_peer_export", "qd_peer_connect", "qd_comm_peer_stats", "qd_comm_peer_carried", "qd_peer_selftest", "qd_peer_disable", "qd_tune_reload",
     "qd_plansim_create", "qd_plansim_destroy", "qd_plansim_plan", "qd_plansim_mark", "qd_plansim_margin", "qd_plansim_segments",
@@ -292,6 +292,8 @@
     lib.qd_median_state.argtypes = [vp, dp]
     lib.qd_step_scalars.argtypes = [vp, dp]
     lib.qd_ocean_mean_next_count.argtypes = [vp, ctypes.POINTER(i64)]
+    lib.qd_ocean_land_skip_counts.argtypes = [vp, ctypes.POINTER(i64)]
+    lib.qd_ocean_land_skip_tally.argtypes = [vp, ctypes.POINTER(i64)]
     lib.qd_comm_stats.argtypes = [vp, ctypes.POINTER(i32)]
     lib.qd_comm_allreduce_count.argtypes = [vp, ctypes.POINTER(i32)]
     lib.qd_comm_grouped_sum_count.argtypes = [vp, ctypes.POINTER(i32)]
diff --git a/qingdai_amd/csrc/qd_api.hip b/qingdai_amd/csrc/qd_api.hip
--- a/qingdai_amd/csrc/qd_api.hip
+++ b/qingdai_amd/csrc/qd_api.hip
@@ -317,6 +317,7 @@
     { const char* ef = std::getenv("QD_FUSED_FAST"); if (ef) c->fused_fast = std::atoi(ef); }
     { const char* ef = std::getenv("QD_TAIL_ACC"); if (ef) c->tail_acc = std::atoi(ef); }
     { const char* ef = std::getenv("QD_MEAN_IN_MOMENTUM"); if (ef) c->mean_in_momentum = ef[0] == '0' ? 0 : 1; }
+    { const char* ef = std::getenv("QD_OCN_LAND_SKIP"); if (ef) c->ocn_land_skip = ef[0] == '0' ? 0 : 1; }
     { const char* ef = std::getenv("QD_SHAPIRO_STREAM"); if (ef) c->shapiro_stream = std::atoi(ef); }
     { const char* ef = std::getenv("QD_OCN_TAIL"); if (ef) c->ocn_tail = std::atoi(ef); }
     if (c->ocn_tail != 0) c->ocn_tail = 1;
@@ -367,6 +368,11 @@
         hipMemsetAsync(c->fix_count, 0, 64, c->stream);
         if ((e = hipMalloc(&c->fix_list, c->geo.cells() * 3 * sizeof(unsigned long long))) != hipSuccess) return bail("hipMalloc", e);
     }
+    { const char* ef = std::getenv("QD_OCN_LAND_SKIP_TALLY");
+      if (ef && ef[0] == '1') {
+          if ((e = hipMalloc(&c->land_tally, 4 * sizeof(unsigned))) != hipSuccess) return bail("hipMalloc", e);
+          hipMemsetAsync(c->land_tally, 0, 4 * sizeof(unsigned), c->stream);
+      } }
     if (!full) {
         if ((e = hipMalloc(&c->med_pred, 64 * sizeof(double))) != hipSuccess) return bail("hipMalloc", e);
         hipMemsetAsync(c->med_pred, 0, 64 * sizeof(double), c->stream);
@@ -459,6 +465,8 @@
     for (int s = 0; s < QD_NSCRATCH; ++s) if (c->scratch[s]) hipFree(c->scratch[s]);
     for (double* t : c->tab_alloc) hipFree(t);
     if (c->land) hipFree(c->land); if (c->icemask) hipFree(c->icemask);
+    for (int k = 0; k < 2; ++k) if (c->land_skip[k].d) hipFree(c->land_skip[k].d);
+    if (c->land_tally) hipFree(c->land_tally);
     if (c->k4_atm) hipFree(c->k4_atm); if (c->k4_ocn) hipFree(c->k4_ocn); for (int k = 0; k < 2; ++k) if (c->qs_tab[k]) hipFree(c->qs_tab[k]);
     if (c->red_partial) hipFree(c->red_partial); if (c->dscal) hipFree(c->dscal);
     if (c->red_partial_b) hipFree(c->red_partial_b);
@@ -545,6 +553,8 @@
             ws += w * cnt;
         }
         c->wsum_ocean = ws;
+        if (c->geo.full) c->h_land.assign(m, m + n);
+        c->land_gen++;
     }
     return 0;
 }
@@ -859,6 +869,23 @@
     return 0;
 }
 
+extern "C" int qd_ocean_land_skip_counts(qd_handle c, int64_t* out) {
+    if (!c || !out) return -1;
+    out[0] = c->land_skip_last[0]; out[1] = c->land_skip_last[1];
+    return 0;
+}
+
+extern "C" int qd_ocean_land_skip_tally(qd_handle c, int64_t* out) {
+    if (!c || !out) return -1;
+    if (!c->land_tally) return qd_fail(c, "qd_ocean_land_skip_tally: the handle was created without QD_OCN_LAND_SKIP_TALLY=1");
+    hipSetDevice(c->desc.device);
+    unsigned h[4] = {0, 0, 0, 0};
+    QD_HIP(c, hipStreamSynchronize(c->stream));
+    QD_HIP(c, hipMemcpy(h, c->land_tally, sizeof(h), hipMemcpyDeviceToHost));
+    for (int k = 0; k < 3; ++k) out[k] = h[k];
+    return 0;
+}
+
 extern "C" int qd_ocean_mean_next_count(qd_handle c, int64_t* out) {
     if (!c || !out) return -1;
     *out = c->mean_next_count;
diff --git a/qingdai_amd/csrc/qd_fused.h b/qingdai_amd/csrc/qd_fused.h
--- a/qingdai_amd/csrc/qd_fused.h
+++ b/qingdai_amd/csrc/qd_fused.h
@@ -32,6 +32,7 @@
     const double* acc_partial = nullptr;
     int acc_n = 0;
     double acc_wsum = 0.0;
+    int may_skip_land = 0;
 };
 
 
@@ -45,3 +46,5 @@
 int qd_launch_ocn_stream(qd_ctx* c, const QdOcnArgs& P, int margin);
 bool qd_ocn_stream_ok_list(const qd_ctx* c, const QdSegList& S);
 int qd_launch_ocn_stream_list(qd_ctx* c, const QdOcnArgs& P, const QdSegList& S);
+bool qd_land_skip_lookup(qd_ctx* c, int which, const int (&key)[6], const int** flags, int* count);
+int qd_land_skip_build(qd_ctx* c, int which, const int (&key)[6], const std::vector<int>& cuts, int tc);
diff --git a/qingdai_amd/csrc/qd_internal.h b/qingdai_amd/csrc/qd_internal.h
--- a/qingdai_amd/csrc/qd_internal.h
+++ b/qingdai_amd/csrc/qd_internal.h
@@ -244,6 +244,12 @@
     int fused_fast = 1;
     long long mean_next_count = 0;
     int mean_in_momentum = 1;
+    int ocn_land_skip = 1;
+    std::vector<uint8_t> h_land;
+    long long land_gen = 0;
+    struct QdLandSkip { int* d = nullptr; int cap = 0, n = 0, count = 0; long long gen = -1; int key[6] = {0, 0, 0, 0, 0, 0}; std::vector<unsigned> bits; } land_skip[2];
+    unsigned* land_tally = nullptr;
+    int land_skip_last[2] = {0, 0};
     int tail_acc = 1;
     unsigned long long* eta_acc = nullptr;
     int shapiro_stream = 1;
diff --git a/qingdai_amd/csrc/qd_ocean.hip b/qingdai_amd/csrc/qd_ocean.hip
--- a/qingdai_amd/csrc/qd_ocean.hip
+++ b/qingdai_amd/csrc/qd_ocean.hip
@@ -822,8 +822,11 @@
                               p.ocean_k4_nsub == 1 && !do_shap && qd_ocn_tail_is_fast(c) && qd_ocn_stream_ok(c, 0);
     if (mean_form_ok) fix_now = false;
     const bool mean_next_ok = mean_form_ok;
+    const bool land_skip_ok = c->ocn_land_skip && !band && G0.full && tail_acc && !use_fused1 && do_diff && c->use_fused &&
+                              p.ocean_k4_nsub == 1 && !do_shap && qd_ocn_tail_is_fast(c) && qd_ocn_stream_ok(c, 0);
     unsigned long long* acc_pending = nullptr;
     for (int s = 0; s < n_sub; ++s) {
+        c->land_skip_last[0] = c->land_skip_last[1] = 0;
         if (use_fused1) {
             QdOcnArgs O;
             O.uo = F[QD_F_UO]; O.vo = F[QD_F_VO]; O.eta = F[QD_F_ETA]; O.taux = taux; O.tauy = tauy; O.land = c->land;
@@ -875,6 +878,7 @@
             O.eta_mean = (defer_eta && s > 0) ? mean_ptr : nullptr;
             O.eta_cap = p.eta_cap;
             if (acc_pending) { O.acc_read = acc_pending; O.acc_partial = c->red_partial; O.acc_n = qd_ocn_tail_tiles(c, Gown); O.acc_wsum = c->wsum_ocean; }
+            O.may_skip_land = land_skip_ok ? 1 : 0;
             int m_int = 0;
             bool split = false;
             if (pending) {
@@ -968,6 +972,7 @@
             acc_pending = (mean_next_ok && s + 1 < n_sub) ? QD_ACC_NEXT_SET(c->eta_acc, s & 1) : nullptr;
             A.acc_next = acc_pending;
             if (acc_pending) c->mean_next_count++;
+            A.may_skip_land = land_skip_ok ? 1 : 0;
             if (qd_launch_ocn_tail(c, Gown, A)) return -1;
             if (!tail_acc)
                 hipLaunchKernelGGL(k_eta_mean_tail, dim3(1), dim3(256), 0, c->stream, c->red_partial, qd_ocn_tail_tiles(c, Gown), c->wsum_ocean,
diff --git a/qingdai_amd/csrc/qd_ocntail.h b/qingdai_amd/csrc/qd_ocntail.h
--- a/qingdai_amd/csrc/qd_ocntail.h
+++ b/qingdai_amd/csrc/qd_ocntail.h
@@ -20,6 +20,9 @@
     unsigned long long* fix_list = nullptr;
     unsigned long long* acc_next = nullptr;
     unsigned long long* acc_clear = nullptr;
+    int may_skip_land = 0;
+    const int* deep_land = nullptr;
+    unsigned* deep_tally = nullptr;
     QdPeerFold pf;
 };
 
diff --git a/qingdai_amd/csrc/qd_ocntail.hip b/qingdai_amd/csrc/qd_ocntail.hip
--- a/qingdai_amd/csrc/qd_ocntail.hip
+++ b/qingdai_amd/csrc/qd_ocntail.hip
@@ -448,6 +448,21 @@
     return acc;
 }
 
+template <bool FIX>
+__device__ __forceinline__ double qt_currents_land(const QdTailArgs& P, const QtW& W) {
+    const unsigned sb = W.slab, m = (unsigned)W.m;
+    const qt_rsrc E = qt_make_rsrc(P.eta, sb), UO = qt_make_rsrc(P.uo_out, sb), VO = qt_make_rsrc(P.vo_out, sb);
+    unsigned ro = (unsigned)(W.o0 - W.lbase) * m;
+    for (int g = W.o0; g < W.o1; ++g) {
+        qt_st(E, ro, W.vs, 0.0);
+        if (!FIX) { qt_st(UO, ro, W.vs, 0.0); qt_st(VO, ro, W.vs, 0.0); }
+        ro += m;
+    }
+    if (P.deep_tally != nullptr && W.lane == 0)
+        __hip_atomic_fetch_add(P.deep_tally + (FIX ? 2 : 1), 1u, __ATOMIC_RELAXED, __HIP_MEMORY_SCOPE_AGENT);
+    return 0.0;
+}
+
 struct QtSstSlot { double u, v, s, q; int l, ic; qt_f64x2 k0, k1, k2; };
 struct QtSstK { double a, r_a, dt, dlon, r_dlon, dlat, r_dlat, alpha, om_alpha, dtK, rcH, r_rcH, dtq; int has_ice, qfac_on; };
 
@@ -611,7 +626,8 @@
     __shared__ unsigned int s_nfix;
     const QtFixW FX{P.fix_count, P.fix_list, s_fix, &s_nfix};
     if (FIX && W.lane == 0) __hip_atomic_store(&s_nfix, 0u, __ATOMIC_RELAXED, __HIP_MEMORY_SCOPE_WAVEFRONT);
-    double acc = (plain && W.o0 >= 1 && W.o1 <= W.n - 1) ? qt_currents_fast<FIX>(P, W, FX) : qt_currents_wave<FIX>(T, P, W, FX);
+    double acc = qs_deep_land(P.deep_land, w) ? qt_currents_land<FIX>(P, W)
+                 : (plain && W.o0 >= 1 && W.o1 <= W.n - 1) ? qt_currents_fast<FIX>(P, W, FX) : qt_currents_wave<FIX>(T, P, W, FX);
     if (FIX) qt_fix_flush(FX);
     QT_STAMP(2);
     if (FIX) __syncthreads();
@@ -963,6 +979,21 @@
     if ((P.acc_next || P.acc_clear) && (!fast || P.fix_count || !G.full))
         return qd_fail(c, "k_ocn_tail: the mean of a sub-step can only be left to the next launch by the storing fast form");
     if (!fast || !P.acc) { P.fix_count = nullptr; P.fix_list = nullptr; }
+    P.deep_land = nullptr; P.deep_tally = nullptr;
+    if (P.may_skip_land && fast && G.full) {
+        P.deep_tally = c->land_tally;
+        const int key[6] = {G.row0, G.nrows, G.nlon, P.R, P.Rp, QS_TCF};
+        if (!qd_land_skip_lookup(c, 1, key, &P.deep_land, &c->land_skip_last[1])) {
+            std::vector<int> cuts;
+            cuts.push_back(G.row0);
+            if (part.ps > 0) cuts.push_back(part.mid0);
+            const int M = part.mid1 - part.mid0;
+            for (int k = 1; k <= part.nmid; ++k) cuts.push_back(part.mid0 + (int)(((long long)k * M) / part.nmid));
+            if (part.pn > 0) cuts.push_back(G.row0 + G.nrows);
+            if ((int)cuts.size() != nrs + 1) return qd_fail(c, "k_ocn_tail_fast: deep-land flags do not match the strip cut");
+            if (qd_land_skip_build(c, 1, key, cuts, QS_TCF) || !qd_land_skip_lookup(c, 1, key, &P.deep_land, &c->land_skip_last[1])) return -1;
+        }
+    }
     if (fast && P.fix_count) QD_LAUNCH_TIMED(sc, k_ocn_tail_fast<true>, dim3(nrs * P.ntc), dim3(128), c->stream, G, c->tabs, P);
     else if (fast) QD_LAUNCH_TIMED(sc, k_ocn_tail_fast<false>, dim3(nrs * P.ntc), dim3(128), c->stream, G, c->tabs, P);
     else QD_LAUNCH_TIMED(sc, k_ocn_tail_stream<1>, dim3(nrs * P.ntc), dim3(128), c->stream, G, c->tabs, P);
diff --git a/qingdai_amd/csrc/qd_stream.h b/qingdai_amd/csrc/qd_stream.h
--- a/qingdai_amd/csrc/qd_stream.h
+++ b/qingdai_amd/csrc/qd_stream.h
@@ -34,7 +34,13 @@
     const double* acc_partial = nullptr;
     int acc_n = 0;
     double acc_wsum = 0.0;
-};
+    unsigned* deep_tally = nullptr;
+};
+
+#define QS_DEEP_WORDS 64
+struct QsDeepBits { unsigned w[QS_DEEP_WORDS]; };
+static_assert(alignof(QsDeepBits) <= 4 && sizeof(QsOcnArgs) % alignof(QsDeepBits) == 0 && alignof(QsOcnArgs) >= alignof(QsDeepBits),
+              "QsDeepBits must follow QsOcnArgs in the kernarg segment without padding");
 
 typedef unsigned int qs_u32x2 __attribute__((ext_vector_type(2)));
 typedef __amdgpu_buffer_rsrc_t qs_rsrc;
@@ -540,6 +546,19 @@
     return bad;
 }
 
+template <class OUT>
+__device__ __forceinline__ void qs_ocn_wave_land(const QsOcnArgs& A, const QsW& W, OUT& out, double* sy) {
+    for (int g = W.o0; g < W.o1; ++g) out.put(0.0);
+    if (A.acc_read != nullptr) (void)qs_mean_handover(A, sy, false);
+}
+__device__ __forceinline__ bool qs_deep_land(const int* flags, unsigned w) {
+    return flags != nullptr && ((const int QD_CONST*)(unsigned long long)flags)[w] != 0;
+}
+__device__ __forceinline__ bool qs_deep_bit(unsigned b) {
+    const unsigned QD_CONST* bits = (const unsigned QD_CONST*)((const char QD_CONST*)__builtin_amdgcn_kernarg_segment_ptr() + sizeof(QsOcnArgs));
+    return ((bits[(b >> 5) & (QS_DEEP_WORDS - 1)] >> (b & 31u)) & 1u) != 0u;
+}
+
 
 const double* qd_stream_tables(qd_ctx* c, int kind, int nf, const double* const* k4row, const double* k4s, const int* skip);
 bool qd_stream_ocn_args(qd_ctx* c, const QdOcnArgs& P, QsOcnArgs& A);
diff --git a/qingdai_amd/csrc/qd_stream.hip b/qingdai_amd/csrc/qd_stream.hip
--- a/qingdai_amd/csrc/qd_stream.hip
+++ b/qingdai_amd/csrc/qd_stream.hip
@@ -41,7 +41,7 @@
 }
 
 __global__ void __launch_bounds__(192)
-k_ocn_stream(QsOcnArgs A) {
+k_ocn_stream(QsOcnArgs A, QsDeepBits) {
     QsW W;
     qs_strip(A.G, A.vb, A.ntc, A.nrs, W);
     const int wv = __builtin_amdgcn_readfirstlane(threadIdx.x >> 6);
@@ -50,6 +50,13 @@
     const QsRec QD_CONST* fp = &Ak->rec[wv];
     __shared__ double s_em;
     double em = 0.0;
+    const bool deep = qs_deep_bit(blockIdx.x);
+    if (deep && wv <= 1) {
+        QsOutGlobal out{qs_make_rsrc(fp->out, W.slab_bytes), qs_off(A.G, W.o0), W.vs, (unsigned)W.nlon};
+        qs_ocn_wave_land(A, W, out, &s_em);
+        if (A.deep_tally != nullptr && wv == 0 && W.lane == 0) __hip_atomic_fetch_add(A.deep_tally, 1u, __ATOMIC_RELAXED, __HIP_MEMORY_SCOPE_AGENT);
+        return;
+    }
     if (!A.exact) {
         QsOutGlobal out{qs_make_rsrc(fp->out, W.slab_bytes), qs_off(A.G, W.o0), W.vs, (unsigned)W.nlon};
         const bool bad = qs_ocn_wave<QS_FAST>(A, W, wv, fp, out, &s_em, &em);
@@ -203,6 +210,83 @@
     return true;
 }
 
+#define QD_LS_ROWS 5
+#define QD_LS_COLS 3
+bool qd_land_skip_lookup(qd_ctx* c, int which, const int (&key)[6], const int** flags, int* count) {
+    const qd_ctx::QdLandSkip& L = c->land_skip[which];
+    if (L.gen != c->land_gen || !std::equal(key, key + 6, L.key)) return false;
+    *flags = L.count > 0 ? L.d : nullptr;
+    *count = L.count;
+    return true;
+}
+int qd_land_skip_build(qd_ctx* c, int which, const int (&key)[6], const std::vector<int>& cuts, int tc) {
+    qd_ctx::QdLandSkip& L = c->land_skip[which];
+    const int nlat = c->geo.nlat, nlon = c->geo.nlon;
+    const int nrs = (int)cuts.size() - 1, ntc = (nlon + tc - 1) / tc;
+    std::vector<int> fl((size_t)std::max(1, nrs * ntc), 0);
+    int count = 0;
+    if (c->h_land.size() == (size_t)nlat * nlon) {
+        std::vector<int> S((size_t)(nlat + 1) * (nlon + 1), 0);
+        for (int i = 0; i < nlat; ++i)
+            for (int j = 0; j < nlon; ++j)
+                S[(size_t)(i + 1) * (nlon + 1) + j + 1] = S[(size_t)i * (nlon + 1) + j + 1] + S[(size_t)(i + 1) * (nlon + 1) + j] -
+                                                         S[(size_t)i * (nlon + 1) + j] + (c->h_land[(size_t)i * nlon + j] != 1);
+        auto ocean = [&](int r0, int r1, int c0, int c1) {
+            return S[(size_t)r1 * (nlon + 1) + c1] - S[(size_t)r0 * (nlon + 1) + c1] - S[(size_t)r1 * (nlon + 1) + c0] + S[(size_t)r0 * (nlon + 1) + c0];
+        };
+        for (int rs = 0; rs < nrs; ++rs) {
+            const int r0 = cuts[rs] - QD_LS_ROWS, r1 = cuts[rs + 1] + QD_LS_ROWS;
+            if (cuts[rs + 1] <= cuts[rs] || r0 < 1 || r1 > nlat - 1) continue;
+            for (int cs = 0; cs < ntc; ++cs) {
+                const int c0 = cs * tc - QD_LS_COLS, c1 = std::min((cs + 1) * tc, nlon) + QD_LS_COLS;
+                int oc;
+                if (c1 - c0 >= nlon) oc = ocean(r0, r1, 0, nlon);
+                else if (c0 < 0) oc = ocean(r0, r1, c0 + nlon, nlon) + ocean(r0, r1, 0, c1);
+                else if (c1 > nlon) oc = ocean(r0, r1, c0, nlon) + ocean(r0, r1, 0, c1 - nlon);
+                else oc = ocean(r0, r1, c0, c1);
+                if (oc == 0) { fl[(size_t)rs * ntc + cs] = 1; ++count; }
+            }
+        }
+    }
+    if (which == 0) {
+        const unsigned nb = (unsigned)(nrs * ntc);
+        L.bits.assign(QS_DEEP_WORDS, 0u);
+        if (nb > 32u * QS_DEEP_WORDS) count = 0;
+        else
+            for (unsigned b = 0; b < nb; ++b) {
+                const unsigned per = nb >> 3, rem = nb & 7u, x = b & 7u;
+                const unsigned w = x * per + (x < rem ? x : rem) + (b >> 3);
+                if (fl[w]) L.bits[b >> 5] |= 1u << (b & 31u);
+            }
+    } else {
+        if ((int)fl.size() > L.cap) {
+            hipStreamSynchronize(c->stream);
+            if (L.d) hipFree(L.d);
+            L.d = nullptr; L.cap = 0;
+            if (hipMalloc(&L.d, fl.size() * sizeof(int)) != hipSuccess) return qd_fail(c, "deep-land flags: allocation");
+            L.cap = (int)fl.size();
+        }
+        if (hipMemcpyAsync(L.d, fl.data(), fl.size() * sizeof(int), hipMemcpyHostToDevice, c->stream) != hipSuccess) return qd_fail(c, "deep-land flags: copy");
+        hipStreamSynchronize(c->stream);
+    }
+    L.n = (int)fl.size(); L.count = count; L.gen = c->land_gen;
+    std::copy(key, key + 6, L.key);
+    return 0;
+}
+
+static int qs_land_skip(qd_ctx* c, const QdGeom& G, const QsShape& sh, QsDeepBits& D, int* count) {
+    const int key[6] = {G.row0, G.nrows, G.nlon, sh.nrs, sh.vb, QS_TC};
+    const int* unused = nullptr;
+    if (!qd_land_skip_lookup(c, 0, key, &unused, count)) {
+        std::vector<int> cuts(sh.nrs + 1);
+        for (int rs = 0; rs <= sh.nrs; ++rs) cuts[rs] = G.row0 + qs_cut(G.nrows, sh.nrs, sh.vb, rs);
+        if (qd_land_skip_build(c, 0, key, cuts, QS_TC) || !qd_land_skip_lookup(c, 0, key, &unused, count)) return -1;
+    }
+    const std::vector<unsigned>& b = c->land_skip[0].bits;
+    std::copy(b.begin(), b.end(), D.w);
+    return 0;
+}
+
 static bool qs_seg_ok(const QdGeom& G) {
     const int s0 = G.row0, s1 = G.row0 + G.nrows;
     return !((s0 > 0 && s0 < 5) || (s1 < G.nlat && s1 > G.nlat - 5) || G.nrows < 10);
@@ -233,7 +317,7 @@
         const QdGeom& G = S.g[k];
         const QsShape sh = qs_shape(c, G.nrows, G.nlon, 2, G.row0 + G.nrows == G.nlat);
         A.G = G; A.vb = sh.vb; A.nrs = sh.nrs; A.ntc = (G.nlon + QS_TC - 1) / QS_TC;
-        if (!qd_launch_ocn_stream_push(c, A)) hipLaunchKernelGGL(k_ocn_stream, dim3(A.nrs * A.ntc), dim3(192), 0, c->stream, A);
+        if (!qd_launch_ocn_stream_push(c, A)) hipLaunchKernelGGL(k_ocn_stream, dim3(A.nrs * A.ntc), dim3(192), 0, c->stream, A, QsDeepBits{});
     }
     return 0;
 }
@@ -257,6 +341,9 @@
     QD_ROWS(c, margin, G,
             const QsShape sh = qs_shape(c, G.nrows, G.nlon, 2, G.row0 + G.nrows == G.nlat);
             A.G = G; A.vb = sh.vb; A.nrs = sh.nrs; A.ntc = (G.nlon + QS_TC - 1) / QS_TC;
-            QD_LAUNCH_TIMED(sc, k_ocn_stream, dim3(A.nrs * A.ntc), dim3(192), c->stream, A));
-    return 0;
-}
+            QsDeepBits D{};
+            if (P.may_skip_land && G.full && qs_land_skip(c, G, sh, D, &c->land_skip_last[0])) return -1;
+            A.deep_tally = (P.may_skip_land && G.full) ? c->land_tally : nullptr;
+            QD_LAUNCH_TIMED(sc, k_ocn_stream, dim3(A.nrs * A.ntc), dim3(192), c->stream, A, D));
+    return 0;
+}
diff --git a/qingdai_amd/device.py b/qingdai_amd/device.py
--- a/qingdai_amd/device.py
+++ b/qingdai_amd/device.py
@@ -566,6 +566,16 @@
         self._chk(self.lib.qd_ocean_mean_next_count(self.h, ctypes.byref(n)), "qd_ocean_mean_next_count")
         return n.value
 
+    def ocean_land_skip_counts(self):
+        n = (ctypes.c_int64 * 2)(0, 0)
+        self._chk(self.lib.qd_ocean_land_skip_counts(self.h, n), "qd_ocean_land_skip_counts")
+        return int(n[0]), int(n[1])
+
+    def ocean_land_skip_tally(self):
+        n = (ctypes.c_int64 * 3)(0, 0, 0)
+        self._chk(self.lib.qd_ocean_land_skip_tally(self.h, n), "qd_ocean_land_skip_tally")
+        return int(n[0]), int(n[1]), int(n[2])
+
     def counters(self):
         a, o = ctypes.c_int64(0), ctypes.c_int64(0)
         self.lib.qd_get_step_counter(self.h, ctypes.byref(a), ctypes.byref(o))
```

Result: no change. 5.066 planet-days/s (-0.4%).
